# CompVis/stable-diffusion

Hardware: AMD Instinct MI355X
Metric: 512x512 images/sec, SD-v1-4 50-step PLMS CFG=7.5 (higher is better)
Workload: dtype f16

## Files before the change

include/sdmi.h:

```cpp
#ifndef SDMI_H_
#define SDMI_H_

#include <stdint.h>

#ifdef __cplusplus
extern "C" {
#endif

#define SDMI_ABI_VERSION 17

typedef struct sdmi_unet sdmi_unet;

typedef struct sdmi_unet_cfg {
  int32_t in_channels;
  int32_t out_channels;
  int32_t model_channels;
  int32_t num_res_blocks;
  int32_t n_levels;
  int32_t channel_mult[8];
  int32_t n_attention_resolutions;
  int32_t attention_resolutions[8];
  int32_t num_heads;
  int32_t transformer_depth;
  int32_t context_dim;
// ... 95 lines not shown
int sdmi_clip_set_weight(sdmi_clip* h, const char* key, const float* ptr, const int64_t* shape, int ndim, void* stream);
int sdmi_clip_finalize(sdmi_clip* h);
int64_t sdmi_clip_workspace_bytes(sdmi_clip* h, int B, int L);
int sdmi_clip_forward(sdmi_clip* h, const int64_t* ids, float* out, int B, int L, void* workspace, int64_t workspace_bytes,
                      void* stream);

typedef struct sdmi_bert sdmi_bert;
typedef struct sdmi_bert_cfg {
  int32_t vocab_size;
  int32_t dim;
  int32_t depth;
  int32_t heads;
  int32_t dim_head;
  int32_t ff_inner;
  int32_t max_seq_len;
} sdmi_bert_cfg;
int sdmi_bert_create(const sdmi_bert_cfg* cfg, sdmi_bert** out);
int sdmi_bert_destroy(sdmi_bert* h);
int sdmi_bert_num_weights(const sdmi_bert* h);
int sdmi_bert_weight_info(const sdmi_bert* h, int idx, char* key_buf, int key_buf_len, int64_t* shape4, int* ndim);
int sdmi_bert_set_weight(sdmi_bert* h, const char* key, const float* ptr, const int64_t* shape, int ndim, void* stream);
int sdmi_bert_finalize(sdmi_bert* h);
int64_t sdmi_bert_workspace_bytes(sdmi_bert* h, int B, int L);
int sdmi_bert_forward(sdmi_bert* h, const int64_t* ids, float* out, int B, int L, void* workspace, int64_t workspace_bytes,
                      void* stream);

typedef struct sdmi_igemm_desc {
  const void* a0; const void* a1; const void* a2;
  int32_t c0, c1, c2, lda0, lda1, lda2;
  int32_t B, Hin, Win, Hout, Wout, ksize, stride, up;
  const void* w;
  int32_t N;
  int32_t mode;
  const float* bias; const float* rowvec; int32_t ld_rowvec;
  const float* residual; int32_t ldr;
  float* out_f32; void* out_f16; int32_t ldo;
  void* seg_dst[3]; int32_t seg_kind[3];
  int32_t heads, dh, ntok, ntok_pad, segC;
  int32_t splitk;
  float* splitk_ws; int64_t splitk_ws_floats;
  int32_t tile;
  int32_t dma;
  int32_t asym_pad;
  int32_t gn_n; void* gn_acc[2]; int32_t gn_cpg[2]; int32_t gn_cbase[2];
  int32_t* splitk_cnt; int32_t splitk_cnt_ints;
  int32_t split16;
  const float* f16_scale; float* lnp_out;
  const float* lnf_part; int32_t lnf_npart; float lnf_eps; const float* lnf_cs; const float* lnf_d;
  const float* pgn_gamma; const float* pgn_beta; float pgn_eps; int32_t pgn_silu;
  void* pgn_out; int32_t pgn_keep_f32; int32_t* pgn_applied;
  void* out_lo;
} sdmi_igemm_desc;
int sdmi_k_igemm(const sdmi_igemm_desc* d, void* stream);
int sdmi_k_ff_tail(const sdmi_igemm_desc* proj_out, const void* ln_f16, const float* lnp, float ln_eps, const float* csd,
                   const void* wgg_f16, const void* wff2_f16, const float* bff2, const float* t, void* stream);
int sdmi_k_st_tail(const sdmi_igemm_desc* proj_out, const void* a_f16, const void* wo_f16, const float* bo, float* t, const float* ln_gamma,
                   float ln_eps, const float* csd, const void* wgg_f16, const void* wff2_f16, const float* bff2, void* stream);
int sdmi_k_gn_conv3(const sdmi_igemm_desc* conv, const float* x0, const float* x1, int c0, int c1, float* gn_ws, int64_t gn_ws_floats,
                    const float* gn_gamma, const float* gn_beta, float gn_eps, void* stream);
int sdmi_k_st_head(const float* x, float* gn_ws, int64_t gn_ws_floats, const float* gn_gamma, const float* gn_beta, float gn_eps,
                   const void* w_in3, const float* b_in, float* t, const float* ln_gamma, float ln_eps, const void* wqkv_f16,
                   const float* lnf_cs, const float* lnf_d, void* q, void* k, void* vt, int B, int ntok, int ntok_pad, int heads, int dh,
                   int C, void* stream);
int sdmi_k_st_mid(const void* a_f16, const void* wo_f16, const float* bo, float* t, const float* ln_gamma, float ln_eps, const void* wq_f16,
                  const float* lnf_cs, const float* lnf_d, void* q, int B, int ntok, int heads, int dh, int C, void* stream);
int sdmi_k_st_mid_ctx(const void* a_f16, const void* wo_f16, const float* bo, float* t, const float* ln_gamma, float ln_eps, const void* wq_f16,
                      const float* lnf_cs, const float* lnf_d, const void* ctx_k, const void* ctx_vt, int nkv, int nkv_pad, float scale, void* ao_out,
                      int B, int ntok, int heads, int dh, int C, void* stream);
int sdmi_k_ln_fold_prep(const void* w_f16, int N, int K, int ldw, const float* gamma, const float* beta, const float* bias,
                        float* cs, float* d, void* stream);
int sdmi_k_attention(const void* q, const void* k, const void* vt, void* out, int BH, int heads, int nq, int nkv,
                     int nkv_pad, int d, float scale, void* stream);
int sdmi_k_attention_split16(const void* q, const void* q_lo, const void* k, const void* k_lo, const void* vt, const void* vt_lo, void* out,
                             void* out_lo, int BH, int heads, int nq, int nkv, int nkv_pad, int d, float scale, void* stream);
int sdmi_k_attention_causal(const void* q, const void* k, const void* vt, void* out, int BH, int heads, int n, int n_pad,
                            int d, float scale, void* stream);
int sdmi_k_groupnorm(const float* x0, const float* x1, int c0, int c1, int B, int HW, const float* gamma,
                     const float* beta, float eps, int silu, void* out_f16, float* out_f32, void* raw_f16, void* out_lo,
                     void* raw_lo, float* partial_ws, int64_t partial_floats, void* stream);
int64_t sdmi_k_groupnorm_ws_floats(int B, int HW);
int sdmi_k_layernorm(const float* x, const float* gamma, const float* beta, void* out_f16, int M, int C, float eps,
                     void* stream);
int sdmi_k_cast_f16(const float* x, void* out_f16, void* out_lo, int64_t n, void* stream);
int sdmi_k_split_heads(const float* src, int ld, int col0, void* dst, void* dst_lo, int kind, int B, int ntok, int ntok_pad, int heads, int dh,
                       void* stream);
int sdmi_k_geglu_split(const float* src, int M, int F, void* out, void* out_lo, void* stream);
int sdmi_k_layernorm_split(const float* x, const float* gamma, const float* beta, void* out, void* out_lo, int M, int C, float eps, void* stream);
int sdmi_k_timestep_embedding(const int64_t* t_i64, const float* t_f32, float* out, int B, int dim, void* stream);
int sdmi_k_small_linear(const float* in, int ld_in, const float* w, const float* bias, float* out, int ld_out, int B,
                        int N, int K, int silu_in, void* stream);
int sdmi_k_conv_in(const float* x_nchw, const float* w_oihw, const float* bias, float* out_nhwc, int B, int Cin, int H,
                   int W, int Cout, void* stream);
int sdmi_k_conv_out(const float* h_nhwc, const float* w_ohwi, const float* bias, float* out_nchw, int B, int H, int W,
                    int Cin, int Cout, void* stream);
int sdmi_k_pack_conv_weight(const float* w_oihw, void* dst_f16, int O, int I, int KH, int KW, void* stream);
int sdmi_k_pack_conv_out(const float* w_oihw, float* dst_ohwi, int O, int I, void* stream);
int sdmi_k_pack_split3(const float* w, void* dst_f16, int N, int K, void* stream);
int sdmi_k_pack_conv_split3(const float* w_oihw, void* dst_f16, int O, int I, int KH, int KW, void* stream);
int sdmi_k_pointwise_nchw(const float* x, const float* w, const float* bias, float* out, int B, int Cin, int Cout, int HW,
                          float in_scale, void* stream);
int sdmi_k_softmax_rows(const float* S, void* P_f16, int rows, int cols, float scale, void* stream);
int sdmi_k_vq_quantize(const float* z, float z_scale, const float* codebook, float* norms_ws, int n_embed, int D, float* zq, int32_t* idx,
                       int B, int HW, void* stream);
int sdmi_k_resample2(const float* x, float* out_f32, void* out_f16, void* out_lo, int B, int H, int W, int C, int dir, void* stream);
int sdmi_k_gelu_erf(const float* x, void* out_f16, int64_t n, void* stream);
int sdmi_k_pack_geglu(const float* w, const float* bias, void* wdst_f16, float* bdst, int N, int K, void* stream);
// ... 17 lines not shown
```

stable-diffusion_amd/_lib.py:

```python
import ctypes as C
import os

_HERE = os.path.dirname(os.path.abspath(__file__))
LIB_PATH = os.environ.get('SDMI_LIB_PATH') or os.path.join(_HERE, 'libsdmi.so')

c_f32p = C.c_void_p
c_ptr = C.c_void_p


class UNetCfg(C.Structure):
    _fields_ = [('in_channels', C.c_int32), ('out_channels', C.c_int32), ('model_channels', C.c_int32),
                ('num_res_blocks', C.c_int32), ('n_levels', C.c_int32), ('channel_mult', C.c_int32 * 8),
                ('n_attention_resolutions', C.c_int32), ('attention_resolutions', C.c_int32 * 8),
                ('num_heads', C.c_int32), ('transformer_depth', C.c_int32), ('context_dim', C.c_int32)]


class VaeCfg(C.Structure):
    _fields_ = [('ch', C.c_int32), ('out_ch', C.c_int32), ('n_levels', C.c_int32), ('ch_mult', C.c_int32 * 8),
                ('num_res_blocks', C.c_int32), ('in_channels', C.c_int32), ('z_channels', C.c_int32),
                ('embed_dim', C.c_int32)]


class UNetExt(C.Structure):
    _fields_ = [('attention_block', C.c_int32), ('resblock_updown', C.c_int32)]
# ... 45 lines not shown
    'sdmi_unet_create_ext': (C.c_int, [C.POINTER(UNetCfg), C.POINTER(UNetExt), C.c_int, C.POINTER(c_ptr)]),
    'sdmi_unet_destroy': (C.c_int, [c_ptr]),
    'sdmi_unet_num_weights': (C.c_int, [c_ptr]),
    'sdmi_unet_weight_info': (C.c_int, [c_ptr, C.c_int, C.c_char_p, C.c_int, C.POINTER(C.c_int64), C.POINTER(C.c_int)]),
    'sdmi_unet_set_weight': (C.c_int, [c_ptr, C.c_char_p, c_ptr, C.POINTER(C.c_int64), C.c_int, c_ptr]),
    'sdmi_unet_finalize': (C.c_int, [c_ptr]),
    'sdmi_unet_packed_bytes': (C.c_int64, [c_ptr]),
    'sdmi_unet_export_packed': (C.c_int, [c_ptr, c_ptr, C.c_int64, c_ptr]),
    'sdmi_unet_import_packed': (C.c_int, [c_ptr, c_ptr, C.c_int64, c_ptr]),
    'sdmi_unet_workspace_bytes': (C.c_int64, [c_ptr, C.c_int, C.c_int, C.c_int, C.c_int]),
    'sdmi_unet_cache_context': (C.c_int, [c_ptr, c_ptr, C.c_int, C.c_int, c_ptr, C.c_int64, c_ptr]),
    'sdmi_unet_reserve_context': (C.c_int, [c_ptr, C.c_int, C.c_int]),
    'sdmi_unet_cache_timesteps': (C.c_int, [c_ptr, C.POINTER(C.c_int64), C.c_int, c_ptr]),
    'sdmi_unet_hint_timestep': (C.c_int, [c_ptr, C.c_int64]),
    'sdmi_unet_tape_stats': (C.c_int, [c_ptr, C.POINTER(C.c_int64), C.POINTER(C.c_int64)]),
    'sdmi_unet_forward': (C.c_int, [c_ptr, c_ptr, c_ptr, c_ptr, c_ptr, c_ptr, C.c_int, C.c_int, C.c_int, C.c_int,
                                    c_ptr, C.c_int64, c_ptr]),
    'sdmi_sampler_step': (C.c_int, [c_ptr, C.c_int, C.c_float, c_ptr, C.c_int, c_ptr, c_ptr, c_ptr, C.c_float,
                                    C.c_float, C.c_float, C.c_float, c_ptr, c_ptr, c_ptr, c_ptr, C.c_int64, c_ptr]),
    'sdmi_dpm_solver_step': (C.c_int, [c_ptr, C.c_int, C.c_float, c_ptr, c_ptr, C.c_float, C.c_float, C.c_float, C.c_float,
                                       C.c_float, C.c_int, c_ptr, c_ptr, C.c_int64, c_ptr]),
    'sdmi_vae_create': (C.c_int, [C.POINTER(VaeCfg), C.c_int, C.POINTER(c_ptr)]),
    'sdmi_vae_destroy': (C.c_int, [c_ptr]),
    'sdmi_vae_create_ext': (C.c_int, [C.POINTER(VaeCfg), C.POINTER(VaeExt), C.c_int, C.POINTER(c_ptr)]),
    'sdmi_vae_decode_vq': (C.c_int, [c_ptr, c_ptr, C.c_float, C.c_int, c_ptr, C.c_int, C.c_int, C.c_int, c_ptr, C.c_int64, c_ptr]),
    'sdmi_k_vq_quantize': (C.c_int, [c_ptr, C.c_float, c_ptr, c_ptr, C.c_int, C.c_int, c_ptr, c_ptr, C.c_int, C.c_int, c_ptr]),
    'sdmi_k_resample2': (C.c_int, [c_ptr, c_ptr, c_ptr, c_ptr, C.c_int, C.c_int, C.c_int, C.c_int, C.c_int, c_ptr]),
    'sdmi_vae_num_weights': (C.c_int, [c_ptr]),
    'sdmi_vae_weight_info': (C.c_int, [c_ptr, C.c_int, C.c_char_p, C.c_int, C.POINTER(C.c_int64), C.POINTER(C.c_int)]),
    'sdmi_vae_set_weight': (C.c_int, [c_ptr, C.c_char_p, c_ptr, C.POINTER(C.c_int64), C.c_int, c_ptr]),
    'sdmi_vae_finalize': (C.c_int, [c_ptr]),
    'sdmi_vae_decode_workspace_bytes': (C.c_int64, [c_ptr, C.c_int, C.c_int, C.c_int]),
    'sdmi_vae_decode': (C.c_int, [c_ptr, c_ptr, C.c_float, c_ptr, C.c_int, C.c_int, C.c_int, c_ptr, C.c_int64, c_ptr]),
    'sdmi_vae_encode_workspace_bytes': (C.c_int64, [c_ptr, C.c_int, C.c_int, C.c_int]),
    'sdmi_vae_encode': (C.c_int, [c_ptr, c_ptr, c_ptr, C.c_int, C.c_int, C.c_int, c_ptr, C.c_int64, c_ptr]),
    'sdmi_clip_create': (C.c_int, [C.POINTER(ClipCfg), C.POINTER(c_ptr)]),
    'sdmi_clip_destroy': (C.c_int, [c_ptr]),
    'sdmi_clip_num_weights': (C.c_int, [c_ptr]),
    'sdmi_clip_weight_info': (C.c_int, [c_ptr, C.c_int, C.c_char_p, C.c_int, C.POINTER(C.c_int64), C.POINTER(C.c_int)]),
    'sdmi_clip_set_weight': (C.c_int, [c_ptr, C.c_char_p, c_ptr, C.POINTER(C.c_int64), C.c_int, c_ptr]),
    'sdmi_clip_finalize': (C.c_int, [c_ptr]),
    'sdmi_clip_workspace_bytes': (C.c_int64, [c_ptr, C.c_int, C.c_int]),
    'sdmi_clip_forward': (C.c_int, [c_ptr, c_ptr, c_ptr, C.c_int, C.c_int, c_ptr, C.c_int64, c_ptr]),
    'sdmi_bert_create': (C.c_int, [C.POINTER(BertCfg), C.POINTER(c_ptr)]),
    'sdmi_bert_destroy': (C.c_int, [c_ptr]),
    'sdmi_bert_num_weights': (C.c_int, [c_ptr]),
    'sdmi_bert_weight_info': (C.c_int, [c_ptr, C.c_int, C.c_char_p, C.c_int, C.POINTER(C.c_int64), C.POINTER(C.c_int)]),
    'sdmi_bert_set_weight': (C.c_int, [c_ptr, C.c_char_p, c_ptr, C.POINTER(C.c_int64), C.c_int, c_ptr]),
    'sdmi_bert_finalize': (C.c_int, [c_ptr]),
    'sdmi_bert_workspace_bytes': (C.c_int64, [c_ptr, C.c_int, C.c_int]),
    'sdmi_bert_forward': (C.c_int, [c_ptr, c_ptr, c_ptr, C.c_int, C.c_int, c_ptr, C.c_int64, c_ptr]),
    'sdmi_has_experiments': (C.c_int, []),
    'sdmi_k_igemm': (C.c_int, [C.POINTER(IGemmDesc), c_ptr]),
    'sdmi_k_ff_tail': (C.c_int, [C.POINTER(IGemmDesc), c_ptr, c_ptr, C.c_float, c_ptr, c_ptr, c_ptr, c_ptr, c_ptr, c_ptr]),
    'sdmi_k_gn_conv3': (C.c_int, [C.POINTER(IGemmDesc), c_ptr, c_ptr, C.c_int, C.c_int, c_ptr, C.c_int64, c_ptr, c_ptr, C.c_float, c_ptr]),
    'sdmi_k_st_mid_ctx': (C.c_int, [c_ptr, c_ptr, c_ptr, c_ptr, c_ptr, C.c_float, c_ptr, c_ptr, c_ptr, c_ptr, c_ptr, C.c_int, C.c_int, C.c_float, c_ptr,
                                    C.c_int, C.c_int, C.c_int, C.c_int, C.c_int, c_ptr]),
    'sdmi_k_st_tail': (C.c_int, [C.POINTER(IGemmDesc), c_ptr, c_ptr, c_ptr, c_ptr, c_ptr, C.c_float, c_ptr, c_ptr, c_ptr, c_ptr, c_ptr]),
    'sdmi_k_st_mid': (C.c_int, [c_ptr, c_ptr, c_ptr, c_ptr, c_ptr, C.c_float, c_ptr, c_ptr, c_ptr, c_ptr, C.c_int, C.c_int, C.c_int, C.c_int,
                                C.c_int, c_ptr]),
    'sdmi_k_st_head': (C.c_int, [c_ptr, c_ptr, C.c_int64, c_ptr, c_ptr, C.c_float, c_ptr, c_ptr, c_ptr, c_ptr, C.c_float, c_ptr, c_ptr, c_ptr,
                                 c_ptr, c_ptr, c_ptr, C.c_int, C.c_int, C.c_int, C.c_int, C.c_int, C.c_int, c_ptr]),
    'sdmi_k_attention_split16': (C.c_int, [c_ptr, c_ptr, c_ptr, c_ptr, c_ptr, c_ptr, c_ptr, c_ptr, C.c_int, C.c_int, C.c_int, C.c_int,
                                           C.c_int, C.c_int, C.c_float, c_ptr]),
    'sdmi_k_attention_causal': (C.c_int, [c_ptr, c_ptr, c_ptr, c_ptr, C.c_int, C.c_int, C.c_int, C.c_int, C.c_int, C.c_float,
                                          c_ptr]),
    'sdmi_k_pointwise_nchw': (C.c_int, [c_ptr, c_ptr, c_ptr, c_ptr, C.c_int, C.c_int, C.c_int, C.c_int, C.c_float, c_ptr]),
    'sdmi_k_softmax_rows': (C.c_int, [c_ptr, c_ptr, C.c_int, C.c_int, C.c_float, c_ptr]),
    'sdmi_k_gelu_erf': (C.c_int, [c_ptr, c_ptr, C.c_int64, c_ptr]),
    'sdmi_k_attention': (C.c_int, [c_ptr, c_ptr, c_ptr, c_ptr, C.c_int, C.c_int, C.c_int, C.c_int, C.c_int, C.c_int,
                                   C.c_float, c_ptr]),
    'sdmi_k_groupnorm': (C.c_int, [c_ptr, c_ptr, C.c_int, C.c_int, C.c_int, C.c_int, c_ptr, c_ptr, C.c_float, C.c_int,
                                   c_ptr, c_ptr, c_ptr, c_ptr, c_ptr, c_ptr, C.c_int64, c_ptr]),
    'sdmi_k_groupnorm_ws_floats': (C.c_int64, [C.c_int, C.c_int]),
    'sdmi_k_layernorm': (C.c_int, [c_ptr, c_ptr, c_ptr, c_ptr, C.c_int, C.c_int, C.c_float, c_ptr]),
    'sdmi_k_cast_f16': (C.c_int, [c_ptr, c_ptr, c_ptr, C.c_int64, c_ptr]),
    'sdmi_k_split_heads': (C.c_int, [c_ptr, C.c_int, C.c_int, c_ptr, c_ptr, C.c_int, C.c_int, C.c_int, C.c_int, C.c_int, C.c_int,
                                     c_ptr]),
    'sdmi_k_geglu_split': (C.c_int, [c_ptr, C.c_int, C.c_int, c_ptr, c_ptr, c_ptr]),
    'sdmi_k_layernorm_split': (C.c_int, [c_ptr, c_ptr, c_ptr, c_ptr, c_ptr, C.c_int, C.c_int, C.c_float, c_ptr]),
    'sdmi_k_timestep_embedding': (C.c_int, [c_ptr, c_ptr, c_ptr, C.c_int, C.c_int, c_ptr]),
    'sdmi_k_small_linear': (C.c_int, [c_ptr, C.c_int, c_ptr, c_ptr, c_ptr, C.c_int, C.c_int, C.c_int, C.c_int,
                                      C.c_int, c_ptr]),
    'sdmi_k_conv_in': (C.c_int, [c_ptr, c_ptr, c_ptr, c_ptr, C.c_int, C.c_int, C.c_int, C.c_int, C.c_int, c_ptr]),
    'sdmi_k_conv_out': (C.c_int, [c_ptr, c_ptr, c_ptr, c_ptr, C.c_int, C.c_int, C.c_int, C.c_int, C.c_int, c_ptr]),
    'sdmi_k_pack_conv_weight': (C.c_int, [c_ptr, c_ptr, C.c_int, C.c_int, C.c_int, C.c_int, c_ptr]),
    'sdmi_k_pack_conv_out': (C.c_int, [c_ptr, c_ptr, C.c_int, C.c_int, c_ptr]),
    'sdmi_k_pack_split3': (C.c_int, [c_ptr, c_ptr, C.c_int, C.c_int, c_ptr]),
    'sdmi_k_pack_conv_split3': (C.c_int, [c_ptr, c_ptr, C.c_int, C.c_int, C.c_int, C.c_int, c_ptr]),
    'sdmi_k_pack_geglu': (C.c_int, [c_ptr, c_ptr, c_ptr, c_ptr, C.c_int, C.c_int, c_ptr]),
    'sdmi_k_ln_fold_prep': (C.c_int, [c_ptr, C.c_int, C.c_int, C.c_int, c_ptr, c_ptr, c_ptr, c_ptr, c_ptr, c_ptr]),
    'sdmi_image_to_uint8': (C.c_int, [c_ptr, c_ptr, C.c_int, C.c_int, C.c_int, C.c_int, c_ptr]),
    'sdmi_range_check': (C.c_int, [C.c_int]),
    'sdmi_range_report': (C.c_int, [C.c_char_p, C.c_int]),
    'sdmi_tune_begin': (C.c_int, []),
    'sdmi_tune_round': (C.c_int, [C.c_int]),
    'sdmi_tune_end': (C.c_int, [C.c_char_p, C.POINTER(C.c_int)]),
    'sdmi_tune_dump': (C.c_int, [C.c_char_p, C.c_int]),
    'sdmi_profile_begin': (C.c_int, []),
    'sdmi_profile_end': (C.c_int, [C.c_char_p, C.c_int]),
    'sdmi_k_prefetch_lines': (C.c_int, [c_ptr, C.c_int64, c_ptr]),
    'sdmi_zero_page': (c_ptr, []),
}

_lib = None

# ... 39 lines not shown
```

stable-diffusion_amd/csrc/api.cpp:

```cpp
#include <string.h>

#include <new>

#include "prof.h"
#include "split16.h"
#include "unet.h"
#include "vae.h"
#include "clip.h"

namespace sdmi {
static thread_local std::string g_err;
void set_error(const std::string& msg) { g_err = msg; }
int fail(const std::string& msg) { g_err = msg; return -1; }
}

struct sdmi_unet { sdmi::UNet impl; };
struct sdmi_vae { sdmi::Vae impl; };
struct sdmi_clip { sdmi::ClipText impl; };
struct sdmi_bert { sdmi::BertText impl; };

using namespace sdmi;

static void* g_zero_page[16] = {nullptr};
static int zero_page(const f16** out) {
// ... 273 lines not shown
  SDMI_CHECK(h && ids && out, "null argument");
  return h->impl.forward(ids, out, B, L, workspace, workspace_bytes, (hipStream_t)stream, false, nullptr);
}
int sdmi_k_vq_quantize(const float* z, float z_scale, const float* codebook, float* norms_ws, int n_embed, int D, float* zq, int32_t* idx,
                       int B, int HW, void* stream) {
  if (launch_vq_norms(codebook, norms_ws, n_embed, D, (hipStream_t)stream)) return -1;
  return launch_vq_quantize(z, z_scale, codebook, norms_ws, n_embed, D, zq, (int*)idx, B, HW, (hipStream_t)stream);
}
int sdmi_k_resample2(const float* x, float* out_f32, void* out_f16, void* out_lo, int B, int H, int W, int C, int dir, void* stream) {
  return launch_resample2(x, out_f32, (f16*)out_f16, (f16*)out_lo, B, H, W, C, dir, (hipStream_t)stream);
}
int sdmi_k_gelu_erf(const float* x, void* out_f16, int64_t n, void* stream) {
  return launch_gelu_erf(x, (f16*)out_f16, n, (hipStream_t)stream);
}
int sdmi_k_attention_causal(const void* q, const void* k, const void* vt, void* out, int BH, int heads, int n, int n_pad,
                            int d, float scale, void* stream) {
  AttnParams a = AttnParams();
  a.q = (const f16*)q; a.k = (const f16*)k; a.vt = (const f16*)vt; a.out = (f16*)out;
  a.BH = BH; a.heads = heads; a.nq = n; a.nkv = n; a.nkv_pad = n_pad; a.d = d; a.scale = scale; a.causal = 1;
  return launch_attention(a, (hipStream_t)stream);
}

static int igemm_params_of(const sdmi_igemm_desc* d, IGemmParams& p) {
  p.a0 = (const f16*)d->a0; p.a1 = (const f16*)d->a1; p.a2 = (const f16*)d->a2;
  p.c0 = d->c0; p.c1 = d->c1; p.c2 = d->c2; p.lda0 = d->lda0; p.lda1 = d->lda1; p.lda2 = d->lda2;
  p.B = d->B; p.Hin = d->Hin; p.Win = d->Win; p.Hout = d->Hout; p.Wout = d->Wout;
  p.ksize = d->ksize; p.stride = d->stride; p.up = d->up; p.pad = d->asym_pad ? 0 : 1;
  p.w = (const f16*)d->w; p.M = d->B * d->Hout * d->Wout; p.N = d->N; p.K = d->ksize * d->ksize * (d->c0 + d->c1 + d->c2);
  p.mode = d->mode; p.bias = d->bias; p.rowvec = d->rowvec; p.ld_rowvec = d->ld_rowvec;
  p.residual = d->residual; p.ldr = d->ldr; p.out_f32 = d->out_f32; p.out_f16 = (f16*)d->out_f16; p.ldo = d->ldo;
  for (int i = 0; i < 3; ++i) { p.seg_dst[i] = (f16*)d->seg_dst[i]; p.seg_kind[i] = d->seg_kind[i]; }
  p.heads = d->heads; p.dh = d->dh; p.ntok = d->ntok; p.ntok_pad = d->ntok_pad; p.segC = d->segC;
  p.splitk = d->splitk; p.splitk_ws = d->splitk_ws; p.splitk_ws_floats = d->splitk_ws_floats;
  p.splitk_cnt = d->splitk_cnt; p.splitk_cnt_ints = d->splitk_cnt_ints;
  p.gn_n = d->gn_n;
  for (int i = 0; i < 2; ++i) { p.gn_acc[i] = (long long*)d->gn_acc[i]; p.gn_cpg[i] = d->gn_cpg[i]; p.gn_cbase[i] = d->gn_cbase[i]; }
  if (d->split16) {
    p.split16 = 1; p.c1 = 0; p.K = d->c0; p.ldw = 3 * d->c0;
  }
  p.f16_scale = d->f16_scale; p.lnp_out = d->lnp_out;
  p.lnf_part = d->lnf_part; p.lnf_npart = d->lnf_npart; p.lnf_eps = d->lnf_eps; p.lnf_cs = d->lnf_cs; p.lnf_d = d->lnf_d;
  p.pgn_gamma = d->pgn_gamma; p.pgn_beta = d->pgn_beta; p.pgn_eps = d->pgn_eps; p.pgn_silu = d->pgn_silu;
  p.pgn_out = (f16*)d->pgn_out; p.pgn_keep_f32 = d->pgn_keep_f32; p.pgn_applied = d->pgn_applied;
  p.out_lo = (f16*)d->out_lo;
  return zero_page(&p.zero_page);
}
int sdmi_k_igemm(const sdmi_igemm_desc* d, void* stream) {
  SDMI_CHECK(d, "null descriptor");
  IGemmParams p = IGemmParams();
  if (igemm_params_of(d, p)) return -1;
  IGemmTune t; t.tile = d->tile; t.dma = d->dma;
  return launch_igemm(p, t, (hipStream_t)stream);
}
int sdmi_k_ff_tail(const sdmi_igemm_desc* proj_out, const void* ln_f16, const float* lnp, float ln_eps, const float* csd,
                   const void* wgg_f16, const void* wff2_f16, const float* bff2, const float* t, void* stream) {
  SDMI_CHECK(proj_out, "null descriptor");
  FfTailParams q = FfTailParams();
  if (igemm_params_of(proj_out, q.epi)) return -1;
  SDMI_CHECK(proj_out->split16 && proj_out->ksize == 1, "ff_tail: the proj_out descriptor is a split-fp16 1x1 (w = sdmi_k_pack_split3)");
  q.ln = (const f16*)ln_f16; q.lnp = lnp; q.ln_eps = ln_eps; q.csd = csd; q.wgg = (const f16*)wgg_f16; q.wff2 = (const f16*)wff2_f16;
  q.bff2 = bff2; q.t = t; q.wpo = (const f16*)proj_out->w;
  return launch_ff_tail(q, (hipStream_t)stream);
}
int sdmi_k_st_tail(const sdmi_igemm_desc* proj_out, const void* a_f16, const void* wo_f16, const float* bo, float* t, const float* ln_gamma,
                   float ln_eps, const float* csd, const void* wgg_f16, const void* wff2_f16, const float* bff2, void* stream) {
  SDMI_CHECK(proj_out && a_f16, "null argument");
  FfTailParams q = FfTailParams();
  if (igemm_params_of(proj_out, q.epi)) return -1;
  SDMI_CHECK(proj_out->split16 && proj_out->ksize == 1, "st_tail: the proj_out descriptor is a split-fp16 1x1 (w = sdmi_k_pack_split3)");
  q.a16 = (const f16*)a_f16; q.wo = (const f16*)wo_f16; q.bo = bo; q.ln_gamma = ln_gamma; q.ln_eps = ln_eps; q.csd = csd;
  q.wgg = (const f16*)wgg_f16; q.wff2 = (const f16*)wff2_f16; q.bff2 = bff2; q.t = t; q.wpo = (const f16*)proj_out->w;
  return launch_ff_tail(q, (hipStream_t)stream);
}
int sdmi_k_gn_conv3(const sdmi_igemm_desc* conv, const float* x0, const float* x1, int c0, int c1, float* gn_ws, int64_t gn_ws_floats,
                    const float* gn_gamma, const float* gn_beta, float gn_eps, void* stream) {
  SDMI_CHECK(conv && x0 && gn_ws && gn_gamma && gn_beta, "gn_conv3: null argument");
  GnConvParams q = GnConvParams();
  if (igemm_params_of(conv, q.epi)) return -1;
  const int B = q.epi.B;
  SDMI_CHECK(gn_ws_floats >= gn_acc_words(B) * 2, "groupnorm workspace too small");
  SDMI_HIP_OK(hipMemsetAsync(gn_ws, 0, gn_acc_words(B) * sizeof(long long), (hipStream_t)stream));
  GroupNormParams g = GroupNormParams();
  g.x0 = x0; g.c0 = c0; g.x1 = x1; g.c1 = c1; g.B = B; g.HW = q.epi.Hout * q.epi.Wout; g.gamma = gn_gamma; g.beta = gn_beta; g.eps = gn_eps;
  g.stats_only = 1; g.acc = (long long*)gn_ws;
  if (launch_groupnorm(g, (hipStream_t)stream)) return -1;
  q.x0 = x0; q.x1 = x1; q.c0 = c0; q.c1 = c1; q.gn_acc = (const long long*)gn_ws; q.gn_gamma = gn_gamma; q.gn_beta = gn_beta; q.gn_eps = gn_eps;
  q.w = (const f16*)conv->w;
  return launch_gn_conv3(q, (hipStream_t)stream);
}
int sdmi_k_st_head(const float* x, float* gn_ws, int64_t gn_ws_floats, const float* gn_gamma, const float* gn_beta, float gn_eps,
                   const void* w_in3, const float* b_in, float* t, const float* ln_gamma, float ln_eps, const void* wqkv_f16,
                   const float* lnf_cs, const float* lnf_d, void* q, void* k, void* vt, int B, int ntok, int ntok_pad, int heads, int dh,
                   int C, void* stream) {
  SDMI_CHECK(x && gn_ws && gn_gamma && gn_beta, "st_head: null argument");
  SDMI_CHECK(gn_ws_floats >= gn_acc_words(B) * 2, "groupnorm workspace too small");
  SDMI_HIP_OK(hipMemsetAsync(gn_ws, 0, gn_acc_words(B) * sizeof(long long), (hipStream_t)stream));
  GroupNormParams g = GroupNormParams();
  g.x0 = x; g.c0 = C; g.B = B; g.HW = ntok; g.gamma = gn_gamma; g.beta = gn_beta; g.eps = gn_eps; g.stats_only = 1; g.acc = (long long*)gn_ws;
  if (launch_groupnorm(g, (hipStream_t)stream)) return -1;
  StHeadParams p = StHeadParams();
  p.x = x; p.gn_acc = (const long long*)gn_ws; p.gn_gamma = gn_gamma; p.gn_beta = gn_beta; p.gn_eps = gn_eps;
  p.w_in = (const f16*)w_in3; p.b_in = b_in; p.t = t; p.ln_gamma = ln_gamma; p.ln_eps = ln_eps; p.wqkv = (const f16*)wqkv_f16;
  p.lnf_cs = lnf_cs; p.lnf_d = lnf_d; p.q = (f16*)q; p.k = (f16*)k; p.vt = (f16*)vt;
  p.M = B * ntok; p.B = B; p.ntok = ntok; p.ntok_pad = ntok_pad; p.heads = heads; p.dh = dh; p.C = C;
  return launch_st_head(p, (hipStream_t)stream);
}
// ... 142 lines not shown
```

stable-diffusion_amd/csrc/common.h:

```cpp
#pragma once
#include <hip/hip_runtime.h>
#include <stdint.h>
#include <algorithm>
#include <string>

#include "tape.h"

typedef _Float16 f16;
typedef _Float16 f16x2 __attribute__((ext_vector_type(2)));
typedef _Float16 f16x4 __attribute__((ext_vector_type(4)));
typedef _Float16 f16x8 __attribute__((ext_vector_type(8)));
typedef float f32x4 __attribute__((ext_vector_type(4)));
typedef float f32x16 __attribute__((ext_vector_type(16)));

#ifdef __HIPCC__
__device__ __forceinline__ float gn_apply_elem(float v, float mean, float rstd, float gamma, float beta, int silu) {
  float t = __builtin_fmaf((v - mean) * rstd, gamma, beta);
  if (silu) t = t * __builtin_amdgcn_rcpf(1.0f + __expf(-t));
  return t;
}
__device__ __forceinline__ void gn_acc_add(unsigned long long* dst, float v) {
  const double d = (double)v;
  const double hi = rint(d);
  atomicAdd(dst, (unsigned long long)(long long)hi);
// ... 30 lines not shown
      return ::sdmi::fail(std::string(#expr) + ": " + hipGetErrorString(_e));                \
  } while (0)

#define SDMI_CHECK(cond, msg)                                                                \
  do {                                                                                       \
    if (!(cond)) return ::sdmi::fail(std::string("check failed: ") + #cond + " -- " + (msg)); \
  } while (0)

static inline int cdiv(int a, int b) { return (a + b - 1) / b; }
static inline int64_t round_up(int64_t a, int64_t b) { return (a + b - 1) / b * b; }

enum EpiMode { EPI_PLAIN = 0, EPI_GEGLU = 1, EPI_HEADS = 2 };

#ifdef SDMI_NT_STORES
#define SDMI_ST(T, ptr, val) __builtin_nontemporal_store((T)(val), (T*)(ptr))
#else
#define SDMI_ST(T, ptr, val) (*(T*)(ptr) = (T)(val))
#endif
#ifndef SDMI_W_AUX
#define SDMI_W_AUX 0
#endif
#ifndef SDMI_WT_STORES
#define SDMI_WT_STORES 1
#endif
#if defined(__HIPCC__) && SDMI_WT_STORES >= 1
typedef unsigned sdmi_u32x4 __attribute__((ext_vector_type(4)));
typedef unsigned sdmi_u32x2 __attribute__((ext_vector_type(2)));
__device__ __forceinline__ void sdmi_st_wt16(const void* base, size_t byte_off, f32x4 v) {
  if (__builtin_expect(byte_off < (size_t)0x80000000u - 16, 1)) {
    const __amdgpu_buffer_rsrc_t r = __builtin_amdgcn_make_buffer_rsrc((void*)base, 0, (int)0x80000000, 0x00020000);
    __builtin_amdgcn_raw_buffer_store_b128(__builtin_bit_cast(sdmi_u32x4, v), r, (int)byte_off, 0, 16);
  } else {
    *(f32x4*)((char*)base + byte_off) = v;
  }
}
__device__ __forceinline__ void sdmi_st_wt8(const void* base, size_t byte_off, f16x4 v) {
  if (__builtin_expect(byte_off < (size_t)0x80000000u - 16, 1)) {
    const __amdgpu_buffer_rsrc_t r = __builtin_amdgcn_make_buffer_rsrc((void*)base, 0, (int)0x80000000, 0x00020000);
    __builtin_amdgcn_raw_buffer_store_b64(__builtin_bit_cast(sdmi_u32x2, v), r, (int)byte_off, 0, 16);
  } else {
    *(f16x4*)((char*)base + byte_off) = v;
  }
}
#define SDMI_ST_F32X4(base, off, val) sdmi_st_wt16((base), (size_t)(off) * 4, (val))
#if SDMI_WT_STORES >= 2
#define SDMI_ST_F16X4(base, off, val) sdmi_st_wt8((base), (size_t)(off) * 2, (val))
#else
#define SDMI_ST_F16X4(base, off, val) SDMI_ST(f16x4, (base) + (off), (val))
#endif
#else
#define SDMI_ST_F32X4(base, off, val) SDMI_ST(f32x4, (base) + (off), (val))
#define SDMI_ST_F16X4(base, off, val) SDMI_ST(f16x4, (base) + (off), (val))
#endif

struct IGemmParams {
  const f16* a0 = nullptr; const f16* a1 = nullptr; const f16* a2 = nullptr;
  int c0 = 0, c1 = 0, c2 = 0;
  int lda0 = 0, lda1 = 0, lda2 = 0;
  int B = 1, Hin = 1, Win = 1;
  int Hout = 1, Wout = 1;
  int ksize = 1, stride = 1, up = 0;
  int pad = 1;
  const f16* w = nullptr;
  int M = 0, N = 0, K = 0;
  int k_alg = 0;
  int split16 = 0;
  int ldw = 0;
  int mode = EPI_PLAIN;
  const float* bias = nullptr;
  const float* rowvec = nullptr; int ld_rowvec = 0;
  const float* residual = nullptr; int ldr = 0;
  float* out_f32 = nullptr; f16* out_f16 = nullptr; int ldo = 0;
  f16* out_lo = nullptr;
  const float* ln_gamma = nullptr; const float* ln_beta = nullptr; f16* ln_out = nullptr; float ln_eps = 1e-5f;
  const float* f16_scale = nullptr;
  float* lnp_out = nullptr;
  const float* lnf_part = nullptr; int lnf_npart = 0; float lnf_eps = 1e-5f;
  const float* lnf_cs = nullptr; const float* lnf_d = nullptr;
  f16* seg_dst[3] = {nullptr, nullptr, nullptr};
  int seg_kind[3] = {0, 0, 0};
  int heads = 0, dh = 0, ntok = 0, ntok_pad = 0, segC = 0;
  int splitk = 1;
  float* splitk_ws = nullptr; int64_t splitk_ws_floats = 0;
  int* splitk_cnt = nullptr; int splitk_cnt_ints = 0;
  int gn_safe = 0;
#ifdef SDMI_IGEMM_TIMING
  long long* dbg_times = nullptr;
  int dbg_abl = 0;
#endif
  int splitk_fused = 0;
  int slab_tiled = 0, slab_bm = 0, slab_bn = 0, slab_wm = 0, slab_wn = 0;
  int slab_sh_qpt = 0, slab_sh_nt = 0, slab_sh_tn = 0, slab_sh_wn = 0;
  int epi_vec = 0;
  int tile_n_fastest = 0;
  const f16* zero_page = nullptr;
  int gn_n = 0;
  long long* gn_acc[2] = {nullptr, nullptr};
  int gn_cpg[2] = {0, 0}, gn_cbase[2] = {0, 0};
  unsigned long long gn_magic[2] = {0, 0};
  const float* pgn_gamma = nullptr; const float* pgn_beta = nullptr; float pgn_eps = 1e-5f; int pgn_silu = 1;
  f16* pgn_out = nullptr;
  int pgn_keep_f32 = 0;
  int* pgn_applied = nullptr;
  unsigned long long magic_hw = 0, magic_w = 0, magic_w2 = 0;
  int log2w = 0;
  const float* xf0 = nullptr; const float* xf1 = nullptr;
  const long long* gn_in_acc = nullptr;
  const float* gn_in_gamma = nullptr; const float* gn_in_beta = nullptr; float gn_in_eps = 1e-5f; int gn_in_silu = 1;
  f16* raw_hi = nullptr; f16* raw_lo = nullptr;
  f16* gn_scratch = nullptr;
  unsigned long long magic_cpg_in = 0;
  int halo_thi = 0, halo_ipt = 1, log2_tpi = 30;
  unsigned long long magic_hpi = 0;
};

constexpr int SDMI_NUM_TILES = 22;
struct IGemmTune {
  int tile = -1;
  int dma = -1;
};

int launch_igemm(const IGemmParams& p, const IGemmTune& tune, hipStream_t stream);
bool range_check_enabled();
uint64_t tune_generation();
bool tune_collecting();
int range_check_set(int enable);
int range_scan(const char* what, const f16* p, int64_t n, hipStream_t stream);
int range_report(std::string* json);

int tune_begin();
int tune_round(int r);
int tune_end(const char* path, int* n_keys);
int tune_dump(std::string* out);
int launch_splitk_reduce(const IGemmParams& p, int nsplit, hipStream_t stream);

struct FfTailParams {
  const f16* ln = nullptr;
  const float* lnp = nullptr;
  float ln_eps = 1e-5f;
  const float* csd = nullptr;
  const f16* wgg = nullptr;
  const f16* wff2 = nullptr;
  const float* bff2 = nullptr;
  const float* t = nullptr;
  const f16* wpo = nullptr;
  const f16* a16 = nullptr;
  const f16* wo = nullptr;
  const float* bo = nullptr;
  const float* ln_gamma = nullptr;
#ifdef SDMI_RC_TIMING
  long long* dbg = nullptr;
#endif
  IGemmParams epi;
};
bool ff_tail_supported(int C, int M, int rows_per_sample);
int launch_ff_tail(const FfTailParams& p, hipStream_t stream);

struct StHeadParams {
  const f16* a16 = nullptr;
  const float* x = nullptr;
  const long long* gn_acc = nullptr;
  const float* gn_gamma = nullptr; const float* gn_beta = nullptr; float gn_eps = 1e-6f;
  const f16* w_in = nullptr;
  const float* b_in = nullptr;
  float* t = nullptr;
  const float* ln_gamma = nullptr;
// ... 134 lines not shown
```

stable-diffusion_amd/csrc/conv3halo.hip:

```cpp
#include "igemm_dev.h"

namespace sdmi {
namespace {

template <int BM, int BN, int WARPS_M, int WARPS_N, int NS>
__global__ void __launch_bounds__(WARPS_M* WARPS_N * 64) conv3halo_kernel(const IGemmParams p, const int tiles_m,
                                                                           const int tiles_n, const int chunks_per_split) {
#if defined(__HIP_DEVICE_COMPILE__)
  constexpr int NT = WARPS_M * WARPS_N * 64;
  constexpr int RPP = NT / 8;
  constexpr int PB = BN / RPP;
  constexpr int WTM = BM / WARPS_M, WTN = BN / WARPS_N;
  constexpr int TM = WTM / 32, TN = WTN / 32;
  constexpr int HPMAX = (BM / 64 + 2) * 66;
  constexpr int AHP = (HPMAX + RPP - 1) / RPP;
  constexpr int HALO_BYTES = AHP * RPP * 128;
  constexpr int BSTAGE = BN * 128;
  constexpr int LDS_BYTES = 2 * HALO_BYTES + NS * BSTAGE;
  constexpr int LASTA = 10 - NS;
  constexpr int PA = (AHP + LASTA) / (LASTA + 1);
  constexpr int KS = BK / 16;
  constexpr int G = (TM * TN >= 4) ? 1 : 2;
  constexpr int U = KS / G;
  constexpr int MPU = G * TM * TN;
  static_assert(PB >= 1 && TM >= 1 && TN >= 1 && RPP % 16 == 0 && NS >= 2 && NS <= 9, "tile/wave shape");
  static_assert(LDS_BYTES <= 160 * 1024, "LDS budget");

  __shared__ __attribute__((aligned(16))) unsigned char smem[LDS_BYTES];

  const int nblk = gridDim.x;
  const int bid = blockIdx.x;
  const int q8 = nblk >> 3, r8 = nblk & 7, xcd = bid & 7;
  const int wgid = (xcd < r8 ? xcd * (q8 + 1) : r8 * (q8 + 1) + (xcd - r8) * q8) + (bid >> 3);
  const int tiles_mn = tiles_m * tiles_n;
  const int split = wgid / tiles_mn;
  const int tmn = wgid - split * tiles_mn;
  int tile_m, tile_n;
  if (p.tile_n_fastest) { tile_m = tmn / tiles_n; tile_n = tmn - tile_m * tiles_n; }
  else { tile_n = tmn / tiles_m; tile_m = tmn - tile_n * tiles_m; }
  const int m0 = tile_m * BM, n0 = tile_n * BN;
  const int nch = (p.c0 + p.c1 + p.c2) / BK;
  const int c_begin = split * chunks_per_split;
  const int c_end = min(nch, c_begin + chunks_per_split);
  if (c_begin >= c_end) return;

  const int tid = threadIdx.x;
  SDMI_STAMP(dbg_t0);
  const int lane = tid & 63;
  const int wave = tid >> 6;
  const int cpos = tid & 7, lrow = tid >> 3;
  const int gch = cpos ^ ((lrow >> 1) & 7);
  const int wave_u = __builtin_amdgcn_readfirstlane(wave);
  const int wm = wave / WARPS_N, wn = wave - wm * WARPS_N;
  const int l31 = lane & 31, lg = lane >> 5;
  const int rsw = (l31 >> 1) & 7;

  const int W = p.Wout, H = p.Hout, HW = H * W, W2 = W + 2, ld = p.lda0;
  const int bimg = m0 / HW;
  const int THI = p.halo_thi;
  const int HPI = (THI + 2) * W2;
  const int y0 = p.halo_ipt > 1 ? 0 : (m0 - bimg * HW) >> p.log2w;
  const int HP = p.halo_ipt * HPI;
  constexpr int OOB = (int)0x80000000;

  int hvoff[AHP];
#pragma unroll
  for (int q = 0; q < AHP; ++q) {
    const int hp = q * RPP + lrow;
    const int ip = fast_div(hp, p.magic_hpi), hr = hp - ip * HPI;
    const int hy = fast_div(hr, p.magic_w2), hx = hr - hy * W2;
    const int y = y0 + hy - 1, x = hx - 1;
    const bool valid = hp < HP && y >= 0 && y < H && x >= 0 && x < W;
    hvoff[q] = valid ? ((((bimg + ip) * H + y) * W + x) * ld + gch * 8) * 2 : OOB;
  }
  int b_off[PB];
#pragma unroll
  for (int i = 0; i < PB; ++i) {
    const int n = min(n0 + i * RPP + lrow, p.N - 1);
    b_off[i] = (n * p.K + gch * 8) * 2;
  }
  int hr0[TM];
#pragma unroll
  for (int i = 0; i < TM; ++i) {
    const int ml = wm * WTM + i * 32 + l31;
// ... 91 lines not shown
      const int kt = c * 9 + tap;
      const int tap1 = tap == 8 ? 0 : tap + 1;
      const int hb1 = tap == 8 ? (hb ^ 1) : hb;
      const int cur1 = (cur + 1 == NS) ? 0 : cur + 1;
      int ab1[TM];
#pragma unroll
      for (int i = 0; i < TM; ++i) ab1[i] = a_base(i, tap1 / 3, tap1 % 3, hb1);
      const int alo = a_lo(tap);
      const int na = a_hi(tap) - alo;
      const int npieces = na + PB;
      const int ppu = (npieces + U - 2) / (U - 1);
      const int bt = min(kt + NS - 1, kt_last);
#pragma unroll
      for (int u = 0; u < U; ++u) {
        if (u + 1 < U) {
#pragma unroll
          for (int g = 0; g < G; ++g) read_frags(ab, cur, (u + 1) * G + g, fa[(u + 1) & 1][g], fb[(u + 1) & 1][g]);
#pragma unroll
          for (int e = u * ppu; e < (u + 1) * ppu && e < npieces; ++e) {
            if (e < na) issue_halo(csn, hb ^ 1, alo + e);
            else issue_b(bt, nxt, e - na);
          }
        } else {
          wait_vmcnt_n(in_flight_ok(tap));
          asm volatile("s_waitcnt lgkmcnt(0)\n\ts_barrier" ::: "memory");
#pragma unroll
          for (int g = 0; g < G; ++g) read_frags(ab1, cur1, g, fa[0][g], fb[0][g]);
        }
#pragma unroll
        for (int g = 0; g < G; ++g) mfma_step(fa[u & 1][g], fb[u & 1][g]);
        __builtin_amdgcn_sched_group_barrier(0x100, G * (TM + TN), 0);
#pragma unroll
        for (int e = 0; e < MPU; ++e) {
          __builtin_amdgcn_sched_group_barrier(0x008, 1, 0);
          if (u + 1 < U && e < ppu && u * ppu + e < npieces) __builtin_amdgcn_sched_group_barrier(0x010, 1, 0);
        }
      }
#pragma unroll
      for (int i = 0; i < TM; ++i) ab[i] = ab1[i];
      cur = cur1;
      nxt = (nxt + 1 == NS) ? 0 : nxt + 1;
      hb = hb1;
    }
  }
  wait_vmcnt<0>();
  SDMI_STAMP(dbg_t2);
  igemm_epilogue<BM, BN, WARPS_M, WARPS_N, LDS_BYTES>(p, acc, m0, n0, split, tile_m, tile_n, smem);
#ifdef SDMI_IGEMM_TIMING
  if (p.dbg_times && tid == 0) {
    long long* d = p.dbg_times + 6 * (size_t)blockIdx.x;
    d[0] = dbg_t0; d[1] = dbg_t1; d[2] = dbg_t2; d[4] = (long long)__builtin_readcyclecounter();
  }
#endif
#endif
}

}

bool halo_supported(const IGemmParams& p, int bm) {
  const int W = p.Wout, HW = p.Hout * p.Wout;
  if (!(p.ksize == 3 && p.stride == 1 && p.pad == 1 && !p.up && p.Hin == p.Hout && p.Win == p.Wout && W >= 8 && W <= 64 &&
        (W & (W - 1)) == 0 && bm % W == 0))
    return false;
  const int cap = (((bm / 64 + 2) * 66 + bm / 4 - 1) / (bm / 4)) * (bm / 4);
  if (bm <= HW) return HW % bm == 0 && (bm / W + 2) * (W + 2) <= cap;
  return bm % HW == 0 && p.M % bm == 0 && (bm / HW) * (p.Hout + 2) * (W + 2) <= cap;
}

template <int BM, int BN, int WARPS_M, int WARPS_N, int NS>
int launch_halo_cfg(const IGemmParams& p, int splitk, hipStream_t stream) {
  SDMI_CHECK(halo_supported(p, BM), "halo-staged conv tile requested for an unsupported shape");
  const int tiles_m = cdiv(p.M, BM), tiles_n = cdiv(p.N, BN);
  const int nch = (p.c0 + p.c1 + p.c2) / BK;
  const int chunks_per_split = cdiv(nch, splitk);
  const int nsplit = cdiv(nch, chunks_per_split);
  IGemmParams q = p;
  q.splitk = nsplit;
  q.tile_n_fastest = tile_order_n_fastest(p);
  q.splitk_fused = 0;
  slab_layout(q, BM, BN, WARPS_M, WARPS_N, nsplit);
  q.epi_vec = epi_vec_ok(p);
  SDMI_CHECK(splitk_ws_need(p, BM, BN, nsplit) <= p.splitk_ws_floats, "split-K workspace too small");
  SDMI_CHECK((int64_t)p.M < (int64_t)65536 * p.Hout * p.Wout, "fast_div_hw: at most 65535 samples per launch");
  q.magic_hw = div_magic_hw(p.Hout * p.Wout);
  q.magic_w = div_magic(p.Wout);
  q.magic_w2 = div_magic(p.Wout + 2);
  q.log2w = 0;
  while ((1 << q.log2w) < p.Wout) ++q.log2w;
  {
    const int HW = p.Hout * p.Wout;
    q.halo_ipt = BM <= HW ? 1 : BM / HW;
    q.halo_thi = BM <= HW ? BM / p.Wout : p.Hout;
    q.magic_hpi = div_magic((q.halo_thi + 2) * (p.Wout + 2));
    const int tpi = q.halo_thi * p.Wout;
    q.log2_tpi = 0;
    while ((1 << q.log2_tpi) < tpi) ++q.log2_tpi;
    if (q.halo_ipt == 1) q.log2_tpi = 30;
  }
  for (int t = 0; t < p.gn_n; ++t) q.gn_magic[t] = div_magic(p.gn_cpg[t]);
  dim3 grid(tiles_m * tiles_n * nsplit), block(WARPS_M * WARPS_N * 64);
  static const int by_shape = env_int("SDMI_PROF_SHAPES", 0);
  std::string pname = std::string("conv3halo_") + std::to_string(BM) + "x" + std::to_string(BN) + "w" +
                      std::to_string(WARPS_M * WARPS_N) + "s" + std::to_string(NS);
  if (by_shape && prof_enabled())
    pname += "_M" + std::to_string(p.M) + "_N" + std::to_string(p.N) + "_K" + std::to_string(p.K) + "_s" + std::to_string(nsplit);
  const double src_pix = (double)p.B * p.Hin * p.Win;
  ProfScope ps(pname.c_str(), 2.0 * p.M * (double)p.N * p.K,
               src_pix * (p.c0 + p.c1) * 2.0 + (double)p.N * p.K * 2.0 + (double)p.M * p.N * ((p.out_f32 ? 4.0 : 0.0) + (p.out_f16 ? 2.0 : 0.0)) +
                   (p.residual ? (double)p.M * p.N * 4.0 : 0.0),
               stream);
  SDMI_LAUNCH((conv3halo_kernel<BM, BN, WARPS_M, WARPS_N, NS>), grid, block, 0, stream, q, tiles_m, tiles_n, chunks_per_split);
  SDMI_HIP_OK(hipGetLastError());
  ps.end();
  if (nsplit > 1) return launch_splitk_reduce(q, nsplit, stream);
  if (q.ln_out) return launch_layernorm(q.out_f32, q.ln_gamma, q.ln_beta, q.ln_out, q.M, q.N, q.ln_eps, stream);
  return 0;
}

int launch_halo_tile(int tile, const IGemmParams& p, int splitk, hipStream_t stream) {
  switch (tile) {
    case 14: return launch_halo_cfg<256, 64, 4, 2, 5>(p, splitk, stream);
    case 15: return launch_halo_cfg<256, 128, 4, 2, 3>(p, splitk, stream);
    case 16: return launch_halo_cfg<128, 64, 2, 2, 8>(p, splitk, stream);
    case 17: return launch_halo_cfg<128, 128, 2, 2, 5>(p, splitk, stream);
    default: return fail("not a halo-staged conv tile id");
  }
}

}
```

stable-diffusion_amd/csrc/gemm_split16.hip:

```cpp
#include "igemm_dev.h"

namespace sdmi {
namespace {

template <int BM, int BN, int WARPS_M, int WARPS_N, int NS>
__global__ void __launch_bounds__(WARPS_M* WARPS_N * 64) gemm_split16_kernel(const IGemmParams p, const int tiles_m, const int tiles_n,
                                                                               const int kt_per_split) {
#if defined(__HIP_DEVICE_COMPILE__)
  constexpr int NT = WARPS_M * WARPS_N * 64;
  constexpr int RPP = NT / 8;
  constexpr int A_PASSES = BM / RPP, B_PASSES = BN / RPP;
  constexpr int WTM = BM / WARPS_M, WTN = BN / WARPS_N;
  constexpr int TM = WTM / 32, TN = WTN / 32;
  constexpr int A_BYTES = BM * 128, B_BYTES = BN * 128;
  constexpr int STAGE_BYTES = 2 * (A_BYTES + B_BYTES);
  constexpr int LPT = 2 * (A_PASSES + B_PASSES);
  constexpr int KS = BK / 16;
  constexpr int PPU = (LPT + KS - 2) / (KS - 1);
  static_assert(A_PASSES >= 1 && B_PASSES >= 1 && TM >= 1 && TN >= 1 && RPP % 16 == 0 && NS >= 2, "tile/wave shape");
  static_assert(NS * STAGE_BYTES <= 160 * 1024, "LDS budget");

  __shared__ __attribute__((aligned(16))) unsigned char smem[NS * STAGE_BYTES];

  const int nblk = gridDim.x, bid = blockIdx.x;
  const int q8 = nblk >> 3, r8 = nblk & 7, xcd = bid & 7;
  const int wgid = (xcd < r8 ? xcd * (q8 + 1) : r8 * (q8 + 1) + (xcd - r8) * q8) + (bid >> 3);
  const int tiles_mn = tiles_m * tiles_n;
  const int split = wgid / tiles_mn;
  const int tmn = wgid - split * tiles_mn;
  int tile_m, tile_n;
  if (p.tile_n_fastest) { tile_m = tmn / tiles_n; tile_n = tmn - tile_m * tiles_n; }
  else { tile_n = tmn / tiles_m; tile_m = tmn - tile_n * tiles_m; }
  const int m0 = tile_m * BM, n0 = tile_n * BN;
  const int nkt = p.K / BK;
  const int kt_begin = split * kt_per_split;
  const int kt_end = min(nkt, kt_begin + kt_per_split);
  if (kt_begin >= kt_end) return;

  const int tid = threadIdx.x;
  SDMI_STAMP(dbg_t0);
  const int lane = tid & 63, wave = tid >> 6;
  const int cpos = tid & 7, lrow = tid >> 3;
  const int gch = cpos ^ ((lrow >> 1) & 7);
  const int wave_u = __builtin_amdgcn_readfirstlane(wave);

  int a_off[A_PASSES], b_off[B_PASSES];
#pragma unroll
  for (int i = 0; i < A_PASSES; ++i) a_off[i] = (min(m0 + i * RPP + lrow, p.M - 1) * p.lda0 + gch * 8) * 2;
#pragma unroll
  for (int i = 0; i < B_PASSES; ++i) b_off[i] = (min(n0 + i * RPP + lrow, p.N - 1) * p.ldw + gch * 8) * 2;
  constexpr int OOB = (int)0x80000000;
  const __amdgpu_buffer_rsrc_t rsrc_hi = __builtin_amdgcn_make_buffer_rsrc((void*)p.a0, 0, OOB, 0x00020000);
  const __amdgpu_buffer_rsrc_t rsrc_lo = __builtin_amdgcn_make_buffer_rsrc((void*)p.a1, 0, OOB, 0x00020000);
  const __amdgpu_buffer_rsrc_t rsrc_w = __builtin_amdgcn_make_buffer_rsrc((void*)p.w, 0, OOB, 0x00020000);
  const int w_lo_off = 2 * p.K * 2;

  auto issue_piece = [&](int kt, int stage, int q) {
    const int soff = kt * (BK * 2);
    const bool isA = q < 2 * A_PASSES;
    const int qa = isA ? q : q - 2 * A_PASSES;
    const int npass = isA ? A_PASSES : B_PASSES;
    const int half = qa >= npass ? 1 : 0, pass = qa - half * npass;
    const unsigned row0 = (isA ? half * BM : 2 * BM + half * BN) + pass * RPP + wave_u * 8;
    auto dst = (__attribute__((address_space(3))) void*)(smem + stage * STAGE_BYTES + row0 * 128);
    if (isA) __builtin_amdgcn_raw_ptr_buffer_load_lds(half ? rsrc_lo : rsrc_hi, dst, 16, a_off[pass], soff, 0, 0);
    else __builtin_amdgcn_raw_ptr_buffer_load_lds(rsrc_w, dst, 16, b_off[pass], soff + (half ? w_lo_off : 0), 0, SDMI_W_AUX);
  };

  const int wm = wave / WARPS_N, wn = wave - wm * WARPS_N;
  const int l31 = lane & 31, lg = lane >> 5;
  const int rsw = (l31 >> 1) & 7;
  f32x16 acc[TM][TN];
#pragma unroll
  for (int i = 0; i < TM; ++i)
#pragma unroll
    for (int j = 0; j < TN; ++j)
#pragma unroll
      for (int r = 0; r < 16; ++r) acc[i][j][r] = 0.f;

  struct Frags { f16x8 ah[TM], al[TM], bh[TN], bl[TN]; };
  const int a_lds = (wm * WTM + l31) * 128, b_lds = 2 * A_BYTES + (wn * WTN + l31) * 128;
  auto read_frags = [&](int stage, int ks, Frags& f) {
    const unsigned char* st = smem + stage * STAGE_BYTES + (((ks * 2 + lg) ^ rsw) << 4);
#pragma unroll
    for (int i = 0; i < TM; ++i) {
      f.ah[i] = *(const f16x8*)(st + a_lds + i * 32 * 128);
      f.al[i] = *(const f16x8*)(st + a_lds + A_BYTES + i * 32 * 128);
    }
#pragma unroll
    for (int j = 0; j < TN; ++j) {
      f.bh[j] = *(const f16x8*)(st + b_lds + j * 32 * 128);
      f.bl[j] = *(const f16x8*)(st + b_lds + B_BYTES + j * 32 * 128);
    }
  };
  auto mfma_step = [&](const Frags& f) {
#pragma unroll
    for (int i = 0; i < TM; ++i)
#pragma unroll
      for (int j = 0; j < TN; ++j) {
        acc[i][j] = __builtin_amdgcn_mfma_f32_32x32x16_f16(f.ah[i], f.bh[j], acc[i][j], 0, 0, 0);
        acc[i][j] = __builtin_amdgcn_mfma_f32_32x32x16_f16(f.al[i], f.bh[j], acc[i][j], 0, 0, 0);
        acc[i][j] = __builtin_amdgcn_mfma_f32_32x32x16_f16(f.ah[i], f.bl[j], acc[i][j], 0, 0, 0);
      }
  };

  SDMI_STAMP(dbg_t1);
  int ld_kt = kt_begin;
  auto next_kt = [&]() { const int k = ld_kt; if (ld_kt + 1 < kt_end) ++ld_kt; return k; };
#pragma unroll
  for (int s = 0; s < NS - 1; ++s) {
    const int k = next_kt();
#pragma unroll
    for (int q = 0; q < LPT; ++q) issue_piece(k, s, q);
  }
  wait_vmcnt<LPT*(NS - 2)>();
  asm volatile("s_waitcnt lgkmcnt(0)\n\ts_barrier" ::: "memory");
  Frags fr[2];
  read_frags(0, 0, fr[0]);
  int cur = 0, nxt = NS - 1;
  for (int kt = kt_begin; kt < kt_end; ++kt) {
    const int kload = next_kt();
    const int cur1 = (cur + 1 == NS) ? 0 : cur + 1;
#pragma unroll
    for (int u = 0; u < KS; ++u) {
      if (u + 1 < KS) {
        read_frags(cur, u + 1, fr[(u + 1) & 1]);
#pragma unroll
        for (int q = u * PPU; q < (u + 1) * PPU && q < LPT; ++q) issue_piece(kload, nxt, q);
      } else {
        wait_vmcnt<LPT*(NS - 2)>();
        asm volatile("s_waitcnt lgkmcnt(0)\n\ts_barrier" ::: "memory");
        read_frags(cur1, 0, fr[0]);
      }
      mfma_step(fr[u & 1]);
      __builtin_amdgcn_sched_group_barrier(0x100, 2 * (TM + TN), 0);
#pragma unroll
      for (int e = 0; e < 3 * TM * TN; ++e) {
        __builtin_amdgcn_sched_group_barrier(0x008, 1, 0);
        if (u + 1 < KS && e < PPU && u * PPU + e < LPT) __builtin_amdgcn_sched_group_barrier(0x010, 1, 0);
      }
    }
    cur = cur1;
    nxt = (nxt + 1 == NS) ? 0 : nxt + 1;
  }
  wait_vmcnt<0>();
  SDMI_STAMP(dbg_t2);
  igemm_epilogue<BM, BN, WARPS_M, WARPS_N, NS * STAGE_BYTES>(p, acc, m0, n0, split, tile_m, tile_n, smem);
#ifdef SDMI_IGEMM_TIMING
  if (p.dbg_times && tid == 0) {
    long long* d = p.dbg_times + 6 * (size_t)blockIdx.x;
    d[0] = dbg_t0; d[1] = dbg_t1; d[2] = dbg_t2; d[4] = (long long)__builtin_readcyclecounter();
  }
#endif
#endif
}

template <int BM, int BN, int WARPS_M, int WARPS_N, int NS>
int launch_split16_cfg(const IGemmParams& p, int splitk, hipStream_t stream) {
  const int tiles_m = cdiv(p.M, BM), tiles_n = cdiv(p.N, BN);
  const int nkt = p.K / BK;
  const int kt_per_split = cdiv(nkt, splitk);
  const int nsplit = cdiv(nkt, kt_per_split);
  IGemmParams q = p;
  q.splitk = nsplit;
  q.tile_n_fastest = tile_order_n_fastest(p);
  q.splitk_fused = 0;
  slab_layout(q, BM, BN, WARPS_M, WARPS_N, nsplit);
  q.epi_vec = epi_vec_ok(p);
  SDMI_CHECK(splitk_ws_need(p, BM, BN, nsplit) <= p.splitk_ws_floats, "split-K workspace too small");
  SDMI_CHECK((int64_t)p.M < (int64_t)65536 * p.Hout * p.Wout, "fast_div_hw: at most 65535 samples per launch");
  q.magic_hw = div_magic_hw(p.Hout * p.Wout);
  q.magic_w = div_magic(p.Wout);
  for (int t = 0; t < p.gn_n; ++t) q.gn_magic[t] = div_magic(p.gn_cpg[t]);
  dim3 grid(tiles_m * tiles_n * nsplit), block(WARPS_M * WARPS_N * 64);
  static const int by_shape = env_int("SDMI_PROF_SHAPES", 0);
  std::string pname = std::string("gemm_split16_") + std::to_string(BM) + "x" + std::to_string(BN) + "w" +
                      std::to_string(WARPS_M * WARPS_N) + "s" + std::to_string(NS);
  if (by_shape && prof_enabled())
    pname += "_M" + std::to_string(p.M) + "_N" + std::to_string(p.N) + "_K" + std::to_string(p.K) + "_s" + std::to_string(nsplit);
  ProfScope ps(pname.c_str(), 2.0 * p.M * (double)p.N * p.K,
               (double)p.M * p.K * 2.0 + (double)p.N * p.K * 2.0 + (double)p.M * p.N * ((p.out_f32 ? 4.0 : 0.0) + (p.out_f16 ? 2.0 : 0.0)) +
                   (p.residual ? (double)p.M * p.N * 4.0 : 0.0),
               stream, 6.0 * p.M * (double)p.N * p.K);
  SDMI_LAUNCH((gemm_split16_kernel<BM, BN, WARPS_M, WARPS_N, NS>), grid, block, 0, stream, q, tiles_m, tiles_n, kt_per_split);
  SDMI_HIP_OK(hipGetLastError());
  ps.end();
  if (nsplit > 1) return launch_splitk_reduce(q, nsplit, stream);
  if (q.ln_out) return launch_layernorm(q.out_f32, q.ln_gamma, q.ln_beta, q.ln_out, q.M, q.N, q.ln_eps, stream);
  return 0;
}

}

bool split16_tile_supported(int tile) { return tile == 0 || tile == 1 || tile == 2 || tile == 4 || tile == 5 || tile == 8 || tile == 10; }

int launch_split16_tile(int tile, const IGemmParams& p, int splitk, hipStream_t stream) {
  SDMI_CHECK(p.a0 && p.a1 && p.ksize == 1 && p.mode == EPI_PLAIN && p.c1 == 0 && p.c2 == 0 && p.K == p.c0 && p.K % BK == 0 &&
                 p.lda0 % 8 == 0 && p.ldw % 8 == 0 && p.ldw >= 3 * p.K,
             "split-fp16 GEMM: hi + lo operands, plain epilogue, K % 64 == 0, packed [N][3K] weights");
  switch (tile) {
    case 0: return launch_split16_cfg<128, 128, 2, 2, 2>(p, splitk, stream);
    case 1: return launch_split16_cfg<128, 64, 2, 2, 2>(p, splitk, stream);
    case 2: return launch_split16_cfg<64, 64, 2, 2, 2>(p, splitk, stream);
    case 4: return launch_split16_cfg<128, 64, 2, 2, 3>(p, splitk, stream);
    case 5: return launch_split16_cfg<64, 64, 2, 2, 3>(p, splitk, stream);
    case 8: return launch_split16_cfg<64, 128, 2, 2, 3>(p, splitk, stream);
    case 10: return launch_split16_cfg<64, 64, 2, 2, 4>(p, splitk, stream);
    default: return fail("split-fp16 GEMM: tile id without an instantiation");
  }
}

}
```

stable-diffusion_amd/csrc/igemm.hip:

```cpp
#include <dlfcn.h>

#include <map>
#include <mutex>
#include <tuple>
#include <vector>

#include "igemm_dev.h"

namespace sdmi {
namespace {

__global__ void __launch_bounds__(256) splitk_reduce_kernel(IGemmParams p, int nsplit, int rows_per_block) {
  __shared__ unsigned long long s_gn[2][32][GN_WORDS];
  const int tx = threadIdx.x & 7, ty = threadIdx.x >> 3;
  const int n = (blockIdx.x * 8 + tx) * 4;
  const int row0 = blockIdx.y * rows_per_block;
  const int HW = p.Hout * p.Wout;
  const bool gn = p.gn_n > 0;
  const bool ncol = n < p.N;
  if (gn) {
    for (int i = threadIdx.x; i < 2 * 32 * GN_WORDS; i += 256) (&s_gn[0][0][0])[i] = 0ull;
    __syncthreads();
  }
  const size_t slab_sz = (size_t)p.M * p.N;
// ... 85 lines not shown
  f16* dst = p.seg_dst[seg];
  if (p.seg_kind[seg] == 0) {
    *(f16x4*)(dst + (bh * p.ntok + tok) * p.dh + dd) = f16x4{(f16)v[0], (f16)v[1], (f16)v[2], (f16)v[3]};
  } else {
#pragma unroll
    for (int j = 0; j < 4; ++j) dst[(bh * p.dh + dd + j) * p.ntok_pad + tok] = (f16)v[j];
  }
}

__device__ __forceinline__ float pick4(const f32x4 v, int idx) {
  return idx == 0 ? v[0] : (idx == 1 ? v[1] : (idx == 2 ? v[2] : v[3]));
}
template <int CTRL>
__device__ __forceinline__ float quad_dpp(float x) {
  return __builtin_bit_cast(float, __builtin_amdgcn_update_dpp(0, __builtin_bit_cast(int, x), CTRL, 0xF, 0xF, true));
}
__device__ __forceinline__ f32x4 quad_transpose(const f32x4 v, int sub) {
  const float r0 = pick4(v, sub);
  const float r1 = quad_dpp<0x93>(pick4(v, (sub + 1) & 3));
  const float r2 = quad_dpp<0x4E>(pick4(v, (sub + 2) & 3));
  const float r3 = quad_dpp<0x39>(pick4(v, (sub + 3) & 3));
  const f32x4 r = {r0, r1, r2, r3};
  return f32x4{pick4(r, sub & 3), pick4(r, (sub - 1) & 3), pick4(r, (sub - 2) & 3), pick4(r, (sub - 3) & 3)};
}
__device__ __forceinline__ void quad_partials_split(const f32x4 v, int gsplit, float* a1, float* a2, float* c1, float* c2) {
#pragma clang fp contract(off)
  float s1 = 0.f, s2 = 0.f, t1 = 0.f, t2 = 0.f;
#pragma unroll
  for (int j = 0; j < 4; ++j) {
    const float sq = v[j] * v[j];
    if (j < gsplit) { s1 += v[j]; s2 += sq; } else { t1 += v[j]; t2 += sq; }
  }
  *a1 = s1; *a2 = s2; *c1 = t1; *c2 = t2;
}
struct TiledQuad { size_t off; int m, n; bool valid; };
__device__ __forceinline__ TiledQuad tiled_quad(const IGemmParams& p, int q, int lane) {
  const int BM = p.slab_bm, BN = p.slab_bn;
  const int WTM = BM / p.slab_wm, WTN = BN >> p.slab_sh_wn;
  const int tiles_n = (p.N + BN - 1) / BN;
  const int tile = q >> p.slab_sh_qpt, rem = q - (tile << p.slab_sh_qpt);
  const int blk = rem >> p.slab_sh_nt, t_in = rem - (blk << p.slab_sh_nt);
  const int wave = t_in >> 6;
  const int ij = blk >> 2, r4 = blk & 3, i = ij >> p.slab_sh_tn, j = ij - (i << p.slab_sh_tn);
  const int wm = wave >> p.slab_sh_wn, wn = wave - (wm << p.slab_sh_wn);
  const int tile_m = tile / tiles_n, tile_n = tile - tile_m * tiles_n;
  const int l31 = lane & 31, lg = lane >> 5;
  TiledQuad t;
  t.off = (size_t)tile * (size_t)(BM * BN) + (size_t)rem * 4;
  t.m = tile_m * BM + wm * WTM + i * 32 + 8 * r4 + 4 * lg + (l31 & 3);
  t.n = tile_n * BN + wn * WTN + j * 32 + (l31 & ~3);
  t.valid = t.m < p.M && t.n < p.N;
  return t;
}
#ifndef SDMI_REDUCE_GN_XCD_DEFAULT
#define SDMI_REDUCE_GN_XCD_DEFAULT 0
#endif
constexpr int COOP_BAR_INTS = 18 * 32;
template <bool COOP>
__global__ void __launch_bounds__(COOP ? 1024 : 256) splitk_reduce_tiled_kernel(IGemmParams p, int nsplit) {
  constexpr int NWV = COOP ? 16 : 4;
  __shared__ unsigned long long s_gn[2][NWV][32][GN_WORDS];
  const int tid = threadIdx.x, lane = tid & 63, wv = tid >> 6, NTB = blockDim.x;
  const bool gn = p.gn_n > 0;
  if (gn) {
    for (int i = tid; i < 2 * NWV * 32 * GN_WORDS; i += NTB) (&s_gn[0][0][0][0])[i] = 0ull;
    __syncthreads();
  }
  const TiledQuad t = tiled_quad(p, blockIdx.x * NTB + tid, lane);
  const int ntiles = ((p.M + p.slab_bm - 1) / p.slab_bm) * ((p.N + p.slab_bn - 1) / p.slab_bn);
  const size_t split_stride = (size_t)ntiles * (size_t)(p.slab_bm * p.slab_bn);
  const float* src = p.splitk_ws + t.off;
  const int HW = p.Hout * p.Wout;
  const int m = min(t.m, p.M - 1), n = min(t.n, p.N - 4);
  f32x4 biasv = {0.f, 0.f, 0.f, 0.f}, rvv = {0.f, 0.f, 0.f, 0.f}, resv = {0.f, 0.f, 0.f, 0.f};
  if (p.bias) biasv = *(const f32x4*)(p.bias + n);
  if (p.rowvec) rvv = *(const f32x4*)(p.rowvec + (size_t)(m / HW) * p.ld_rowvec + n);
  if (p.residual) resv = *(const f32x4*)(p.residual + (size_t)m * p.ldr + n);
  f32x4 part[16];
#pragma unroll
  for (int s = 0; s < 16; ++s) part[s] = (s < nsplit) ? *(const f32x4*)(src + s * split_stride) : f32x4{0.f, 0.f, 0.f, 0.f};
  f32x4 a = part[0];
#pragma unroll
  for (int s = 1; s < 16; ++s) a += part[s];
  f32x4 v = quad_transpose(a, lane & 3);
  v += biasv;
  if (p.rowvec) v += rvv;
  if (p.residual) v += resv;
  if (t.valid) {
    if (p.out_f32 && (!COOP || p.pgn_keep_f32)) SDMI_ST_F32X4(p.out_f32, (size_t)m * p.ldo + n, v);
    if (p.out_f16) SDMI_ST_F16X4(p.out_f16, (size_t)m * p.ldo + n, (f16x4{(f16)v[0], (f16)v[1], (f16)v[2], (f16)v[3]}));
    if (p.out_lo) {
      f16x4 lo;
#pragma unroll
      for (int j = 0; j < 4; ++j) lo[j] = (f16)(v[j] - (float)(f16)v[j]);
      *(f16x4*)(p.out_lo + (size_t)m * p.ldo + n) = lo;
    }
  }
  if (gn) {
    if (t.valid) {
      for (int tg = 0; tg < p.gn_n; ++tg) {
        const int c = p.gn_cbase[tg] + n;
        const int g0 = fast_div(c, p.gn_magic[tg]), g1 = fast_div(c + 3, p.gn_magic[tg]);
        const int gsplit = (g0 + 1) * p.gn_cpg[tg] - c;
        float a1, a2, c1, c2;
        quad_partials_split(v, gsplit, &a1, &a2, &c1, &c2);
        gn_acc_add(&s_gn[tg][wv][g0][0], a1);
        gn_acc_add(&s_gn[tg][wv][g0][2], a2);
        if (g1 != g0) { gn_acc_add(&s_gn[tg][wv][g1][0], c1); gn_acc_add(&s_gn[tg][wv][g1][2], c2); }
      }
    }
    __syncthreads();
    const int slot = blockIdx.x & (GN_SLOTS - 1);
    for (int e = tid; e < p.gn_n * NWV * 32 * GN_WORDS; e += NTB) {
      const unsigned long long w = (&s_gn[0][0][0][0])[e];
      if (w == 0ull) continue;
      const int word = e % GN_WORDS, g = (e / GN_WORDS) % 32, w4 = (e / (GN_WORDS * 32)) % NWV, tg = e / (GN_WORDS * 32 * NWV);
      if (w4 * 64 >= NTB) continue;
      const TiledQuad t0 = tiled_quad(p, blockIdx.x * NTB + w4 * 64, 0);
      if (t0.m >= p.M) continue;
      const int b = t0.m / HW;
      atomicAdd((unsigned long long*)p.gn_acc[tg] + ((size_t)(b * 32 + g) * GN_SLOTS + slot) * GN_STRIDE + word, w);
    }
  }
  if constexpr (COOP) {
    __shared__ int s_ok;
    __shared__ float2 s_tab[NWV][4];
    asm volatile("s_waitcnt vmcnt(0)" ::: "memory");
    __syncthreads();
    int* const blk = p.splitk_cnt + p.splitk_cnt_ints - COOP_BAR_INTS;
    const int nblk = (int)gridDim.x, ngrp = min(nblk, 8);
    if (tid == 0) {
      const int g = (int)blockIdx.x & 7, pop = (nblk - g + 7) >> 3;
      const int ep = __hip_atomic_load(blk + 9 * 32, __ATOMIC_RELAXED, __HIP_MEMORY_SCOPE_AGENT) + 1;
      if (__hip_atomic_fetch_add(blk + g * 32, 1, __ATOMIC_RELAXED, __HIP_MEMORY_SCOPE_AGENT) == pop - 1) {
        if (__hip_atomic_fetch_add(blk + 8 * 32, 1, __ATOMIC_RELAXED, __HIP_MEMORY_SCOPE_AGENT) == ngrp - 1) {
          for (int j = 0; j <= 8; ++j) __hip_atomic_store(blk + j * 32, 0, __ATOMIC_RELAXED, __HIP_MEMORY_SCOPE_AGENT);
          __hip_atomic_store(blk + 9 * 32, ep, __ATOMIC_RELAXED, __HIP_MEMORY_SCOPE_AGENT);
          for (int j = 0; j < ngrp; ++j) __hip_atomic_store(blk + (10 + j) * 32, ep, __ATOMIC_RELAXED, __HIP_MEMORY_SCOPE_AGENT);
        }
      }
// ... 18 lines not shown
      if (sub == 0) {
        float mu, rs;
        gn_mean_rstd(a0, a1, q0, q1, (double)cpg * (double)HW, p.pgn_eps, &mu, &rs);
        s_tab[wv][lane >> 3] = float2{mu, rs};
      }
    }
    __syncthreads();
    if (t.valid) {
      const float2 mr = s_tab[wv][min(fast_div(n, p.gn_magic[0]) - gfirst, 3)];
      const f32x4 ga = *(const f32x4*)(p.pgn_gamma + n), be = *(const f32x4*)(p.pgn_beta + n);
      f16x4 o;
#pragma unroll
      for (int j = 0; j < 4; ++j) o[j] = s_ok ? (f16)gn_apply_elem(v[j], mr.x, mr.y, ga[j], be[j], p.pgn_silu) : (f16)__builtin_nanf("");
      SDMI_ST_F16X4(p.pgn_out, (size_t)m * p.N + n, o);
    }
  }
}

__global__ void __launch_bounds__(256) splitk_reduce_tiled_heads_kernel(IGemmParams p, int nsplit) {
  const int tid = threadIdx.x, lane = tid & 63;
  const TiledQuad t = tiled_quad(p, blockIdx.x * 256 + tid, lane);
  const int ntiles = ((p.M + p.slab_bm - 1) / p.slab_bm) * ((p.N + p.slab_bn - 1) / p.slab_bn);
  const size_t split_stride = (size_t)ntiles * (size_t)(p.slab_bm * p.slab_bn);
  const float* src = p.splitk_ws + t.off;
  f32x4 part[16];
#pragma unroll
  for (int s = 0; s < 16; ++s) part[s] = (s < nsplit) ? *(const f32x4*)(src + s * split_stride) : f32x4{0.f, 0.f, 0.f, 0.f};
  f32x4 a = part[0];
#pragma unroll
  for (int s = 1; s < 16; ++s) a += part[s];
  f32x4 v = quad_transpose(a, lane & 3);
  if (!t.valid) return;
  const int m = t.m, n = t.n;
  if (p.bias) v += *(const f32x4*)(p.bias + n);
  const int seg = n / p.segC;
  const int c = n - seg * p.segC;
  const int head = c / p.dh;
  const int dd = c - head * p.dh;
  const int b = m / p.ntok;
  const int tok = m - b * p.ntok;
  const size_t bh = (size_t)b * p.heads + head;
  f16* dst = p.seg_dst[seg];
  if (p.seg_kind[seg] == 0) {
    *(f16x4*)(dst + (bh * p.ntok + tok) * p.dh + dd) = f16x4{(f16)v[0], (f16)v[1], (f16)v[2], (f16)v[3]};
  } else {
#pragma unroll
    for (int j = 0; j < 4; ++j) dst[(bh * p.dh + dd + j) * p.ntok_pad + tok] = (f16)v[j];
  }
}


}

int launch_splitk_reduce(const IGemmParams& p, int nsplit, hipStream_t stream) {
  SDMI_CHECK(nsplit >= 1 && nsplit <= 16 && p.N % 4 == 0 && p.splitk_ws, "splitk_reduce: bad arguments");
  if (p.slab_tiled) {
    const int64_t quads = (int64_t)cdiv(p.M, p.slab_bm) * cdiv(p.N, p.slab_bn) * (p.slab_bm * p.slab_bn / 4);
    SDMI_CHECK(quads % 256 == 0 && quads / 256 < (1ll << 31) && p.slab_wm > 0 && p.slab_wn > 0, "tiled split-K slabs: bad geometry");
    const double mn = (double)p.M * p.N;
    if (p.mode == EPI_HEADS) {
      ProfScope psh("splitk_reduce", 0.0, mn * (4.0 * nsplit + 2.0), stream);
      SDMI_LAUNCH(splitk_reduce_tiled_heads_kernel, dim3((unsigned)(quads / 256)), dim3(256), 0, stream, p, nsplit);
      SDMI_HIP_OK(hipGetLastError());
      return 0;
    }
    if (p.gn_n > 0) SDMI_CHECK((p.Hout * p.Wout) % 32 == 0, "GroupNorm statistics need Hout*Wout % 32 == 0");
    const bool coop = env_int("SDMI_REDUCE_GN_XCD", SDMI_REDUCE_GN_XCD_DEFAULT) && p.pgn_out && p.pgn_gamma && p.pgn_beta && p.mode == EPI_PLAIN && p.gn_n == 1 &&
                      p.gn_cbase[0] == 0 && p.gn_cpg[0] == p.N / 32 && p.N % 128 == 0 && p.N / 32 >= 16 && p.M == p.B * p.Hout * p.Wout &&
                      (p.Hout * p.Wout) % 32 == 0 && !p.out_f16 && !p.out_lo && !p.ln_out && p.splitk_cnt && p.splitk_cnt_ints >= COOP_BAR_INTS &&
                      quads % 1024 == 0 && quads / 1024 <= 256 && (!p.pgn_keep_f32 || (p.out_f32 && p.ldo % 4 == 0));
    ProfScope pst(coop ? "splitk_reduce_gn" : "splitk_reduce", 0.0, coop ? mn * (4.0 * nsplit + 2.0 + (p.pgn_keep_f32 ? 4.0 : 0.0)) : mn * 4.0 * (nsplit + 1), stream);
    const int rb_env = env_int("SDMI_REDUCE_BLOCK", 256);
    const int rb = (rb_env == 128 || (rb_env == 0 && quads / 256 < 512)) ? 128 : 256;
    if (coop) {
      SDMI_LAUNCH(splitk_reduce_tiled_kernel<true>, dim3((unsigned)(quads / 1024)), dim3(1024), 0, stream, p, nsplit);
      SDMI_HIP_OK(hipGetLastError());
      pst.end();
      if (p.pgn_applied) *p.pgn_applied = 1;
      if (range_check_enabled() && range_scan("GroupNorm fp16 output (split-K reduction)", p.pgn_out, (int64_t)p.M * p.N, stream)) return -1;
      return 0;
    }
    SDMI_LAUNCH(splitk_reduce_tiled_kernel<false>, dim3((unsigned)(quads / rb)), dim3(rb), 0, stream, p, nsplit);
    SDMI_HIP_OK(hipGetLastError());
    pst.end();
    if (p.ln_out) return launch_layernorm(p.out_f32, p.ln_gamma, p.ln_beta, p.ln_out, p.M, p.N, p.ln_eps, stream);
    return 0;
  }
  if (p.mode == EPI_HEADS) {
    const int64_t total_h = (int64_t)p.M * (p.N / 4);
    ProfScope psh("splitk_reduce", 0.0, (double)p.M * p.N * (4.0 * nsplit + 2.0), stream);
    SDMI_LAUNCH(splitk_reduce_heads_kernel, dim3((unsigned)((total_h + 255) / 256)), dim3(256), 0, stream, p, nsplit);
    SDMI_HIP_OK(hipGetLastError());
    return 0;
  }
  const int hw = p.Hout * p.Wout;
  if (p.gn_n > 0) SDMI_CHECK(hw % 32 == 0, "GroupNorm statistics need Hout*Wout % 32 == 0");
  const int rpb = reduce_rows_per_block(p);
  ProfScope ps2("splitk_reduce", 0.0, (double)p.M * p.N * 4.0 * (nsplit + 1), stream);
  SDMI_LAUNCH(splitk_reduce_kernel, dim3((unsigned)cdiv(p.N / 4, 8), (unsigned)cdiv(p.M, rpb)), dim3(256), 0, stream, p, nsplit,
                     rpb);
  SDMI_HIP_OK(hipGetLastError());
  ps2.end();
  if (p.ln_out) return launch_layernorm(p.out_f32, p.ln_gamma, p.ln_beta, p.ln_out, p.M, p.N, p.ln_eps, stream);
  return 0;
}

struct TileCfg { int bm, bn, wm, wn, ns; };
static const TileCfg kTiles[SDMI_NUM_TILES] = {
    {128, 128, 2, 2, 2},
    {128, 64, 2, 2, 2},
    {64, 64, 2, 2, 2},
    {256, 128, 4, 2, 2},
    {128, 64, 2, 2, 3},
    {64, 64, 2, 2, 3},
    {256, 128, 4, 2, 3},
    {128, 128, 2, 2, 3},
    {64, 128, 2, 2, 3},
    {128, 128, 4, 2, 3},
    {64, 64, 2, 2, 4},
    {128, 256, 2, 4, 2},
    {64, 256, 1, 4, 3},
    {256, 64, 4, 1, 3},
    {256, 64, 4, 2, 5},
    {256, 128, 4, 2, 3},
    {128, 64, 2, 2, 8},
    {128, 128, 2, 2, 5},
    {64, 64, 2, 2, 8},
    {64, 128, 2, 2, 6},
    {128, 64, 2, 2, 6},
    {128, 128, 4, 2, 4},
};
static inline bool tile_is_halo(int t) { return t >= 14 && t <= 17; }
static inline bool tile_tn_even(int t) { return (kTiles[t].bn / kTiles[t].wn / 32) % 2 == 0; }

static int launch_tile(int tile, const IGemmParams& p, bool dma, int splitk, hipStream_t stream) {
// ... 124 lines not shown
}
bool tune_collecting() { return g_tuner.collecting; }
static uint64_t g_tune_generation = 0;
uint64_t tune_generation() { return g_tune_generation; }
int tune_end(const char* path, int* n_keys) {
  std::lock_guard<std::mutex> lk(g_tuner.mu);
  if (!g_tuner.collecting) return fail("sdmi_tune_end without sdmi_tune_begin");
  if (tune_drain()) return -1;
  g_tuner.collecting = false;
  auto score = [](std::vector<float> v) -> double {
    if (v.empty()) return 1e30;
    std::sort(v.begin(), v.end());
    return v.size() % 2 ? v[v.size() / 2] : 0.5 * (v[v.size() / 2 - 1] + v[v.size() / 2]);
  };
  for (auto& kv : g_tuner.stats) {
    double best = 1e30; const TuneChoice* bc = nullptr;
    for (auto& c : kv.second) {
      const double sc = score(c.second);
      if (sc < best) { best = sc; bc = &c.first; }
    }
    if (bc) g_tuner.table[kv.first] = {bc->tile, bc->splitk, best};
  }
  if (n_keys) *n_keys = (int)g_tuner.stats.size();
  ++g_tune_generation;
  const std::string out = (path && *path) ? std::string(path) : Tuner::default_path();
  FILE* f = fopen(out.c_str(), "w");
  if (!f) return fail("cannot write the tuning table to " + out);
  fprintf(f, "# libsdmi igemm tuning table (gfx950), measured in situ by tools/tune.py -- M N K ksize stride up mode splitk_req tile splitk us\n");
  for (auto& kv : g_tuner.table) {
    const TuneKey& k = kv.first;
    fprintf(f, "%d %d %d %d %d %d %d %d %d %d %.2f\n", k.M, k.N, k.K, k.ksize, k.stride, k.up, k.mode, k.splitk_req, kv.second.tile,
            kv.second.splitk, kv.second.us);
  }
  fclose(f);
  return 0;
}
int tune_dump(std::string* out) {
  std::lock_guard<std::mutex> lk(g_tuner.mu);
  char buf[256];
  for (auto& kv : g_tuner.stats) {
    const TuneKey& k = kv.first;
    for (auto& c : kv.second) {
      if (c.second.empty()) continue;
      std::vector<float> v = c.second;
      std::sort(v.begin(), v.end());
      snprintf(buf, sizeof buf, "%d %d %d %d %d %d %d %d | %d %d %.2f %.2f %d\n", k.M, k.N, k.K, k.ksize, k.stride, k.up, k.mode,
               k.splitk_req, c.first.tile, c.first.splitk, (double)v[v.size() / 2], (double)v[0], (int)v.size());
      *out += buf;
    }
  }
  return 0;
}

int launch_igemm(const IGemmParams& p, const IGemmTune& tune, hipStream_t stream) {
  SDMI_CHECK(p.M > 0 && p.N > 0 && p.K > 0, "empty GEMM");
  SDMI_CHECK(p.ksize == 1 || p.ksize == 3, "ksize must be 1 or 3");
  const int Cin = p.c0 + p.c1 + p.c2;
  SDMI_CHECK(p.K == p.ksize * p.ksize * Cin, "K != ksize^2 * (c0 + c1 + c2)");
  SDMI_CHECK(Cin % BK == 0 && p.c0 % BK == 0 && p.c1 % BK == 0, "channel counts must be multiples of 64");
  SDMI_CHECK(p.lda0 % 8 == 0 && (p.a1 == nullptr || p.lda1 % 8 == 0), "A row pitch must be a multiple of 8 halves");
  SDMI_CHECK(p.zero_page != nullptr, "zero page missing");
  SDMI_CHECK(p.M == p.B * p.Hout * p.Wout, "M != B * Hout * Wout");
  SDMI_CHECK(p.c1 == 0 || p.a1 != nullptr, "second A source missing");
  SDMI_CHECK(p.c2 == 0 || (p.a2 != nullptr && p.lda2 % 8 == 0), "third A source missing");
  SDMI_CHECK((p.c1 == 0 || p.lda1 == p.lda0) && (p.c2 == 0 || p.lda2 == p.lda0), "all A sources must share one row pitch");
  SDMI_CHECK(!p.up || (p.ksize == 3 && p.stride == 1), "upsample folding needs a 3x3 stride-1 conv");
  if (p.mode == EPI_GEGLU) SDMI_CHECK(p.N % 64 == 0 && p.out_f16 != nullptr, "GEGLU needs N % 64 == 0 and an fp16 output");
  if (p.ln_out)
    SDMI_CHECK(p.mode == EPI_PLAIN && p.out_f32 && p.ldo == p.N && p.N % 4 == 0 && p.N <= 2560 && p.ln_gamma && p.ln_beta,
               "LayerNorm post-op needs plain mode, an fp32 output with ldo == N <= 2560, gamma and beta");
  if (p.out_lo) SDMI_CHECK(p.mode == EPI_PLAIN && p.ldo % 4 == 0, "out_lo needs plain mode");
  if (p.lnp_out || p.f16_scale)
    SDMI_CHECK(p.mode == EPI_PLAIN && p.out_f32 && p.out_f16 && !p.out_lo && !p.ln_out && p.N % 64 == 0 && p.M % 64 == 0 &&
                   (p.Hout * p.Wout) % 64 == 0 && p.splitk == 1 && epi_vec_ok(p),
               "LayerNorm row statistics: plain mode, fp32 + fp16 outputs, no split-K, M / N / rows per sample multiples of 64, 16-byte aligned rows");
  if (p.lnf_part)
    SDMI_CHECK(p.ksize == 1 && p.c1 == 0 && p.c2 == 0 && !p.split16 && p.lnf_npart * 32 == p.K && p.lnf_cs && p.lnf_d && !p.bias &&
                   p.splitk == 1 && p.lnf_npart <= 40,
               "LayerNorm-folding GEMM: dense, one source, K = 32 * lnf_npart <= 1280, column sums + offsets, no bias, no split-K");
  if (p.gn_n) {
    SDMI_CHECK(p.mode == EPI_PLAIN && p.gn_n <= 2 && (p.Hout * p.Wout) % 32 == 0, "GroupNorm statistics need plain mode and Hout*Wout % 32 == 0");
    SDMI_CHECK(p.N % 4 == 0, "GroupNorm statistics: N % 4 == 0");
    for (int t = 0; t < p.gn_n; ++t)
      SDMI_CHECK(p.gn_acc[t] && p.gn_cpg[t] >= 2 && (p.gn_cbase[t] + p.N + p.gn_cpg[t] - 1) / p.gn_cpg[t] <= 32, "bad GroupNorm statistics target");
  }
  if (p.mode == EPI_HEADS) SDMI_CHECK(p.segC > 0 && p.dh > 0 && p.N % p.segC == 0 && p.N / p.segC <= 3, "bad head scatter");

  SDMI_CHECK((int64_t)p.B * p.Hin * p.Win * p.lda0 * 2 + (int64_t)(p.Win + 1) * p.lda0 * 2 < ((int64_t)1 << 31) - 65536 &&
                 (int64_t)p.N * p.K * 2 < ((int64_t)1 << 31) - 65536,
             "tensor too large for 31-bit byte offsets (buffer addressing)");
  static const int env_dma = env_int("SDMI_IGEMM_DMA", 1);
  static const int env_tile = env_int("SDMI_IGEMM_TILE", -1);
  const bool dma = (tune.dma >= 0 ? tune.dma : env_dma) != 0;
  int tile = tune.tile >= 0 ? tune.tile : env_tile;
  SDMI_CHECK(tile < SDMI_NUM_TILES, "unknown igemm tile id");
  int splitk = p.splitk;
  const int nkt = p.K / BK;
  static const int env_split = env_int("SDMI_SPLITK", -1);
  const bool can_split_plain = p.mode == EPI_PLAIN && p.splitk_ws && p.N % 4 == 0 && p.ldo % 4 == 0 &&
                               (p.residual == nullptr || p.ldr % 4 == 0);
  const bool can_split_heads = p.mode == EPI_HEADS && p.splitk_ws && p.dh % 4 == 0 && p.segC % 4 == 0;
  const bool can_split = can_split_plain || can_split_heads;
  if (env_split >= 0 && splitk == 0) splitk = env_split;

  hipEvent_t ev0 = nullptr, ev1 = nullptr;
  TuneKey tkey{p.M, p.N, p.K, p.split16 ? 11 : p.ksize, p.stride, p.up, p.mode, splitk};
  int tcand = -1;
  if (tile < 0) {
    std::lock_guard<std::mutex> lk(g_tuner.mu);
    g_tuner.ensure_loaded();
    static const int only_ksize = env_int("SDMI_TUNE_ONLY_KSIZE", -1);
    if (g_tuner.collecting && (only_ksize < 0 || tkey.ksize == only_ksize)) {
      IGemmParams q = p; q.splitk = splitk;
      const std::vector<TuneChoice> cands = tune_candidates(q, can_split);
      auto& st = g_tuner.stats[tkey];
      if (st.empty()) for (auto& c : cands) st.push_back({c, {}});
      tcand = g_tuner.round % (int)cands.size();
      tile = cands[tcand].tile; splitk = cands[tcand].splitk;
      ev0 = g_tuner.ev(); ev1 = g_tuner.ev();
    } else {
      auto it = g_tuner.table.find(tkey);
      if (it != g_tuner.table.end()) {
        const int tt = it->second.tile, sk = it->second.splitk;
        const bool halo = tile_is_halo(tt);
        const bool ws_ok = sk == 1 || (can_split && splitk_ws_need(p, kTiles[tt].bm, kTiles[tt].bn, sk) <= p.splitk_ws_floats);
        const bool split_ok = splitk != 0 ? (sk == splitk && ws_ok)
                                          : (sk == 1 || (ws_ok && nkt / sk >= 4 && (halo || (sk != 5 && sk != 10)) &&
                                                         (!halo || (nkt / 9) % sk == 0)));
        if (split_ok && (p.mode != EPI_GEGLU || tile_tn_even(tt)) && (!halo || halo_supported(p, kTiles[tt].bm)) &&
            (!p.split16 || split16_tile_supported(tt))) {
          tile = tt; splitk = sk;
        }
      }
    }
  }
  if (p.mode == EPI_GEGLU && tile >= 0 && !tile_tn_even(tile)) tile = 0;
  if (p.split16) {
    if (tile >= 0) SDMI_CHECK(split16_tile_supported(tile), "split-fp16 GEMM: tile id without an instantiation");
    else tile = 5;
  }
  if (tile < 0) {
    const double gflop = 2.0 * p.M * (double)p.N * p.K * 1e-9;
    if (p.mode == EPI_GEGLU) tile = 0;
    else if (p.mode == EPI_HEADS) tile = 2;
    else tile = gflop >= 25.0 ? 3 : 5;
  }
  if (p.lnp_out) {
    const int hw = p.Hout * p.Wout;
    if (p.M % kTiles[tile].bm || p.N % kTiles[tile].bn || hw % kTiles[tile].bm || (p.split16 && !split16_tile_supported(tile))) tile = 5;
  }
  if (splitk <= 0) {
    splitk = 1;
    if (can_split) {
      const long blocks = (long)cdiv(p.M, kTiles[tile].bm) * cdiv(p.N, kTiles[tile].bn);
      const long want = (kTiles[tile].wm * kTiles[tile].wn == 8) ? 160 : 512;
      while (blocks * splitk < want && nkt / (splitk * 2) >= 8 && splitk < 16 &&
             splitk_ws_need(p, kTiles[tile].bm, kTiles[tile].bn, splitk * 2) <= p.splitk_ws_floats)
        splitk *= 2;
    }
  }
  if (splitk > 1) {
    SDMI_CHECK(can_split, "split-K needs plain or head-scatter mode, a slab workspace and N / ldo / ldr multiples of 4");
    SDMI_CHECK(splitk_ws_need(p, kTiles[tile].bm, kTiles[tile].bn, splitk) <= p.splitk_ws_floats, "split-K workspace too small");
  }
  if (ev0) SDMI_HIP_OK(hipEventRecord(ev0, stream));
#ifdef SDMI_IGEMM_TIMING
  static const char* dbg_path = getenv("SDMI_IGEMM_TIMING");
  static const int dbg_abl = env_int("SDMI_EPI_ABL", 0);
  static long long* dbg_buf = nullptr;
  constexpr int DBG_WG = 16384;
  IGemmParams pd = p;
  pd.dbg_abl = dbg_abl;
  if (dbg_path) {
    if (!dbg_buf) SDMI_HIP_OK(hipMalloc((void**)&dbg_buf, 6 * DBG_WG * sizeof(long long)));
    SDMI_HIP_OK(hipMemsetAsync(dbg_buf, 0, 6 * DBG_WG * sizeof(long long), stream));
    pd.dbg_times = dbg_buf;
  }
  const int rc = launch_tile(tile, pd, dma, splitk, stream);
  if (dbg_path && pd.dbg_times && rc == 0) {
    SDMI_HIP_OK(hipStreamSynchronize(stream));
    std::vector<long long> h(6 * DBG_WG);
    SDMI_HIP_OK(hipMemcpy(h.data(), dbg_buf, h.size() * sizeof(long long), hipMemcpyDeviceToHost));
    std::vector<long long> pro, loop, epi, sto, start;
    long long tmin = 0, tmax = 0;
    for (int b = 0; b < DBG_WG; ++b) {
      const long long* d = &h[6 * b];
      if (d[4] == 0) continue;
      pro.push_back(d[1] - d[0]); loop.push_back(d[2] - d[1]); epi.push_back(d[4] - d[2]);
      sto.push_back(d[3] ? d[3] - d[2] : d[4] - d[2]);
      if (start.empty() || d[0] < tmin) tmin = d[0];
      if (d[4] > tmax) tmax = d[4];
      start.push_back(d[0]);
    }
    if (!pro.empty()) {
      auto med = [](std::vector<long long>& v) { std::sort(v.begin(), v.end()); return v[v.size() / 2]; };
      auto mx = [](std::vector<long long>& v) { return *std::max_element(v.begin(), v.end()); };
      long long late = 0;
      for (long long t : start) late = std::max(late, t - tmin);
      if (FILE* f = fopen(dbg_path, "a")) {
        const int nkt_split = (p.K / BK + std::max(splitk, 1) - 1) / std::max(splitk, 1);
        fprintf(f, "M%d N%d K%d k%d mode%d tile%d split%d res%d gn%d blocks%zu k-tiles/block %d | shader cycles: span %lld last-start %lld | median prologue %lld loop %lld epilogue %lld (stores %lld) | max loop %lld max epi %lld | loop cycles per k-tile %.1f\n",
                p.M, p.N, p.K, p.ksize, p.mode, tile, splitk, p.residual ? 1 : 0, p.gn_n, pro.size(), nkt_split, tmax - tmin, late, med(pro), med(loop),
                med(epi), med(sto), mx(loop), mx(epi), (double)med(loop) / nkt_split);
        fclose(f);
      }
    }
  }
#else
  const int rc = launch_tile(tile, p, dma, splitk, stream);
#endif
  if (rc == 0 && range_check_enabled()) {
    const char* what = p.mode == EPI_GEGLU ? "igemm GEGLU output" : (p.mode == EPI_HEADS ? "igemm q/k/v^T" : "igemm fp16 output");
    if (p.mode == EPI_HEADS) {
      for (int sg = 0; sg < p.N / p.segC; ++sg)
        if (range_scan(what, p.seg_dst[sg], p.seg_kind[sg] == 0 ? (int64_t)p.M * p.segC : (int64_t)p.B * p.segC * p.ntok_pad, stream)) return -1;
    } else if (p.out_f16) {
// ... 15 lines not shown
```

stable-diffusion_amd/csrc/igemm_dev.h:

```cpp
#pragma once
#include "common.h"
#include "prof.h"

namespace sdmi {
typedef unsigned u32x4 __attribute__((ext_vector_type(4)));

int launch_splitk_reduce(const IGemmParams& p, int nsplit, hipStream_t stream);
int launch_generic_tile_g0(int tile, const IGemmParams& p, bool dma, int splitk, hipStream_t stream);
int launch_generic_tile_g1(int tile, const IGemmParams& p, bool dma, int splitk, hipStream_t stream);
int launch_generic_tile_g2(int tile, const IGemmParams& p, bool dma, int splitk, hipStream_t stream);

static int env_int(const char* name, int dflt) {
  const char* v = getenv(name);
  return v ? atoi(v) : dflt;
}

namespace {

constexpr int BK = 64;

#ifdef SDMI_IGEMM_TIMING
#define SDMI_STAMP(name) const long long name = p.dbg_times ? (long long)__builtin_readcyclecounter() : 0
#else
#define SDMI_STAMP(name)
// ... 541 lines not shown
              if (m >= p.M) continue;
              const int b2 = m / p.ntok;
              const int t2 = m - b2 * p.ntok;
              const size_t bh2 = (size_t)b2 * p.heads + head;
              const size_t off = kind == 0 ? ((bh2 * p.ntok + t2) * p.dh + dd) : ((bh2 * p.dh + dd) * p.ntok_pad + t2);
              dst[off] = (f16)acc[i][j][r4 * 4 + e];
            }
          }
        }
    }
  }
}

#endif

static unsigned long long div_magic(int d) {
  const unsigned long long one = 1ull << 40;
  return (one + (unsigned long long)d - 1) / (unsigned long long)d;
}
static unsigned long long div_magic_hw(int d) {
  const unsigned long long one = 1ull << 48;
  return (one + (unsigned long long)d - 1) / (unsigned long long)d;
}

static int tile_order_n_fastest(const IGemmParams& p) {
  static const int env_order = env_int("SDMI_TILE_ORDER", 0);
  if (env_order == 1) return 0;
  if (env_order == 2) return 1;
  return p.M > p.N ? 1 : 0;
}

static int reduce_rows_per_block(const IGemmParams& p) {
  int rpb = 32;
  const int hw = p.Hout * p.Wout;
  while (rpb < 256 && (int64_t)cdiv(p.N / 4, 8) * cdiv(p.M, rpb * 2) >= 1024 && (p.gn_n == 0 || hw % (rpb * 2) == 0)) rpb *= 2;
  return rpb;
}
static bool slab_tiled_ok(const IGemmParams& p, int bm, int bn, int nsplit) {
  const int on = env_int("SDMI_SLAB_TILED", 1);
  if (!on || nsplit <= 1 || p.mode == EPI_GEGLU || p.N % 4) return false;
  if ((bm & (bm - 1)) || (bn & (bn - 1))) return false;
  if (p.mode == EPI_PLAIN && p.gn_n > 0 && reduce_rows_per_block(p) != 32) return false;
  if (p.lnf_part || p.lnp_out || p.f16_scale) return false;
  if ((int64_t)nsplit * cdiv(p.M, bm) * bm * cdiv(p.N, bn) * bn > p.splitk_ws_floats) return false;
  return true;
}
static void slab_layout(IGemmParams& q, int bm, int bn, int wm, int wn, int nsplit) {
  q.slab_tiled = slab_tiled_ok(q, bm, bn, nsplit) ? 1 : 0;
  q.slab_bm = bm; q.slab_bn = bn; q.slab_wm = wm; q.slab_wn = wn;
  auto lg2 = [](int v) { int s = 0; while ((1 << s) < v) ++s; return s; };
  q.slab_sh_qpt = lg2(bm * bn / 4); q.slab_sh_nt = lg2(wm * wn * 64); q.slab_sh_tn = lg2(bn / wn / 32); q.slab_sh_wn = lg2(wn);
  if (q.slab_tiled && (((wm * wn) & (wm * wn - 1)) || (wn & (wn - 1)))) q.slab_tiled = 0;
}
static int64_t splitk_ws_need(const IGemmParams& p, int bm, int bn, int nsplit) {
  if (nsplit <= 1) return 0;
  if (slab_tiled_ok(p, bm, bn, nsplit)) return (int64_t)nsplit * cdiv(p.M, bm) * bm * cdiv(p.N, bn) * bn;
  return (int64_t)nsplit * p.M * p.N;
}

static int epi_vec_ok(const IGemmParams& p) {
  if (!env_int("SDMI_EPI_VEC", 1) || p.N % 4) return 0;
  auto al = [](const void* q, uintptr_t a) { return ((uintptr_t)q & (a - 1)) == 0; };
  if (p.mode == EPI_PLAIN)
    return p.ldo % 4 == 0 && al(p.out_f32, 16) && al(p.out_f16, 8) && al(p.out_lo, 8) && al(p.bias, 16) &&
           al(p.rowvec, 16) && p.ld_rowvec % 4 == 0 && al(p.residual, 16) && p.ldr % 4 == 0;
  if (p.mode == EPI_GEGLU) return 0;
  return p.segC % 32 == 0 && p.dh % 4 == 0 && al(p.bias, 16) && al(p.seg_dst[0], 8) && al(p.seg_dst[1], 8) && al(p.seg_dst[2], 8);
}

}

bool halo_supported(const IGemmParams& p, int bm);
int launch_halo_tile(int tile, const IGemmParams& p, int splitk, hipStream_t stream);
bool split16_tile_supported(int tile);

int launch_split16_tile(int tile, const IGemmParams& p, int splitk, hipStream_t stream);

}
```

stable-diffusion_amd/csrc/igemm_kernel.h:

```cpp
#pragma once
#include <string>

#include "igemm_dev.h"

namespace sdmi {
namespace {


template <int BM, int BN, int WARPS_M, int WARPS_N, bool DMA, int NS, int KIND>
__global__ void __launch_bounds__(WARPS_M* WARPS_N * 64) igemm_kernel(const IGemmParams p, const int tiles_m,
                                                                       const int tiles_n, const int kt_per_split) {
  static_assert(DMA || NS == 2, "the register-staged path is double buffered");
#if defined(__HIP_DEVICE_COMPILE__)
  constexpr bool UP = KIND == KIND_3X3_UP;
  constexpr bool K3 = KIND != KIND_1X1;
  constexpr int NT = WARPS_M * WARPS_N * 64;
  constexpr int RPP = NT / 8;
  constexpr int A_PASSES = BM / RPP;
  constexpr int B_PASSES = BN / RPP;
  constexpr int WTM = BM / WARPS_M, WTN = BN / WARPS_N;
  constexpr int TM = WTM / 32, TN = WTN / 32;
  constexpr int STAGE_BYTES = (BM + BN) * 128;
  static_assert(A_PASSES >= 1 && B_PASSES >= 1 && TM >= 1 && TN >= 1, "tile/wave shape");
  static_assert(RPP % 16 == 0, "swizzle assumes pass offset keeps row bits 1..3");
// ... 223 lines not shown
        __builtin_amdgcn_sched_group_barrier(0x100, G * (TM + TN), 0);
#pragma unroll
        for (int e = 0; e < MPU; ++e) {
          __builtin_amdgcn_sched_group_barrier(0x008, 1, 0);
          if (u + 1 < U && e < PPU && u * PPU + e < LPT) __builtin_amdgcn_sched_group_barrier(0x010, 1, 0);
        }
      }
      cur = cur1;
      nxt = (nxt + 1 == NS) ? 0 : nxt + 1;
    }
    wait_vmcnt<0>();
  } else {
    issue_loads(0);
    commit_regs(0);
    for (int kt = kt_begin; kt < kt_end; ++kt) {
      const int cur = (kt - kt_begin) & 1;
      __syncthreads();
      const bool more = (kt + 1 < kt_end);
      if (more) issue_loads(cur ^ 1);
#pragma unroll
      for (int ks = 0; ks < BK / 16; ++ks) {
        f16x8 a[TM], b[TN];
        read_frags(cur, ks, a, b);
        mfma_step(a, b);
      }
      if (more) commit_regs(cur ^ 1);
    }
  }

  SDMI_STAMP(dbg_t2);
  igemm_epilogue<BM, BN, WARPS_M, WARPS_N, NS * STAGE_BYTES>(p, acc, m0, n0, split, tile_m, tile_n, smem, lnf_mean, lnf_rstd);
#ifdef SDMI_IGEMM_TIMING
  if (p.dbg_times && tid == 0) {
    long long* d = p.dbg_times + 6 * (size_t)blockIdx.x;
    d[0] = dbg_t0; d[1] = dbg_t1; d[2] = dbg_t2; d[4] = (long long)__builtin_readcyclecounter();
  }
#endif
#endif
}

template <int BM, int BN, int WARPS_M, int WARPS_N, int NS>
int launch_cfg(const IGemmParams& p, bool dma, int splitk, hipStream_t stream) {
  const int tiles_m = cdiv(p.M, BM), tiles_n = cdiv(p.N, BN);
  const int nkt = p.K / BK;
  const int kt_per_split = cdiv(nkt, splitk);
  const int nsplit = cdiv(nkt, kt_per_split);
  IGemmParams q = p;
  q.splitk = nsplit;
  q.tile_n_fastest = tile_order_n_fastest(p);
  q.splitk_fused = 0;
  slab_layout(q, BM, BN, WARPS_M, WARPS_N, nsplit);
  q.epi_vec = epi_vec_ok(p);
  SDMI_CHECK(splitk_ws_need(p, BM, BN, nsplit) <= p.splitk_ws_floats, "split-K workspace too small");
  SDMI_CHECK((int64_t)p.M < (int64_t)65536 * p.Hout * p.Wout, "fast_div_hw: at most 65535 samples per launch");
  q.magic_hw = div_magic_hw(p.Hout * p.Wout);
  q.magic_w = div_magic(p.Wout);
  for (int t = 0; t < p.gn_n; ++t) q.gn_magic[t] = div_magic(p.gn_cpg[t]);
  dim3 grid(tiles_m * tiles_n * nsplit), block(WARPS_M * WARPS_N * 64);
  static const int by_shape = env_int("SDMI_PROF_SHAPES", 0);
  std::string pname = std::string("igemm_") + std::to_string(BM) + "x" + std::to_string(BN) + "w" +
                      std::to_string(WARPS_M * WARPS_N) + "s" + std::to_string(NS);
  if (by_shape && prof_enabled())
    pname += "_M" + std::to_string(p.M) + "_N" + std::to_string(p.N) + "_K" + std::to_string(p.K) + "_k" +
             std::to_string(p.ksize) + "_m" + std::to_string(p.mode) + "_s" + std::to_string(nsplit);
  const double src_pix = (double)p.B * p.Hin * p.Win;
  const double out_b = (p.out_f32 ? 4.0 : 0.0) + ((p.out_f16 || p.mode != EPI_PLAIN) ? 2.0 : 0.0);
  const double n_out = p.mode == EPI_GEGLU ? p.N / 2.0 : (double)p.N;
  const int k_alg = p.k_alg > 0 ? p.k_alg : p.K;
  const double cin_alg = p.k_alg > 0 ? (double)p.k_alg : (double)(p.c0 + p.c1 + p.c2);
  ProfScope ps(pname.c_str(), 2.0 * p.M * (double)p.N * k_alg,
               src_pix * cin_alg * 2.0 + (double)p.N * k_alg * 2.0 + (double)p.M * n_out * out_b +
                   (p.residual ? (double)p.M * p.N * 4.0 : 0.0),
               stream, 2.0 * p.M * (double)p.N * p.K);
  const int kind = p.ksize == 1 ? KIND_1X1 : (p.up ? KIND_3X3_UP : KIND_3X3);
#define SDMI_LAUNCH_KIND(K_)                                                                                        \
  do {                                                                                                              \
    if (dma) SDMI_LAUNCH((igemm_kernel<BM, BN, WARPS_M, WARPS_N, true, NS, K_>), grid, block, 0, stream, q,   \
                                tiles_m, tiles_n, kt_per_split);                                                    \
    else SDMI_LAUNCH((igemm_kernel<BM, BN, WARPS_M, WARPS_N, false, 2, K_>), grid, block, 0, stream, q,       \
                            tiles_m, tiles_n, kt_per_split);                                                        \
  } while (0)
  if (kind == KIND_1X1) SDMI_LAUNCH_KIND(KIND_1X1);
  else if (kind == KIND_3X3) SDMI_LAUNCH_KIND(KIND_3X3);
  else SDMI_LAUNCH_KIND(KIND_3X3_UP);
#undef SDMI_LAUNCH_KIND
  SDMI_HIP_OK(hipGetLastError());
  ps.end();
  if (nsplit > 1) return launch_splitk_reduce(q, nsplit, stream);
  if (q.ln_out) return launch_layernorm(q.out_f32, q.ln_gamma, q.ln_beta, q.ln_out, q.M, q.N, q.ln_eps, stream);
  return 0;
}

}
}
```

stable-diffusion_amd/csrc/unet.cpp:

```cpp
#include "unet.h"

extern "C" char** environ;
#include "prof.h"
#include "split16.h"

#include <math.h>
#include <stdio.h>
#include <string.h>

#include <algorithm>

namespace sdmi {

static bool in_list(const int* v, int n, int x) {
  for (int i = 0; i < n; ++i)
    if (v[i] == x) return true;
  return false;
}

void UNet::expect(const std::string& key, std::vector<int64_t> shape, WKind kind, void** dst, int row0, int ld,
                  void** dst2) {
  WeightSlot s;
  s.key = key; s.shape = std::move(shape); s.kind = kind; s.dst = dst; s.row0 = row0; s.ld = ld; s.dst2 = dst2;
  slot_index_[key] = (int)slots_.size();
// ... 473 lines not shown
  if (full()) h.reserved |= PK_FULL;
  h.total_bytes = total;
  memcpy(host_buf, &h, sizeof(h));
  int64_t off = (int64_t)round_up((int64_t)sizeof(PackedHeader), PK_ALIGN);
  for (auto& b : bufs) {
    SDMI_HIP_OK(hipMemcpyAsync((char*)host_buf + off, *b.first, b.second, hipMemcpyDeviceToHost, stream));
    off += (int64_t)round_up((int64_t)b.second, PK_ALIGN);
  }
  SDMI_HIP_OK(hipStreamSynchronize(stream));
  return 0;
}

int UNet::import_packed(const void* host_buf, int64_t bytes, hipStream_t stream) {
  SDMI_CHECK(host_buf && bytes >= (int64_t)sizeof(PackedHeader), "packed blob truncated");
  PackedHeader h;
  memcpy(&h, host_buf, sizeof(h));
  SDMI_CHECK(memcmp(h.magic, "SDMIPK01", 8) == 0, "not a libsdmi packed-weight blob");
  SDMI_CHECK(h.abi == SDMI_ABI_VERSION, "packed blob was written by a different ABI version: repack it");
  SDMI_CHECK(memcmp(&h.cfg, &cfg_, sizeof(cfg_)) == 0, "packed blob was written for a different UNet configuration");
  SDMI_CHECK(((h.reserved & PK_FULL) != 0) == full(), std::string("packed blob was written by a ") +
             ((h.reserved & PK_FULL) ? "full" : "mixed") + "-precision UNet handle and cannot be imported into a " + (full() ? "full" : "mixed") +
             "-precision one: repack it with a handle of this precision");
  SDMI_CHECK((h.precise_1x1 != 0) == precise_1x1_, "packed blob was written with a different precision allocation (split-fp16 1x1 convs)");
  SDMI_CHECK((h.reserved & (3 << 4)) == ((ext_.attention_block << 4) | (ext_.resblock_updown << 5)),
             "packed blob was written for a different UNet family (attention_block / resblock_updown)");
  SDMI_CHECK((h.reserved & ~PK_FULL & ~(3 << 4)) == ((precise_kv_ ? 1 : 0) | (precise_last_res_ ? 2 : 0) | (precise_1x1_max_ds_ << 8)),
             "packed blob was written with a different precision allocation (context K / V, last ResBlock, 1x1 conv levels)");
  std::vector<std::pair<void**, size_t>> bufs;
  int64_t total = 0;
  packed_layout(&bufs, &total);
  SDMI_CHECK(h.n_buffers == (int32_t)bufs.size() && h.total_bytes == total && bytes >= total, "packed blob truncated or inconsistent");
  int64_t off = (int64_t)round_up((int64_t)sizeof(PackedHeader), PK_ALIGN);
  for (auto& b : bufs) {
    if (dev_alloc(b.first, b.second)) return -1;
    SDMI_HIP_OK(hipMemcpyAsync(*b.first, (const char*)host_buf + off, b.second, hipMemcpyHostToDevice, stream));
    off += (int64_t)round_up((int64_t)b.second, PK_ALIGN);
  }
  SDMI_HIP_OK(hipStreamSynchronize(stream));
  for (auto& s : slots_) s.set = true;
  ctx_valid_ = false;
  drop_timestep_table();
  return finalize();
}

struct Fwd : FwdBase {
  UNet* u; int Lctx;
  bool ln_fold_on = false;
  bool ff_tail_on = false;
  bool st_head_on = false;
  bool st_mid_on = false;
  bool st_tail_on = false;
  bool st_mid_ctx_on = false;
  bool ctx1_on = false;
  bool gn_conv_on = false;
  float* emb_all = nullptr;
  int emb_ld = 0;
  bool emb_caller = false;
  const f16* ctx16 = nullptr;
  const f16* ctx16_lo = nullptr;

  Act res_block(Layer& L, const Act& x0, const Act* x1) {
    const int H = x0.H, W = x0.W, M = B * H * W;
    const int Cin = x0.C + (x1 ? x1->C : 0), Cout = L.cout;
    if (Cin != L.cin) { ok(fail("res block channel mismatch at " + L.prefix)); }
    if (Cin == Cout && x1) ok(fail("identity skip with a concatenated input at " + L.prefix));
    const size_t mark = scratch.off;
    f16* raw = (Cin != Cout) ? S<f16>((size_t)M * Cin) : nullptr;
    const bool p1 = L.p1x1;
    const bool p3 = L.precise3;
    f16* raw_lo = (Cin != Cout && p1) ? S<f16>((size_t)M * Cin) : nullptr;
    auto split3 = [&](IGemmParams& q, const f16* hi, const f16* lo, int C) {
      q.a0 = hi; q.c0 = C; q.lda0 = C; q.a1 = lo; q.c1 = C; q.lda1 = C; q.a2 = hi; q.c2 = C; q.lda2 = C; q.K = 27 * C; q.k_alg = 9 * C;
    };
    float* h = S<float>((size_t)M * Cout);
    Act out = make_act(P<float>((size_t)M * Cout), Cout, H, W, true);
    Act hact = make_act(h, Cout, H, W, true);
    f16* a2 = nullptr;
    int& gn2_applied = u->gn2_applied_;
    gn2_applied = 0;
    const bool gc1 = gn_conv_on && !p3 && Cin == Cout && gn_conv3_supported(B, H, W, x0.C, x1 ? x1->C : 0, Cout);
    const bool gc2 = gn_conv_on && !p3 && gn_conv3_supported(B, H, W, Cout, 0, Cout);
    auto gn_conv = [&](const Act& a0, const Act* a1, const float* gamma, const float* beta, const f16* w, IGemmParams& e) {
      GnConvParams g = GnConvParams();
      g.gn_acc = groupnorm(a0, a1, gamma, beta, 1e-5f, 1, nullptr, nullptr, nullptr, nullptr, nullptr, true);
      g.x0 = a0.p; g.c0 = a0.C; g.x1 = a1 ? a1->p : nullptr; g.c1 = a1 ? a1->C : 0;
      g.gn_gamma = gamma; g.gn_beta = beta; g.gn_eps = 1e-5f; g.w = w; g.epi = e;
      if (!dry && !rc) ok(launch_gn_conv3(g, s));
    };
    if (gc1) {
      IGemmParams p = conv3(nullptr, Cin, H, W, H, W, 1, 0, L.w16[0], Cout);
      p.bias = L.f32[2]; p.rowvec = emb_all + L.emb_off; p.ld_rowvec = emb_ld;
      p.out_f32 = h; p.ldo = Cout;
      attach_gn_targets(p, hact);
      TapeCaller tc(Tape::R_EMB, emb_caller ? p.rowvec : nullptr);
      gn_conv(x0, x1, L.f32[0], L.f32[1], L.w16[0], p);
    } else {
      f16* a = S<f16>((size_t)M * Cin);
      f16* a_lo = p3 ? S<f16>((size_t)M * Cin) : nullptr;
      groupnorm(x0, x1, L.f32[0], L.f32[1], 1e-5f, 1, a, nullptr, raw, a_lo, raw_lo);
      IGemmParams p = conv3(a, Cin, H, W, H, W, 1, 0, L.w16[0], Cout);
      if (p3) split3(p, a, a_lo, Cin);
      p.bias = L.f32[2]; p.rowvec = emb_all + L.emb_off; p.ld_rowvec = emb_ld;
      p.out_f32 = h; p.ldo = Cout;
      attach_gn_targets(p, hact);
      if (!gc2 && !p3) {
        a2 = S<f16>((size_t)M * Cout);
        p.pgn_gamma = L.f32[3]; p.pgn_beta = L.f32[4]; p.pgn_eps = 1e-5f; p.pgn_silu = 1; p.pgn_out = a2; p.pgn_applied = &gn2_applied;
      }
      TapeCaller tc(Tape::R_EMB, emb_caller ? p.rowvec : nullptr);
      gemm(p);
    }
    const float* residual = x0.p;
    if (Cin != Cout) {
      IGemmParams p = dense1x1(raw, raw_lo, M, Cin, L.w16[2], Cout, H * W, p1);
      p.bias = L.f32[6]; p.out_f32 = out.p; p.ldo = Cout;
      gemm(p);
      residual = out.p;
    }
    if (gc2) {
      IGemmParams p = conv3(nullptr, Cout, H, W, H, W, 1, 0, L.w16[1], Cout);
      p.bias = L.f32[5]; p.residual = residual; p.ldr = Cout; p.out_f32 = out.p; p.ldo = Cout;
      attach_gn_targets(p, out);
      attach_f16_copy(p, out);
      gn_conv(hact, nullptr, L.f32[3], L.f32[4], L.w16[1], p);
    } else {
      f16* a2_lo = nullptr;
      if (p3) { a2 = S<f16>((size_t)M * Cout); a2_lo = S<f16>((size_t)M * Cout); }
      groupnorm(hact, nullptr, L.f32[3], L.f32[4], 1e-5f, 1, a2, nullptr, nullptr, a2_lo, nullptr, false, gn2_applied != 0);
      IGemmParams p = conv3(a2, Cout, H, W, H, W, 1, 0, L.w16[1], Cout);
      if (p3) split3(p, a2, a2_lo, Cout);
      p.bias = L.f32[5]; p.residual = residual; p.ldr = Cout; p.out_f32 = out.p; p.ldo = Cout;
      attach_gn_targets(p, out);
      attach_f16_copy(p, out);
      gemm(p);
    }
    scratch.off = mark;
    return out;
  }

  void context_kv(Layer& L, int d) {
    TBlock& T = L.tb[d];
    const int C = L.cin, Lp = (int)round_up(Lctx, 8);
    const int CD = u->cfg_.context_dim;
    IGemmParams p = dense(ctx16, B * Lctx, CD, T.wkv2, 2 * C, Lctx);
    if (ctx16_lo) {
      p.a1 = ctx16_lo; p.c1 = CD; p.lda1 = CD; p.a2 = ctx16; p.c2 = CD; p.lda2 = CD; p.K = 3 * CD; p.k_alg = CD;
    }
    if (u->full()) {
      const size_t mark = scratch.off;
      float* kv = S<float>((size_t)B * Lctx * 2 * C);
      p.out_f32 = kv; p.ldo = 2 * C;
      gemm(p);
      if (!dry && !rc) ok(launch_split_heads(kv, 2 * C, 0, T.ck, T.ck_lo, 0, B, Lctx, Lp, L.heads, L.dh, s));
      if (!dry && !rc) ok(launch_split_heads(kv, 2 * C, C, T.cvt, T.cvt_lo, 1, B, Lctx, Lp, L.heads, L.dh, s));
      scratch.off = mark;
      return;
    }
    p.mode = EPI_HEADS; p.seg_dst[0] = T.ck; p.seg_dst[1] = T.cvt; p.seg_kind[0] = 0; p.seg_kind[1] = 1;
    p.heads = L.heads; p.dh = L.dh; p.ntok = Lctx; p.ntok_pad = Lp; p.segC = C; p.splitk = 1;
    if (!dry && !rc && Lp != Lctx) {
      hipError_t e = memset_async(T.cvt, 0, (size_t)B * C * Lp * sizeof(f16), s);
      if (e != hipSuccess) ok(fail(std::string("hipMemsetAsync: ") + hipGetErrorString(e)));
    }
    gemm(p);
  }

  Act attn_block_full(Layer& L, const Act& x) {
    const int H = x.H, W = x.W, N = H * W, M = B * N, C = L.cin;
    const int Np = (int)round_up(N, 8), Lp = (int)round_up(Lctx, 8);
    const float scale = 1.0f / sqrtf((float)L.dh);
    const size_t mark = scratch.off;
    f16* a = S<f16>((size_t)M * C); f16* a_lo = S<f16>((size_t)M * C);
    float* t = S<float>((size_t)M * C);
    float* y = S<float>((size_t)M * 8 * C);
    f16* q = S<f16>((size_t)M * C); f16* q_lo = S<f16>((size_t)M * C);
    f16* k = S<f16>((size_t)M * C); f16* k_lo = S<f16>((size_t)M * C);
    f16* vt = S<f16>((size_t)B * C * Np); f16* vt_lo = S<f16>((size_t)B * C * Np);
    f16* gg = S<f16>((size_t)M * 4 * C); f16* gg_lo = S<f16>((size_t)M * 4 * C);
    auto linear = [&](const f16* hi, const f16* lo, int K, const f16* w, int n_out, const float* bias, float* out, bool residual) {
      IGemmParams p = dense1x1(hi, lo, M, K, w, n_out, N, true);
      p.bias = bias; p.out_f32 = out; p.ldo = n_out;
      if (residual) { p.residual = out; p.ldr = n_out; }
      gemm(p);
    };
// ... 449 lines not shown
    tkey.env = sdmi_env_hash() ^ (tune_generation() * 0x9e3779b97f4a7c15ull); tkey.weights_gen = weights_gen_; tkey.ctx_gen = ctx_gen_;
    auto low4 = [](const void* p, int shift) { return (unsigned)((uintptr_t)p & 15) << shift; };
    tkey.align = low4(x, 0) | low4(eps_out, 4) | low4(ctx, 8) | low4(t_i64 ? (const void*)t_i64 : t_f32, 12);
    caller[Tape::R_X] = (uintptr_t)x; caller[Tape::R_OUT] = (uintptr_t)eps_out;
    caller[Tape::R_T] = hinted ? 0 : (t_i64 ? (uintptr_t)t_i64 : (uintptr_t)t_f32);
    caller[Tape::R_CTX] = (uintptr_t)ctx;
    caller[Tape::R_EMB] = hinted ? (uintptr_t)(emb_tab_ + (size_t)hint_row * emb_total_) : 0;
    for (size_t i = 0; i < tapes_.size(); ++i) {
      if (!(tapes_[i].first == tkey)) continue;
      std::unique_ptr<Tape> hit = std::move(tapes_[i].second);
      tapes_.erase(tapes_.begin() + (long)i);
      SDMI_CHECK(finalized_, "sdmi_unet_finalize() has not succeeded yet");
      if (ensure_ctx_cache(B, Lctx, false)) return -1;
      if (!ctx && has_ctx()) SDMI_CHECK(ctx_valid_, "ctx == NULL but no cached context for this (B, Lctx); call sdmi_unet_cache_context first");
      hit->retarget(caller);
      if (replay_verify) { verify_against = std::move(hit); break; }
      const int e = hit->replay(stream);
      const bool sets = hit->sets_ctx_valid;
      const int64_t need = hit->bytes_needed;
      tapes_.emplace_back(tkey, std::move(hit));
      if (e) return fail(std::string("launch tape replay: ") + hipGetErrorString((hipError_t)e));
      if (sets) ctx_valid_ = true;
      if (bytes_needed) *bytes_needed = need;
      ++tape_hits_;
      return 0;
    }
  }
  std::unique_ptr<Tape> fresh;
  if (tape_ok) {
    fresh.reset(new Tape());
    memcpy(fresh->caller, caller, sizeof(caller));
    rec = fresh.get();
  }

  Fwd f;
  f.u = this; f.s = stream; f.dry = dry; f.B = B; f.Lctx = Lctx; f.zero = zero_; f.precise_1x1 = precise_1x1_;
  {
    const char* e_fold = getenv("SDMI_LN_FOLD"); const char* e_vec = getenv("SDMI_EPI_VEC");
    f.ln_fold_on = (e_fold ? atoi(e_fold) != 0 : ln_fold_) && !(e_vec && atoi(e_vec) == 0);
    const char* e_ff = getenv("SDMI_FF_TAIL");
    f.ff_tail_on = e_ff ? atoi(e_ff) != 0 : ff_tail_;
    const char* e_sh = getenv("SDMI_ST_HEAD");
    f.st_head_on = e_sh ? atoi(e_sh) != 0 : st_head_;
    const char* e_sm = getenv("SDMI_ST_MID");
    f.st_mid_on = e_sm ? atoi(e_sm) != 0 : st_head_;
    const char* e_st = getenv("SDMI_ST_TAIL");
    f.st_tail_on = e_st ? atoi(e_st) != 0 : ff_tail_;
    const char* e_mc = getenv("SDMI_ST_MID_CTX");
    f.st_mid_ctx_on = e_mc ? atoi(e_mc) != 0 : st_head_;
    const char* e_c1 = getenv("SDMI_CTX1");
    f.ctx1_on = !(e_c1 && atoi(e_c1) == 0);
    const char* e_gc = getenv("SDMI_GN_CONV");
    f.gn_conv_on = e_gc ? atoi(e_gc) != 0 : false;
    if (full()) {
      f.ln_fold_on = f.ff_tail_on = f.st_head_on = f.st_mid_on = f.st_tail_on = f.st_mid_ctx_on = f.gn_conv_on = false;
    }
  }
  int64_t persist_bytes = 0, scratch_bytes = 0;
  for (int pass = (dry ? 0 : 0); pass < 2; ++pass) {
    const bool d = (pass == 0) ? true : false;
    if (pass == 1 && dry) break;
    f.dry = d; f.rc = 0;
    f.n_acts = 0;
    TapeRecGuard tape_guard(d ? nullptr : rec);
    f.plan = fuse_gn_stats_ ? &gn_plan_ : nullptr;
    if (d) gn_plan_.clear();
    f.persist = Arena(); f.scratch = Arena();
    f.persist.dry = f.scratch.dry = d;
    if (!d) {
      SDMI_CHECK(persist_bytes + scratch_bytes <= ws_bytes, "workspace too small: need " +
                 std::to_string(persist_bytes + scratch_bytes) + " bytes, got " + std::to_string(ws_bytes));
      SDMI_CHECK(workspace != nullptr, "workspace is NULL");
      f.persist.base = (char*)workspace; f.persist.cap = (size_t)persist_bytes;
      f.scratch.base = (char*)workspace + persist_bytes; f.scratch.cap = (size_t)scratch_bytes;
      if (ensure_ctx_cache(B, Lctx, ctx_only)) return -1;
    }
    const int mc = cfg_.model_channels;
    if (f.begin_pass((int64_t)12 << 20)) return -1;
    f16* ctx16 = f.P<f16>((size_t)B * Lctx * cfg_.context_dim);
    f16* ctx16_lo = precise_kv_ ? f.P<f16>((size_t)B * Lctx * cfg_.context_dim) : nullptr;
    const bool have_ctx = has_ctx() && ((ctx != nullptr) || d);
    if (!has_ctx()) {
      f.ctx16 = nullptr; f.ctx16_lo = nullptr;
    } else if (have_ctx) {
      if (!d) {
        TapeCaller tc(Tape::R_CTX, ctx);
        int r = launch_cast_f16(ctx, ctx16, ctx16_lo, (int64_t)B * Lctx * cfg_.context_dim, stream);
        if (r) return r;
      }
      f.ctx16 = ctx16; f.ctx16_lo = ctx16_lo;
    } else {
      SDMI_CHECK(ctx_valid_, "ctx == NULL but no cached context for this (B, Lctx); call sdmi_unet_cache_context first");
      f.ctx16 = nullptr; f.ctx16_lo = nullptr;
    }
    if (ctx_only) {
      auto each = [&](Layer& L) { if (L.kind == L_ATTN) for (int dd = 0; dd < (int)L.tb.size(); ++dd) f.context_kv(L, dd); };
      for (auto& blk : input_blocks_) for (auto& L : blk) each(L);
      for (auto& L : middle_) each(L);
      for (auto& blk : output_blocks_) for (auto& L : blk) each(L);
    } else {
      float* temb = f.P<float>((size_t)B * mc);
      float* e1 = f.P<float>((size_t)B * te_);
      float* emb = f.P<float>((size_t)B * te_);
      f.emb_all = f.P<float>((size_t)B * emb_total_);
      f.emb_ld = emb_total_;
      if (!d && t_i64 != nullptr && hint_row >= 0 && hint_row < (int)emb_tab_t_.size()) {
// ... 90 lines not shown
```

stable-diffusion_amd/csrc/unet.h:

```cpp
#pragma once
#include <stdlib.h>

#include <map>
#include <memory>
#include <string>
#include <utility>
#include <vector>

#include "../../include/sdmi.h"
#include "common.h"

namespace sdmi {

struct Arena {
  char* base = nullptr; size_t cap = 0, off = 0, peak = 0; bool dry = false; bool overflow = false;
  void* alloc(size_t bytes) {
    const size_t a = (off + 255) & ~(size_t)255;
    off = a + bytes;
    peak = std::max(peak, off);
    if (dry) return (void*)(uintptr_t)(a + 4096);
    if (off > cap) { overflow = true; return base; }
    return base + a;
  }
};

struct Act { float* p = nullptr; int C = 0, H = 0, W = 0; int id = -1; bool stats = false; bool can_f16 = false; };

struct GnTarget { int gn_idx = 0, cbase = 0, cpg = 0; };
struct GnPlan {
  std::vector<std::vector<GnTarget>> targets;
  std::vector<char> fused;
  std::vector<char> want_f16;
  void clear() { targets.clear(); fused.clear(); want_f16.clear(); }
};

struct FwdBase {
  hipStream_t s = nullptr; bool dry = false; int B = 1;
  const f16* zero = nullptr;
  bool precise_1x1 = true;
  Arena persist, scratch;
  long long* gn_acc = nullptr;
  int gn_calls = 0;
  float* splitk_ws = nullptr; int64_t splitk_ws_floats = 0;
  int* splitk_cnt = nullptr;
  static constexpr int SPLITK_CNT_INTS = 8192;
  int rc = 0;
  GnPlan* plan = nullptr;
  int n_acts = 0;

  Act make_act(float* ptr, int C, int H, int W, bool by_igemm) {
    Act a; a.p = ptr; a.C = C; a.H = H; a.W = W; a.id = n_acts++;
    a.stats = by_igemm && plan != nullptr && (H * W) % 32 == 0 && H * W >= 1024 / C + 2 && C % 4 == 0 && C / 32 >= 2;
    if (plan && dry && (int)plan->targets.size() < n_acts) plan->targets.resize(n_acts);
    if (plan && dry && (int)plan->want_f16.size() < n_acts) plan->want_f16.resize(n_acts, 0);
    return a;
  }
  std::vector<f16*> f16_of;
  void attach_f16_copy(IGemmParams& p, Act& a) {
    a.can_f16 = plan != nullptr && p.out_f16 == nullptr && p.mode == EPI_PLAIN;
    if (dry || !a.can_f16 || a.id < 0 || a.id >= (int)plan->want_f16.size() || !plan->want_f16[a.id]) return;
    f16* c = P<f16>((size_t)B * a.H * a.W * a.C);
    if ((int)f16_of.size() <= a.id) f16_of.resize(a.id + 1, nullptr);
    f16_of[a.id] = c;
    p.out_f16 = c;
  }
  bool want_f16_copy(const Act& a) {
    if (!dry || !plan || !a.can_f16 || a.id < 0 || a.id >= (int)plan->want_f16.size()) return false;
    if (const char* e = getenv("SDMI_F16_COPY")) { if (atoi(e) == 0) return false; }
    plan->want_f16[a.id] = 1;
    (void)P<f16>((size_t)B * a.H * a.W * a.C);
    return true;
  }
  const f16* f16_copy(const Act& a) const {
    return (!dry && a.id >= 0 && a.id < (int)f16_of.size()) ? f16_of[a.id] : nullptr;
  }
  void attach_gn_targets(IGemmParams& p, const Act& a) {
    p.gn_n = 0;
    if (dry || !plan || !a.stats || a.id < 0 || a.id >= (int)plan->targets.size()) return;
    for (const GnTarget& t : plan->targets[a.id]) {
      if (p.gn_n >= 2) { ok(fail("internal: more than two GroupNorm consumers of one activation")); return; }
      p.gn_acc[p.gn_n] = gn_acc + (size_t)t.gn_idx * gn_acc_words(B);
      p.gn_cpg[p.gn_n] = t.cpg; p.gn_cbase[p.gn_n] = t.cbase;
      ++p.gn_n;
    }
  }

  template <class T> T* P(size_t n) { return (T*)persist.alloc(n * sizeof(T)); }
  template <class T> T* S(size_t n) { return (T*)scratch.alloc(n * sizeof(T)); }
  void ok(int r) { if (r && !rc) rc = r; }
  long long* next_gn_acc() {
    if (gn_calls >= GN_MAX_CALLS) { ok(fail("more GroupNorm calls than accumulator regions")); return gn_acc; }
    return gn_acc + (size_t)(gn_calls++) * gn_acc_words(B);
  }
  long long* last_gn_acc() const { return gn_acc + (size_t)(gn_calls - 1) * gn_acc_words(B); }
  int begin_pass(int64_t splitk_floats, bool with_gn = true) {
    gn_calls = 0;
    gn_acc = nullptr;
    const size_t acc_words = with_gn ? (size_t)GN_MAX_CALLS * gn_acc_words(B) : 0;
    long long* blk = P<long long>(acc_words + SPLITK_CNT_INTS / 2);
    gn_acc = with_gn ? blk : nullptr;
    splitk_cnt = (int*)(blk + acc_words);
    if (!dry) SDMI_HIP_OK(memset_async(blk, 0, (acc_words + SPLITK_CNT_INTS / 2) * sizeof(long long), s));
    splitk_ws_floats = splitk_floats;
    splitk_ws = P<float>((size_t)splitk_floats);
    (void)P<float>((size_t)(splitk_floats / 2));
    return 0;
  }

  void gemm(IGemmParams& p) {
    p.zero_page = zero;
    p.splitk_ws = splitk_ws; p.splitk_ws_floats = splitk_ws_floats;
    p.splitk_cnt = splitk_cnt; p.splitk_cnt_ints = SPLITK_CNT_INTS;
    if (!dry && !rc) ok(launch_igemm(p, IGemmTune(), s));
  }
  IGemmParams dense(const f16* a, int M, int K, const f16* w, int N, int rows_per_batch) {
    IGemmParams p = IGemmParams();
    p.a0 = a; p.c0 = K; p.lda0 = K;
    p.B = M / rows_per_batch; p.Hin = p.Hout = rows_per_batch; p.Win = p.Wout = 1;
    p.ksize = 1; p.w = w; p.M = M; p.N = N; p.K = K; p.splitk = 0;
    return p;
  }
  IGemmParams conv3(const f16* a, int C, int Hin, int Win, int Hout, int Wout, int stride, int up, const f16* w, int N) {
    IGemmParams p = IGemmParams();
    p.a0 = a; p.c0 = C; p.lda0 = C;
    p.B = B; p.Hin = Hin; p.Win = Win; p.Hout = Hout; p.Wout = Wout;
    p.ksize = 3; p.stride = stride; p.up = up; p.w = w; p.M = B * Hout * Wout; p.N = N; p.K = 9 * C; p.splitk = 0;
    return p;
  }
  IGemmParams dense1x1(const f16* hi, const f16* lo, int M, int K, const f16* w, int N, int rows_per_batch, bool precise) {
    IGemmParams p = dense(hi, M, K, w, N, rows_per_batch);
    if (precise) {
      static const bool family = !(getenv("SDMI_SPLIT16_KERNEL") && atoi(getenv("SDMI_SPLIT16_KERNEL")) == 0);
      if (family && K % 64 == 0) {
        p.a1 = lo; p.lda1 = K; p.split16 = 1; p.ldw = 3 * K;
      } else {
        p.a1 = lo; p.c1 = K; p.lda1 = K; p.a2 = hi; p.c2 = K; p.lda2 = K; p.K = 3 * K; p.k_alg = K;
      }
    }
    return p;
  }
  long long* groupnorm(const Act& x0, const Act* x1, const float* gamma, const float* beta, float eps, int silu, f16* o16,
                       float* o32, f16* raw, f16* o16_lo = nullptr, f16* raw_lo = nullptr, bool stats_only = false,
                       bool already_applied = false) {
    GroupNormParams g = GroupNormParams();
    g.x0 = x0.p; g.c0 = x0.C;
    if (x1) { g.x1 = x1->p; g.c1 = x1->C; }
    g.B = B; g.HW = x0.H * x0.W; g.gamma = gamma; g.beta = beta; g.eps = eps; g.silu = silu;
    g.out_f16 = o16; g.out_f32 = o32; g.raw_f16 = raw; g.out_lo = o16_lo; g.raw_lo = raw_lo;
    g.stats_only = stats_only ? 1 : 0;
    const int idx = gn_calls;
    g.acc = next_gn_acc();
    if (plan) {
      const int cpg = (g.c0 + g.c1) / 32;
      if (dry) {
        const bool f = x0.stats && (!x1 || x1->stats) && x0.id >= 0 && (!x1 || x1->id >= 0);
        if ((int)plan->fused.size() <= idx) plan->fused.resize(idx + 1, 0);
        plan->fused[idx] = f ? 1 : 0;
        if (f) {
// ... 65 lines not shown
  int set_weight(const char* key, const float* ptr, const int64_t* shape, int ndim, hipStream_t stream);
  int finalize();
  int packed_layout(std::vector<std::pair<void**, size_t>>* bufs, int64_t* total) const;
  int export_packed(void* host_buf, int64_t bytes, hipStream_t stream);
  int import_packed(const void* host_buf, int64_t bytes, hipStream_t stream);
  int run(const float* x, const int64_t* t_i64, const float* t_f32, const float* ctx, float* eps_out, int B, int H, int W,
          int Lctx, void* workspace, int64_t ws_bytes, hipStream_t stream, bool dry, bool ctx_only, int64_t* bytes_needed);

  int cache_timesteps(const int64_t* t_host, int n, hipStream_t stream);
  int reserve_ctx_cache(int B, int Lctx);
  int hint_timestep(int64_t t);

  const std::vector<WeightSlot>& slots() const { return slots_; }

  sdmi_unet_cfg cfg_{};
  sdmi_unet_ext ext_{};
  bool has_ctx() const { return ext_.attention_block == 0; }
  int precision_ = SDMI_PRECISION_MIXED;
  bool full() const { return precision_ == SDMI_PRECISION_FULL; }
  int te_ = 0, emb_total_ = 0, n_attn_ = 0;
  f16* zero_ = nullptr;
  bool precise_1x1_ = true;
  bool precise_last_res_ = true;
  int precise_1x1_max_ds_ = 4;
  bool precise_kv_ = true;

 private:
  friend struct Fwd;
  void expect(const std::string& key, std::vector<int64_t> shape, WKind kind, void** dst, int row0 = 0, int ld = 0,
              void** dst2 = nullptr);
  int dev_alloc(void** dst, size_t bytes);
  size_t slot_bytes(const WeightSlot& s) const;
  int ensure_ctx_cache(int B, int Lctx, bool may_grow);
  GnPlan gn_plan_;
  bool fuse_gn_stats_ = true;
  bool ln_fold_ = true; int ln_fold_min_rows_ = 512;
  bool ff_tail_ = true;
  bool st_head_ = true;

  struct TapeKey {
    int B = 0, H = 0, W = 0, Lctx = 0, mode = 0;
    const void* ws = nullptr; int64_t ws_bytes = 0; bool have_ctx = false;
    uint64_t env = 0, weights_gen = 0, ctx_gen = 0;
    unsigned align = 0;
    bool operator==(const TapeKey& o) const {
      return B == o.B && H == o.H && W == o.W && Lctx == o.Lctx && mode == o.mode && ws == o.ws && ws_bytes == o.ws_bytes &&
             have_ctx == o.have_ctx && env == o.env && weights_gen == o.weights_gen && ctx_gen == o.ctx_gen && align == o.align;
    }
  };
  std::vector<std::pair<TapeKey, std::unique_ptr<Tape>>> tapes_;
  static constexpr size_t kMaxTapes = 12;
  uint64_t weights_gen_ = 0, ctx_gen_ = 0;
  int gn2_applied_ = 0;
 public:
  uint64_t tape_hits_ = 0, tape_records_ = 0;
 private:

  std::vector<std::vector<Layer>> input_blocks_, output_blocks_;
  std::vector<Layer> middle_;
  std::vector<WeightSlot> slots_;
  std::map<std::string, int> slot_index_;
  std::vector<void*> owned_;
  float *te_w0_ = nullptr, *te_b0_ = nullptr, *te_w2_ = nullptr, *te_b2_ = nullptr;
  float *emb_w_ = nullptr, *emb_b_ = nullptr;
  float *out_gamma_ = nullptr, *out_beta_ = nullptr, *out_w_ = nullptr, *out_b_ = nullptr;
  bool finalized_ = false;
  int ctx_B_ = 0, ctx_L_ = 0; bool ctx_valid_ = false;
  int64_t ctx_cap_ = 0;
  float* emb_tab_ = nullptr; size_t emb_tab_floats_ = 0;
  int64_t* emb_tab_tdev_ = nullptr; size_t emb_tab_tcap_ = 0;
  std::vector<int64_t> emb_tab_t_;
  std::vector<int64_t> emb_tab_src_;
  int emb_hint_row_ = -1;
  void drop_timestep_table() { emb_tab_t_.clear(); emb_hint_row_ = -1; }
};

}
```

Baseline: 3.617.

## Fuse resblock 1x1 skip GEMM into conv3 launch and defer its split-K reduce

New measurement: 3.676, median of 6. 1.7% higher.

```diff
diff --git a/include/sdmi.h b/include/sdmi.h
--- a/include/sdmi.h
+++ b/include/sdmi.h
@@ -171,6 +171,11 @@
   void* out_lo;
 } sdmi_igemm_desc;
 int sdmi_k_igemm(const sdmi_igemm_desc* d, void* stream);
+int sdmi_k_conv3_skip(const sdmi_igemm_desc* conv, const sdmi_igemm_desc* skip, int* rode, void* stream);
+int64_t sdmi_k_slab_floats(int M, int N, int bm, int bn, int nsplit);
+int64_t sdmi_k_slab_quad_offset(int bm, int bn, int wm, int wn, int N, int m4, int col);
+int sdmi_k_igemm_res_slabs(const sdmi_igemm_desc* skip, const sdmi_igemm_desc* conv, float* slab_ws, int64_t slab_ws_floats, int* deferred,
+                           void* stream);
 int sdmi_k_ff_tail(const sdmi_igemm_desc* proj_out, const void* ln_f16, const float* lnp, float ln_eps, const float* csd,
                    const void* wgg_f16, const void* wff2_f16, const float* bff2, const float* t, void* stream);
 int sdmi_k_st_tail(const sdmi_igemm_desc* proj_out, const void* a_f16, const void* wo_f16, const float* bo, float* t, const float* ln_gamma,
diff --git a/stable-diffusion_amd/_lib.py b/stable-diffusion_amd/_lib.py
--- a/stable-diffusion_amd/_lib.py
+++ b/stable-diffusion_amd/_lib.py
@@ -121,6 +121,10 @@
     'sdmi_bert_forward': (C.c_int, [c_ptr, c_ptr, c_ptr, C.c_int, C.c_int, c_ptr, C.c_int64, c_ptr]),
     'sdmi_has_experiments': (C.c_int, []),
     'sdmi_k_igemm': (C.c_int, [C.POINTER(IGemmDesc), c_ptr]),
+    'sdmi_k_slab_floats': (C.c_int64, [C.c_int] * 5),
+    'sdmi_k_slab_quad_offset': (C.c_int64, [C.c_int] * 7),
+    'sdmi_k_conv3_skip': (C.c_int, [C.POINTER(IGemmDesc), C.POINTER(IGemmDesc), C.POINTER(C.c_int32), c_ptr]),
+    'sdmi_k_igemm_res_slabs': (C.c_int, [C.POINTER(IGemmDesc), C.POINTER(IGemmDesc), c_ptr, C.c_int64, C.POINTER(C.c_int32), c_ptr]),
     'sdmi_k_ff_tail': (C.c_int, [C.POINTER(IGemmDesc), c_ptr, c_ptr, C.c_float, c_ptr, c_ptr, c_ptr, c_ptr, c_ptr, c_ptr]),
     'sdmi_k_gn_conv3': (C.c_int, [C.POINTER(IGemmDesc), c_ptr, c_ptr, C.c_int, C.c_int, c_ptr, C.c_int64, c_ptr, c_ptr, C.c_float, c_ptr]),
     'sdmi_k_st_mid_ctx': (C.c_int, [c_ptr, c_ptr, c_ptr, c_ptr, c_ptr, C.c_float, c_ptr, c_ptr, c_ptr, c_ptr, c_ptr, C.c_int, C.c_int, C.c_float, c_ptr,
diff --git a/stable-diffusion_amd/csrc/api.cpp b/stable-diffusion_amd/csrc/api.cpp
--- a/stable-diffusion_amd/csrc/api.cpp
+++ b/stable-diffusion_amd/csrc/api.cpp
@@ -349,6 +349,43 @@
   IGemmTune t; t.tile = d->tile; t.dma = d->dma;
   return launch_igemm(p, t, (hipStream_t)stream);
 }
+int sdmi_k_igemm_res_slabs(const sdmi_igemm_desc* skip, const sdmi_igemm_desc* conv, float* slab_ws, int64_t slab_ws_floats, int* deferred,
+                           void* stream) {
+  SDMI_CHECK(skip && conv, "null descriptor");
+  IGemmParams ps = IGemmParams(), pc = IGemmParams();
+  if (igemm_params_of(skip, ps) || igemm_params_of(conv, pc)) return -1;
+  SDMI_CHECK(ps.M == pc.M && ps.N == pc.N && ps.out_f32 && ps.out_f32 == pc.out_f32 && ps.ldo == pc.ldo && !pc.residual,
+             "res_slabs: the two GEMMs share M, N and the fp32 output (conv's in-place residual); conv has no other residual");
+  SlabDefer df;
+  df.ws = slab_ws; df.ws_floats = slab_ws_floats;
+  ps.defer = &df;
+  IGemmTune ts; ts.tile = skip->tile; ts.dma = skip->dma;
+  if (launch_igemm(ps, ts, (hipStream_t)stream)) return -1;
+  if (deferred) *deferred = df.got.nsplit > 0 ? 1 : 0;
+  if (df.got.nsplit > 0) pc.rs = df.got;
+  else { pc.residual = ps.out_f32; pc.ldr = ps.ldo; }
+  IGemmTune tc; tc.tile = conv->tile; tc.dma = conv->dma;
+  return launch_igemm(pc, tc, (hipStream_t)stream);
+}
+int64_t sdmi_k_slab_floats(int M, int N, int bm, int bn, int nsplit) { return tiled_slab_floats(M, N, bm, bn, nsplit); }
+int64_t sdmi_k_slab_quad_offset(int bm, int bn, int wm, int wn, int N, int m4, int col) {
+  SlabResidual r;
+  r.bm = bm; r.bn = bn; r.wm = wm; r.wn = wn;
+  return slab_quad_offset(r, N, m4, col);
+}
+int sdmi_k_conv3_skip(const sdmi_igemm_desc* conv, const sdmi_igemm_desc* skip, int* rode, void* stream) {
+  SDMI_CHECK(conv && skip, "null descriptor");
+  IGemmParams pc = IGemmParams(), ps = IGemmParams();
+  if (igemm_params_of(conv, pc) || igemm_params_of(skip, ps)) return -1;
+  int taken = 0;
+  pc.ride = &ps; pc.ride_taken = &taken;
+  IGemmTune tc; tc.tile = conv->tile; tc.dma = conv->dma;
+  if (launch_igemm(pc, tc, (hipStream_t)stream)) return -1;
+  if (rode) *rode = taken;
+  if (taken) return 0;
+  IGemmTune ts; ts.tile = skip->tile; ts.dma = skip->dma;
+  return launch_igemm(ps, ts, (hipStream_t)stream);
+}
 int sdmi_k_ff_tail(const sdmi_igemm_desc* proj_out, const void* ln_f16, const float* lnp, float ln_eps, const float* csd,
                    const void* wgg_f16, const void* wff2_f16, const float* bff2, const float* t, void* stream) {
   SDMI_CHECK(proj_out, "null descriptor");
diff --git a/stable-diffusion_amd/csrc/common.h b/stable-diffusion_amd/csrc/common.h
--- a/stable-diffusion_amd/csrc/common.h
+++ b/stable-diffusion_amd/csrc/common.h
@@ -106,6 +106,17 @@
 #define SDMI_ST_F32X4(base, off, val) SDMI_ST(f32x4, (base) + (off), (val))
 #define SDMI_ST_F16X4(base, off, val) SDMI_ST(f16x4, (base) + (off), (val))
 #endif
+
+struct SlabResidual {
+  const float* ws = nullptr; const float* bias = nullptr;
+  int nsplit = 0, bm = 0, bn = 0, wm = 0, wn = 0;
+};
+int64_t tiled_slab_floats(int M, int N, int bm, int bn, int nsplit);
+int64_t slab_quad_offset(const SlabResidual& r, int N, int m4, int col);
+struct SlabDefer {
+  float* ws = nullptr; int64_t ws_floats = 0;
+  SlabResidual got;
+};
 
 struct IGemmParams {
   const f16* a0 = nullptr; const f16* a1 = nullptr; const f16* a2 = nullptr;
@@ -166,6 +177,10 @@
   unsigned long long magic_cpg_in = 0;
   int halo_thi = 0, halo_ipt = 1, log2_tpi = 30;
   unsigned long long magic_hpi = 0;
+  SlabResidual rs;
+  SlabDefer* defer = nullptr;
+  const IGemmParams* ride = nullptr;
+  int* ride_taken = nullptr;
 };
 
 constexpr int SDMI_NUM_TILES = 22;
diff --git a/stable-diffusion_amd/csrc/conv3halo.hip b/stable-diffusion_amd/csrc/conv3halo.hip
--- a/stable-diffusion_amd/csrc/conv3halo.hip
+++ b/stable-diffusion_amd/csrc/conv3halo.hip
@@ -1,12 +1,17 @@
-#include "igemm_dev.h"
+#include "gemm_split16_body.h"
 
 namespace sdmi {
 namespace {
 
+template <int BM, int WARPS_M, int WARPS_N>
+constexpr int HALO_BUF_BYTES = (((BM / 64 + 2) * 66 + WARPS_M * WARPS_N * 8 - 1) / (WARPS_M * WARPS_N * 8)) * (WARPS_M * WARPS_N * 8) * 128;
 template <int BM, int BN, int WARPS_M, int WARPS_N, int NS>
-__global__ void __launch_bounds__(WARPS_M* WARPS_N * 64) conv3halo_kernel(const IGemmParams p, const int tiles_m,
-                                                                           const int tiles_n, const int chunks_per_split) {
+constexpr int HALO_LDS_BYTES = 2 * HALO_BUF_BYTES<BM, WARPS_M, WARPS_N> + NS * BN * 128;
+
 #if defined(__HIP_DEVICE_COMPILE__)
+template <int BM, int BN, int WARPS_M, int WARPS_N, int NS>
+__device__ __forceinline__ void conv3halo_body(const IGemmParams& p, const int tiles_m, const int tiles_n, const int chunks_per_split,
+                                               const int nblk, const int bid, unsigned char* const smem) {
   constexpr int NT = WARPS_M * WARPS_N * 64;
   constexpr int RPP = NT / 8;
   constexpr int PB = BN / RPP;
@@ -24,12 +29,8 @@
   constexpr int U = KS / G;
   constexpr int MPU = G * TM * TN;
   static_assert(PB >= 1 && TM >= 1 && TN >= 1 && RPP % 16 == 0 && NS >= 2 && NS <= 9, "tile/wave shape");
-  static_assert(LDS_BYTES <= 160 * 1024, "LDS budget");
-
-  __shared__ __attribute__((aligned(16))) unsigned char smem[LDS_BYTES];
-
-  const int nblk = gridDim.x;
-  const int bid = blockIdx.x;
+  static_assert(LDS_BYTES <= 160 * 1024 && LDS_BYTES == HALO_LDS_BYTES<BM, BN, WARPS_M, WARPS_N, NS>, "LDS budget");
+
   const int q8 = nblk >> 3, r8 = nblk & 7, xcd = bid & 7;
   const int wgid = (xcd < r8 ? xcd * (q8 + 1) : r8 * (q8 + 1) + (xcd - r8) * q8) + (bid >> 3);
   const int tiles_mn = tiles_m * tiles_n;
@@ -227,6 +228,32 @@
     d[0] = dbg_t0; d[1] = dbg_t1; d[2] = dbg_t2; d[4] = (long long)__builtin_readcyclecounter();
   }
 #endif
+}
+#endif
+
+template <int BM, int BN, int WARPS_M, int WARPS_N, int NS>
+__global__ void __launch_bounds__(WARPS_M* WARPS_N * 64) conv3halo_kernel(const IGemmParams p, const int tiles_m,
+                                                                           const int tiles_n, const int chunks_per_split) {
+#if defined(__HIP_DEVICE_COMPILE__)
+  __shared__ __attribute__((aligned(16))) unsigned char smem[HALO_LDS_BYTES<BM, BN, WARPS_M, WARPS_N, NS>];
+  conv3halo_body<BM, BN, WARPS_M, WARPS_N, NS>(p, tiles_m, tiles_n, chunks_per_split, (int)gridDim.x, (int)blockIdx.x, smem);
+#endif
+}
+
+template <int BM, int BN, int WARPS_M, int WARPS_N, int NS, int SBM, int SBN, int SNS>
+__global__ void __launch_bounds__(WARPS_M* WARPS_N * 64) conv3halo_kernel_ride(const IGemmParams p, const int tiles_m, const int tiles_n,
+                                                                                const int chunks_per_split, const int n_main,
+                                                                                const IGemmParams ps, const int s_tiles_m,
+                                                                                const int s_tiles_n, const int s_kt_per_split) {
+#if defined(__HIP_DEVICE_COMPILE__)
+  constexpr int LDS_BYTES = HALO_LDS_BYTES<BM, BN, WARPS_M, WARPS_N, NS>;
+  __shared__ __attribute__((aligned(16))) unsigned char smem[LDS_BYTES];
+  const int bid = (int)blockIdx.x;
+  if (bid >= n_main) {
+    gemm_split16_body<SBM, SBN, WARPS_M, WARPS_N, SNS, LDS_BYTES>(ps, s_tiles_m, s_tiles_n, s_kt_per_split, (int)gridDim.x - n_main, bid - n_main, smem);
+    return;
+  }
+  conv3halo_body<BM, BN, WARPS_M, WARPS_N, NS>(p, tiles_m, tiles_n, chunks_per_split, n_main, bid, smem);
 #endif
 }
 
@@ -240,6 +267,22 @@
   const int cap = (((bm / 64 + 2) * 66 + bm / 4 - 1) / (bm / 4)) * (bm / 4);
   if (bm <= HW) return HW % bm == 0 && (bm / W + 2) * (W + 2) <= cap;
   return bm % HW == 0 && p.M % bm == 0 && (bm / HW) * (p.Hout + 2) * (W + 2) <= cap;
+}
+
+static bool ride_ok(const IGemmParams& r, int n_main, int bm) {
+  const int knob = env_int("SDMI_SKIP_RIDE", 1);
+  if (!knob || (knob != 2 && bm != 256)) return false;
+  static const int n_cu = [] { int d = 0, n = 0; return (hipGetDevice(&d) == hipSuccess && hipDeviceGetAttribute(&n, hipDeviceAttributeMultiprocessorCount, d) == hipSuccess) ? n : 0; }();
+  if ((int64_t)n_main * 100 > (int64_t)n_cu * env_int("SDMI_SKIP_RIDE_FILL", 75)) return false;
+  if (!(r.split16 && r.a0 && r.a1 && r.ksize == 1 && r.mode == EPI_PLAIN && r.c1 == 0 && r.c2 == 0 && r.K == r.c0 && r.K % BK == 0 &&
+        r.lda0 % 8 == 0 && r.lda1 == r.lda0 && r.ldw % 8 == 0 && r.ldw >= 3 * r.K && r.M > 0 && r.N > 0 && r.M == r.B * r.Hout * r.Wout &&
+        r.zero_page))
+    return false;
+  if (range_check_enabled() || r.out_f16 || r.out_lo) return false;
+  if (r.gn_n || r.ln_out || r.lnp_out || r.f16_scale || r.lnf_part || r.pgn_out || r.rs.nsplit || r.ride) return false;
+  if ((int64_t)r.M * r.lda0 * 2 >= ((int64_t)1 << 31) - 65536 || (int64_t)r.N * r.ldw * 2 >= ((int64_t)1 << 31) - 65536) return false;
+  if ((int64_t)r.M >= (int64_t)65536 * r.Hout * r.Wout) return false;
+  return r.splitk == 1 || (r.splitk == 0 && igemm_table_split(r) == 1);
 }
 
 template <int BM, int BN, int WARPS_M, int WARPS_N, int NS>
@@ -280,13 +323,42 @@
   if (by_shape && prof_enabled())
     pname += "_M" + std::to_string(p.M) + "_N" + std::to_string(p.N) + "_K" + std::to_string(p.K) + "_s" + std::to_string(nsplit);
   const double src_pix = (double)p.B * p.Hin * p.Win;
-  ProfScope ps(pname.c_str(), 2.0 * p.M * (double)p.N * p.K,
-               src_pix * (p.c0 + p.c1) * 2.0 + (double)p.N * p.K * 2.0 + (double)p.M * p.N * ((p.out_f32 ? 4.0 : 0.0) + (p.out_f16 ? 2.0 : 0.0)) +
-                   (p.residual ? (double)p.M * p.N * 4.0 : 0.0),
-               stream);
-  SDMI_LAUNCH((conv3halo_kernel<BM, BN, WARPS_M, WARPS_N, NS>), grid, block, 0, stream, q, tiles_m, tiles_n, chunks_per_split);
-  SDMI_HIP_OK(hipGetLastError());
-  ps.end();
+  double flops = 2.0 * p.M * (double)p.N * p.K;
+  double bytes = src_pix * (p.c0 + p.c1) * 2.0 + (double)p.N * p.K * 2.0 + (double)p.M * p.N * ((p.out_f32 ? 4.0 : 0.0) + (p.out_f16 ? 2.0 : 0.0)) +
+                 (p.residual ? (double)p.M * p.N * 4.0 : 0.0);
+  constexpr bool CAN_RIDE = BN == 64 && (BM == 256 || BM == 128);
+  constexpr int SBM = BM / 2, SBN = 64, SNS = BM == 256 ? 3 : 4;
+  if (CAN_RIDE && p.ride && ride_ok(*p.ride, (int)grid.x, BM)) {
+    if constexpr (CAN_RIDE) {
+      const IGemmParams& r = *p.ride;
+      IGemmParams qs = r;
+      qs.splitk = 1; qs.splitk_fused = 0; qs.defer = nullptr; qs.ride_taken = nullptr;
+      qs.tile_n_fastest = tile_order_n_fastest(r);
+      slab_layout(qs, SBM, SBN, WARPS_M, WARPS_N, 1);
+      qs.epi_vec = epi_vec_ok(r);
+      qs.magic_hw = div_magic_hw(r.Hout * r.Wout);
+      qs.magic_w = div_magic(r.Wout);
+      const int s_tiles_m = cdiv(r.M, SBM), s_tiles_n = cdiv(r.N, SBN);
+      const int n_main = (int)grid.x;
+      grid.x += (unsigned)(s_tiles_m * s_tiles_n);
+      pname.insert(pname.find("_M") == std::string::npos ? pname.size() : pname.find("_M"), "+skip");
+      if (by_shape && prof_enabled()) pname += "+M" + std::to_string(r.M) + "_N" + std::to_string(r.N) + "_K" + std::to_string(r.K) + "_s1";
+      flops += 2.0 * r.M * (double)r.N * r.K;
+      bytes += (double)r.M * r.K * 2.0 + (double)r.N * r.K * 2.0 + (double)r.M * r.N * ((r.out_f32 ? 4.0 : 0.0) + (r.out_f16 ? 2.0 : 0.0)) +
+               (r.residual ? (double)r.M * r.N * 4.0 : 0.0);
+      ProfScope ps(pname.c_str(), flops, bytes, stream);
+      SDMI_LAUNCH((conv3halo_kernel_ride<BM, BN, WARPS_M, WARPS_N, NS, SBM, SBN, SNS>), grid, block, 0, stream, q, tiles_m, tiles_n,
+                  chunks_per_split, n_main, qs, s_tiles_m, s_tiles_n, r.K / BK);
+      SDMI_HIP_OK(hipGetLastError());
+      ps.end();
+      if (p.ride_taken) *p.ride_taken = 1;
+    }
+  } else {
+    ProfScope ps(pname.c_str(), flops, bytes, stream);
+    SDMI_LAUNCH((conv3halo_kernel<BM, BN, WARPS_M, WARPS_N, NS>), grid, block, 0, stream, q, tiles_m, tiles_n, chunks_per_split);
+    SDMI_HIP_OK(hipGetLastError());
+    ps.end();
+  }
   if (nsplit > 1) return launch_splitk_reduce(q, nsplit, stream);
   if (q.ln_out) return launch_layernorm(q.out_f32, q.ln_gamma, q.ln_beta, q.ln_out, q.M, q.N, q.ln_eps, stream);
   return 0;
diff --git a/stable-diffusion_amd/csrc/gemm_split16.hip b/stable-diffusion_amd/csrc/gemm_split16.hip
--- a/stable-diffusion_amd/csrc/gemm_split16.hip
+++ b/stable-diffusion_amd/csrc/gemm_split16.hip
@@ -1,4 +1,4 @@
-#include "igemm_dev.h"
+#include "gemm_split16_body.h"
 
 namespace sdmi {
 namespace {
@@ -7,151 +7,9 @@
 __global__ void __launch_bounds__(WARPS_M* WARPS_N * 64) gemm_split16_kernel(const IGemmParams p, const int tiles_m, const int tiles_n,
                                                                                const int kt_per_split) {
 #if defined(__HIP_DEVICE_COMPILE__)
-  constexpr int NT = WARPS_M * WARPS_N * 64;
-  constexpr int RPP = NT / 8;
-  constexpr int A_PASSES = BM / RPP, B_PASSES = BN / RPP;
-  constexpr int WTM = BM / WARPS_M, WTN = BN / WARPS_N;
-  constexpr int TM = WTM / 32, TN = WTN / 32;
-  constexpr int A_BYTES = BM * 128, B_BYTES = BN * 128;
-  constexpr int STAGE_BYTES = 2 * (A_BYTES + B_BYTES);
-  constexpr int LPT = 2 * (A_PASSES + B_PASSES);
-  constexpr int KS = BK / 16;
-  constexpr int PPU = (LPT + KS - 2) / (KS - 1);
-  static_assert(A_PASSES >= 1 && B_PASSES >= 1 && TM >= 1 && TN >= 1 && RPP % 16 == 0 && NS >= 2, "tile/wave shape");
-  static_assert(NS * STAGE_BYTES <= 160 * 1024, "LDS budget");
-
-  __shared__ __attribute__((aligned(16))) unsigned char smem[NS * STAGE_BYTES];
-
-  const int nblk = gridDim.x, bid = blockIdx.x;
-  const int q8 = nblk >> 3, r8 = nblk & 7, xcd = bid & 7;
-  const int wgid = (xcd < r8 ? xcd * (q8 + 1) : r8 * (q8 + 1) + (xcd - r8) * q8) + (bid >> 3);
-  const int tiles_mn = tiles_m * tiles_n;
-  const int split = wgid / tiles_mn;
-  const int tmn = wgid - split * tiles_mn;
-  int tile_m, tile_n;
-  if (p.tile_n_fastest) { tile_m = tmn / tiles_n; tile_n = tmn - tile_m * tiles_n; }
-  else { tile_n = tmn / tiles_m; tile_m = tmn - tile_n * tiles_m; }
-  const int m0 = tile_m * BM, n0 = tile_n * BN;
-  const int nkt = p.K / BK;
-  const int kt_begin = split * kt_per_split;
-  const int kt_end = min(nkt, kt_begin + kt_per_split);
-  if (kt_begin >= kt_end) return;
-
-  const int tid = threadIdx.x;
-  SDMI_STAMP(dbg_t0);
-  const int lane = tid & 63, wave = tid >> 6;
-  const int cpos = tid & 7, lrow = tid >> 3;
-  const int gch = cpos ^ ((lrow >> 1) & 7);
-  const int wave_u = __builtin_amdgcn_readfirstlane(wave);
-
-  int a_off[A_PASSES], b_off[B_PASSES];
-#pragma unroll
-  for (int i = 0; i < A_PASSES; ++i) a_off[i] = (min(m0 + i * RPP + lrow, p.M - 1) * p.lda0 + gch * 8) * 2;
-#pragma unroll
-  for (int i = 0; i < B_PASSES; ++i) b_off[i] = (min(n0 + i * RPP + lrow, p.N - 1) * p.ldw + gch * 8) * 2;
-  constexpr int OOB = (int)0x80000000;
-  const __amdgpu_buffer_rsrc_t rsrc_hi = __builtin_amdgcn_make_buffer_rsrc((void*)p.a0, 0, OOB, 0x00020000);
-  const __amdgpu_buffer_rsrc_t rsrc_lo = __builtin_amdgcn_make_buffer_rsrc((void*)p.a1, 0, OOB, 0x00020000);
-  const __amdgpu_buffer_rsrc_t rsrc_w = __builtin_amdgcn_make_buffer_rsrc((void*)p.w, 0, OOB, 0x00020000);
-  const int w_lo_off = 2 * p.K * 2;
-
-  auto issue_piece = [&](int kt, int stage, int q) {
-    const int soff = kt * (BK * 2);
-    const bool isA = q < 2 * A_PASSES;
-    const int qa = isA ? q : q - 2 * A_PASSES;
-    const int npass = isA ? A_PASSES : B_PASSES;
-    const int half = qa >= npass ? 1 : 0, pass = qa - half * npass;
-    const unsigned row0 = (isA ? half * BM : 2 * BM + half * BN) + pass * RPP + wave_u * 8;
-    auto dst = (__attribute__((address_space(3))) void*)(smem + stage * STAGE_BYTES + row0 * 128);
-    if (isA) __builtin_amdgcn_raw_ptr_buffer_load_lds(half ? rsrc_lo : rsrc_hi, dst, 16, a_off[pass], soff, 0, 0);
-    else __builtin_amdgcn_raw_ptr_buffer_load_lds(rsrc_w, dst, 16, b_off[pass], soff + (half ? w_lo_off : 0), 0, SDMI_W_AUX);
-  };
-
-  const int wm = wave / WARPS_N, wn = wave - wm * WARPS_N;
-  const int l31 = lane & 31, lg = lane >> 5;
-  const int rsw = (l31 >> 1) & 7;
-  f32x16 acc[TM][TN];
-#pragma unroll
-  for (int i = 0; i < TM; ++i)
-#pragma unroll
-    for (int j = 0; j < TN; ++j)
-#pragma unroll
-      for (int r = 0; r < 16; ++r) acc[i][j][r] = 0.f;
-
-  struct Frags { f16x8 ah[TM], al[TM], bh[TN], bl[TN]; };
-  const int a_lds = (wm * WTM + l31) * 128, b_lds = 2 * A_BYTES + (wn * WTN + l31) * 128;
-  auto read_frags = [&](int stage, int ks, Frags& f) {
-    const unsigned char* st = smem + stage * STAGE_BYTES + (((ks * 2 + lg) ^ rsw) << 4);
-#pragma unroll
-    for (int i = 0; i < TM; ++i) {
-      f.ah[i] = *(const f16x8*)(st + a_lds + i * 32 * 128);
-      f.al[i] = *(const f16x8*)(st + a_lds + A_BYTES + i * 32 * 128);
-    }
-#pragma unroll
-    for (int j = 0; j < TN; ++j) {
-      f.bh[j] = *(const f16x8*)(st + b_lds + j * 32 * 128);
-      f.bl[j] = *(const f16x8*)(st + b_lds + B_BYTES + j * 32 * 128);
-    }
-  };
-  auto mfma_step = [&](const Frags& f) {
-#pragma unroll
-    for (int i = 0; i < TM; ++i)
-#pragma unroll
-      for (int j = 0; j < TN; ++j) {
-        acc[i][j] = __builtin_amdgcn_mfma_f32_32x32x16_f16(f.ah[i], f.bh[j], acc[i][j], 0, 0, 0);
-        acc[i][j] = __builtin_amdgcn_mfma_f32_32x32x16_f16(f.al[i], f.bh[j], acc[i][j], 0, 0, 0);
-        acc[i][j] = __builtin_amdgcn_mfma_f32_32x32x16_f16(f.ah[i], f.bl[j], acc[i][j], 0, 0, 0);
-      }
-  };
-
-  SDMI_STAMP(dbg_t1);
-  int ld_kt = kt_begin;
-  auto next_kt = [&]() { const int k = ld_kt; if (ld_kt + 1 < kt_end) ++ld_kt; return k; };
-#pragma unroll
-  for (int s = 0; s < NS - 1; ++s) {
-    const int k = next_kt();
-#pragma unroll
-    for (int q = 0; q < LPT; ++q) issue_piece(k, s, q);
-  }
-  wait_vmcnt<LPT*(NS - 2)>();
-  asm volatile("s_waitcnt lgkmcnt(0)\n\ts_barrier" ::: "memory");
-  Frags fr[2];
-  read_frags(0, 0, fr[0]);
-  int cur = 0, nxt = NS - 1;
-  for (int kt = kt_begin; kt < kt_end; ++kt) {
-    const int kload = next_kt();
-    const int cur1 = (cur + 1 == NS) ? 0 : cur + 1;
-#pragma unroll
-    for (int u = 0; u < KS; ++u) {
-      if (u + 1 < KS) {
-        read_frags(cur, u + 1, fr[(u + 1) & 1]);
-#pragma unroll
-        for (int q = u * PPU; q < (u + 1) * PPU && q < LPT; ++q) issue_piece(kload, nxt, q);
-      } else {
-        wait_vmcnt<LPT*(NS - 2)>();
-        asm volatile("s_waitcnt lgkmcnt(0)\n\ts_barrier" ::: "memory");
-        read_frags(cur1, 0, fr[0]);
-      }
-      mfma_step(fr[u & 1]);
-      __builtin_amdgcn_sched_group_barrier(0x100, 2 * (TM + TN), 0);
-#pragma unroll
-      for (int e = 0; e < 3 * TM * TN; ++e) {
-        __builtin_amdgcn_sched_group_barrier(0x008, 1, 0);
-        if (u + 1 < KS && e < PPU && u * PPU + e < LPT) __builtin_amdgcn_sched_group_barrier(0x010, 1, 0);
-      }
-    }
-    cur = cur1;
-    nxt = (nxt + 1 == NS) ? 0 : nxt + 1;
-  }
-  wait_vmcnt<0>();
-  SDMI_STAMP(dbg_t2);
-  igemm_epilogue<BM, BN, WARPS_M, WARPS_N, NS * STAGE_BYTES>(p, acc, m0, n0, split, tile_m, tile_n, smem);
-#ifdef SDMI_IGEMM_TIMING
-  if (p.dbg_times && tid == 0) {
-    long long* d = p.dbg_times + 6 * (size_t)blockIdx.x;
-    d[0] = dbg_t0; d[1] = dbg_t1; d[2] = dbg_t2; d[4] = (long long)__builtin_readcyclecounter();
-  }
-#endif
+  constexpr int LDS_BYTES = SPLIT16_LDS_BYTES<BM, BN, NS>;
+  __shared__ __attribute__((aligned(16))) unsigned char smem[LDS_BYTES];
+  gemm_split16_body<BM, BN, WARPS_M, WARPS_N, NS, LDS_BYTES>(p, tiles_m, tiles_n, kt_per_split, (int)gridDim.x, (int)blockIdx.x, smem);
 #endif
 }
 
@@ -168,6 +26,7 @@
   slab_layout(q, BM, BN, WARPS_M, WARPS_N, nsplit);
   q.epi_vec = epi_vec_ok(p);
   SDMI_CHECK(splitk_ws_need(p, BM, BN, nsplit) <= p.splitk_ws_floats, "split-K workspace too small");
+  const bool deferred = defer_slabs(p, q, BM, BN, WARPS_M, WARPS_N, nsplit);
   SDMI_CHECK((int64_t)p.M < (int64_t)65536 * p.Hout * p.Wout, "fast_div_hw: at most 65535 samples per launch");
   q.magic_hw = div_magic_hw(p.Hout * p.Wout);
   q.magic_w = div_magic(p.Wout);
@@ -185,6 +44,7 @@
   SDMI_LAUNCH((gemm_split16_kernel<BM, BN, WARPS_M, WARPS_N, NS>), grid, block, 0, stream, q, tiles_m, tiles_n, kt_per_split);
   SDMI_HIP_OK(hipGetLastError());
   ps.end();
+  if (deferred) return 0;
   if (nsplit > 1) return launch_splitk_reduce(q, nsplit, stream);
   if (q.ln_out) return launch_layernorm(q.out_f32, q.ln_gamma, q.ln_beta, q.ln_out, q.M, q.N, q.ln_eps, stream);
   return 0;
diff --git a/stable-diffusion_amd/csrc/gemm_split16_body.h b/stable-diffusion_amd/csrc/gemm_split16_body.h
--- /dev/null
+++ b/stable-diffusion_amd/csrc/gemm_split16_body.h
@@ -0,0 +1,160 @@
+#pragma once
+#include "igemm_dev.h"
+
+namespace sdmi {
+namespace {
+
+template <int BM, int BN, int NS> constexpr int SPLIT16_LDS_BYTES = NS * 2 * (BM + BN) * 128;
+
+#if defined(__HIP_DEVICE_COMPILE__)
+template <int BM, int BN, int WARPS_M, int WARPS_N, int NS, int LDS_BYTES>
+__device__ __forceinline__ void gemm_split16_body(const IGemmParams& p, const int tiles_m, const int tiles_n, const int kt_per_split,
+                                                  const int nblk, const int bid, unsigned char* const smem) {
+  static_assert(LDS_BYTES >= SPLIT16_LDS_BYTES<BM, BN, NS>, "the ring does not fit the workgroup's LDS");
+  constexpr int NT = WARPS_M * WARPS_N * 64;
+  constexpr int RPP = NT / 8;
+  constexpr int A_PASSES = BM / RPP, B_PASSES = BN / RPP;
+  constexpr int WTM = BM / WARPS_M, WTN = BN / WARPS_N;
+  constexpr int TM = WTM / 32, TN = WTN / 32;
+  constexpr int A_BYTES = BM * 128, B_BYTES = BN * 128;
+  constexpr int STAGE_BYTES = 2 * (A_BYTES + B_BYTES);
+  constexpr int LPT = 2 * (A_PASSES + B_PASSES);
+  constexpr int KS = BK / 16;
+  constexpr int PPU = (LPT + KS - 2) / (KS - 1);
+  static_assert(A_PASSES >= 1 && B_PASSES >= 1 && TM >= 1 && TN >= 1 && RPP % 16 == 0 && NS >= 2, "tile/wave shape");
+  static_assert(NS * STAGE_BYTES == SPLIT16_LDS_BYTES<BM, BN, NS> && NS * STAGE_BYTES <= 160 * 1024, "LDS budget");
+
+  const int q8 = nblk >> 3, r8 = nblk & 7, xcd = bid & 7;
+  const int wgid = (xcd < r8 ? xcd * (q8 + 1) : r8 * (q8 + 1) + (xcd - r8) * q8) + (bid >> 3);
+  const int tiles_mn = tiles_m * tiles_n;
+  const int split = wgid / tiles_mn;
+  const int tmn = wgid - split * tiles_mn;
+  int tile_m, tile_n;
+  if (p.tile_n_fastest) { tile_m = tmn / tiles_n; tile_n = tmn - tile_m * tiles_n; }
+  else { tile_n = tmn / tiles_m; tile_m = tmn - tile_n * tiles_m; }
+  const int m0 = tile_m * BM, n0 = tile_n * BN;
+  const int nkt = p.K / BK;
+  const int kt_begin = split * kt_per_split;
+  const int kt_end = min(nkt, kt_begin + kt_per_split);
+  if (kt_begin >= kt_end) return;
+
+  const int tid = threadIdx.x;
+  SDMI_STAMP(dbg_t0);
+  const int lane = tid & 63, wave = tid >> 6;
+  const int cpos = tid & 7, lrow = tid >> 3;
+  const int gch = cpos ^ ((lrow >> 1) & 7);
+  const int wave_u = __builtin_amdgcn_readfirstlane(wave);
+
+  int a_off[A_PASSES], b_off[B_PASSES];
+#pragma unroll
+  for (int i = 0; i < A_PASSES; ++i) a_off[i] = (min(m0 + i * RPP + lrow, p.M - 1) * p.lda0 + gch * 8) * 2;
+#pragma unroll
+  for (int i = 0; i < B_PASSES; ++i) b_off[i] = (min(n0 + i * RPP + lrow, p.N - 1) * p.ldw + gch * 8) * 2;
+  constexpr int OOB = (int)0x80000000;
+  const __amdgpu_buffer_rsrc_t rsrc_hi = __builtin_amdgcn_make_buffer_rsrc((void*)p.a0, 0, OOB, 0x00020000);
+  const __amdgpu_buffer_rsrc_t rsrc_lo = __builtin_amdgcn_make_buffer_rsrc((void*)p.a1, 0, OOB, 0x00020000);
+  const __amdgpu_buffer_rsrc_t rsrc_w = __builtin_amdgcn_make_buffer_rsrc((void*)p.w, 0, OOB, 0x00020000);
+  const int w_lo_off = 2 * p.K * 2;
+
+  auto issue_piece = [&](int kt, int stage, int q) {
+    const int soff = kt * (BK * 2);
+    const bool isA = q < 2 * A_PASSES;
+    const int qa = isA ? q : q - 2 * A_PASSES;
+    const int npass = isA ? A_PASSES : B_PASSES;
+    const int half = qa >= npass ? 1 : 0, pass = qa - half * npass;
+    const unsigned row0 = (isA ? half * BM : 2 * BM + half * BN) + pass * RPP + wave_u * 8;
+    auto dst = (__attribute__((address_space(3))) void*)(smem + stage * STAGE_BYTES + row0 * 128);
+    if (isA) __builtin_amdgcn_raw_ptr_buffer_load_lds(half ? rsrc_lo : rsrc_hi, dst, 16, a_off[pass], soff, 0, 0);
+    else __builtin_amdgcn_raw_ptr_buffer_load_lds(rsrc_w, dst, 16, b_off[pass], soff + (half ? w_lo_off : 0), 0, SDMI_W_AUX);
+  };
+
+  const int wm = wave / WARPS_N, wn = wave - wm * WARPS_N;
+  const int l31 = lane & 31, lg = lane >> 5;
+  const int rsw = (l31 >> 1) & 7;
+  f32x16 acc[TM][TN];
+#pragma unroll
+  for (int i = 0; i < TM; ++i)
+#pragma unroll
+    for (int j = 0; j < TN; ++j)
+#pragma unroll
+      for (int r = 0; r < 16; ++r) acc[i][j][r] = 0.f;
+
+  struct Frags { f16x8 ah[TM], al[TM], bh[TN], bl[TN]; };
+  const int a_lds = (wm * WTM + l31) * 128, b_lds = 2 * A_BYTES + (wn * WTN + l31) * 128;
+  auto read_frags = [&](int stage, int ks, Frags& f) {
+    const unsigned char* st = smem + stage * STAGE_BYTES + (((ks * 2 + lg) ^ rsw) << 4);
+#pragma unroll
+    for (int i = 0; i < TM; ++i) {
+      f.ah[i] = *(const f16x8*)(st + a_lds + i * 32 * 128);
+      f.al[i] = *(const f16x8*)(st + a_lds + A_BYTES + i * 32 * 128);
+    }
+#pragma unroll
+    for (int j = 0; j < TN; ++j) {
+      f.bh[j] = *(const f16x8*)(st + b_lds + j * 32 * 128);
+      f.bl[j] = *(const f16x8*)(st + b_lds + B_BYTES + j * 32 * 128);
+    }
+  };
+  auto mfma_step = [&](const Frags& f) {
+#pragma unroll
+    for (int i = 0; i < TM; ++i)
+#pragma unroll
+      for (int j = 0; j < TN; ++j) {
+        acc[i][j] = __builtin_amdgcn_mfma_f32_32x32x16_f16(f.ah[i], f.bh[j], acc[i][j], 0, 0, 0);
+        acc[i][j] = __builtin_amdgcn_mfma_f32_32x32x16_f16(f.al[i], f.bh[j], acc[i][j], 0, 0, 0);
+        acc[i][j] = __builtin_amdgcn_mfma_f32_32x32x16_f16(f.ah[i], f.bl[j], acc[i][j], 0, 0, 0);
+      }
+  };
+
+  SDMI_STAMP(dbg_t1);
+  int ld_kt = kt_begin;
+  auto next_kt = [&]() { const int k = ld_kt; if (ld_kt + 1 < kt_end) ++ld_kt; return k; };
+#pragma unroll
+  for (int s = 0; s < NS - 1; ++s) {
+    const int k = next_kt();
+#pragma unroll
+    for (int q = 0; q < LPT; ++q) issue_piece(k, s, q);
+  }
+  wait_vmcnt<LPT*(NS - 2)>();
+  asm volatile("s_waitcnt lgkmcnt(0)\n\ts_barrier" ::: "memory");
+  Frags fr[2];
+  read_frags(0, 0, fr[0]);
+  int cur = 0, nxt = NS - 1;
+  for (int kt = kt_begin; kt < kt_end; ++kt) {
+    const int kload = next_kt();
+    const int cur1 = (cur + 1 == NS) ? 0 : cur + 1;
+#pragma unroll
+    for (int u = 0; u < KS; ++u) {
+      if (u + 1 < KS) {
+        read_frags(cur, u + 1, fr[(u + 1) & 1]);
+#pragma unroll
+        for (int q = u * PPU; q < (u + 1) * PPU && q < LPT; ++q) issue_piece(kload, nxt, q);
+      } else {
+        wait_vmcnt<LPT*(NS - 2)>();
+        asm volatile("s_waitcnt lgkmcnt(0)\n\ts_barrier" ::: "memory");
+        read_frags(cur1, 0, fr[0]);
+      }
+      mfma_step(fr[u & 1]);
+      __builtin_amdgcn_sched_group_barrier(0x100, 2 * (TM + TN), 0);
+#pragma unroll
+      for (int e = 0; e < 3 * TM * TN; ++e) {
+        __builtin_amdgcn_sched_group_barrier(0x008, 1, 0);
+        if (u + 1 < KS && e < PPU && u * PPU + e < LPT) __builtin_amdgcn_sched_group_barrier(0x010, 1, 0);
+      }
+    }
+    cur = cur1;
+    nxt = (nxt + 1 == NS) ? 0 : nxt + 1;
+  }
+  wait_vmcnt<0>();
+  SDMI_STAMP(dbg_t2);
+  igemm_epilogue<BM, BN, WARPS_M, WARPS_N, LDS_BYTES>(p, acc, m0, n0, split, tile_m, tile_n, smem);
+#ifdef SDMI_IGEMM_TIMING
+  if (p.dbg_times && tid == 0) {
+    long long* d = p.dbg_times + 6 * (size_t)blockIdx.x;
+    d[0] = dbg_t0; d[1] = dbg_t1; d[2] = dbg_t2; d[4] = (long long)__builtin_readcyclecounter();
+  }
+#endif
+}
+#endif
+
+}
+}
diff --git a/stable-diffusion_amd/csrc/igemm.hip b/stable-diffusion_amd/csrc/igemm.hip
--- a/stable-diffusion_amd/csrc/igemm.hip
+++ b/stable-diffusion_amd/csrc/igemm.hip
@@ -161,12 +161,25 @@
   t.valid = t.m < p.M && t.n < p.N;
   return t;
 }
+__host__ __device__ __forceinline__ size_t rs_quad_off(const SlabResidual& r, int N, int mb, int c) {
+  const int sh_bm = __builtin_ctz(r.bm), sh_bn = __builtin_ctz(r.bn);
+  const int sh_wtm = sh_bm - __builtin_ctz(r.wm), sh_wtn = sh_bn - __builtin_ctz(r.wn);
+  const int tiles_n = (N + r.bn - 1) >> sh_bn;
+  const int tile = (mb >> sh_bm) * tiles_n + (c >> sh_bn);
+  const int ml = mb & (r.bm - 1), cl = c & (r.bn - 1);
+  const int wave = (ml >> sh_wtm) * r.wn + (cl >> sh_wtn);
+  const int i = (ml & ((1 << sh_wtm) - 1)) >> 5, j = (cl & ((1 << sh_wtn) - 1)) >> 5, TN = 1 << (sh_wtn - 5);
+  const int r4 = (ml & 31) >> 3, lg = (ml >> 2) & 1;
+  const int thread = (wave << 6) + (lg << 5) + (cl & 31), NT = r.wm * r.wn * 64;
+  return ((size_t)tile << (sh_bm + sh_bn)) + (size_t)((((i * TN + j) * 4 + r4) * NT + thread) * 4);
+}
 #ifndef SDMI_REDUCE_GN_XCD_DEFAULT
 #define SDMI_REDUCE_GN_XCD_DEFAULT 0
 #endif
 constexpr int COOP_BAR_INTS = 18 * 32;
-template <bool COOP>
+template <bool COOP, bool RS = false>
 __global__ void __launch_bounds__(COOP ? 1024 : 256) splitk_reduce_tiled_kernel(IGemmParams p, int nsplit) {
+  static_assert(!(COOP && RS), "32 slab quads in flight do not fit the register budget of 1024-thread workgroups");
   constexpr int NWV = COOP ? 16 : 4;
   __shared__ unsigned long long s_gn[2][NWV][32][GN_WORDS];
   const int tid = threadIdx.x, lane = tid & 63, wv = tid >> 6, NTB = blockDim.x;
@@ -188,13 +201,32 @@
   f32x4 part[16];
 #pragma unroll
   for (int s = 0; s < 16; ++s) part[s] = (s < nsplit) ? *(const f32x4*)(src + s * split_stride) : f32x4{0.f, 0.f, 0.f, 0.f};
+  f32x4 rpart[RS ? 16 : 1], rbias = {0.f, 0.f, 0.f, 0.f};
+  if constexpr (RS) {
+    const int sub = lane & 3;
+    const int mb = min(t.m - sub, (p.M - 1) & ~3), c = n + sub;
+    const size_t rs_stride = (size_t)((p.M + p.rs.bm - 1) / p.rs.bm) * ((p.N + p.rs.bn - 1) / p.rs.bn) * (size_t)(p.rs.bm * p.rs.bn);
+    const float* rsrc = p.rs.ws + rs_quad_off(p.rs, p.N, mb, c);
+#pragma unroll
+    for (int s = 0; s < 16; ++s) rpart[s] = (s < p.rs.nsplit) ? *(const f32x4*)(rsrc + s * rs_stride) : f32x4{0.f, 0.f, 0.f, 0.f};
+    if (p.rs.bias) rbias = *(const f32x4*)(p.rs.bias + n);
+  }
   f32x4 a = part[0];
 #pragma unroll
   for (int s = 1; s < 16; ++s) a += part[s];
   f32x4 v = quad_transpose(a, lane & 3);
   v += biasv;
   if (p.rowvec) v += rvv;
-  if (p.residual) v += resv;
+  if constexpr (RS) {
+    f32x4 ra = rpart[0];
+#pragma unroll
+    for (int s = 1; s < 16; ++s) ra += rpart[s];
+    f32x4 r = quad_transpose(ra, lane & 3);
+    r += rbias;
+    v += r;
+  } else {
+    if (p.residual) v += resv;
+  }
   if (t.valid) {
     if (p.out_f32 && (!COOP || p.pgn_keep_f32)) SDMI_ST_F32X4(p.out_f32, (size_t)m * p.ldo + n, v);
     if (p.out_f16) SDMI_ST_F16X4(p.out_f16, (size_t)m * p.ldo + n, (f16x4{(f16)v[0], (f16)v[1], (f16)v[2], (f16)v[3]}));
@@ -319,8 +351,35 @@
 
 }
 
-int launch_splitk_reduce(const IGemmParams& p, int nsplit, hipStream_t stream) {
-  SDMI_CHECK(nsplit >= 1 && nsplit <= 16 && p.N % 4 == 0 && p.splitk_ws, "splitk_reduce: bad arguments");
+int64_t tiled_slab_floats(int M, int N, int bm, int bn, int nsplit) { return (int64_t)nsplit * cdiv(M, bm) * bm * cdiv(N, bn) * bn; }
+int64_t slab_quad_offset(const SlabResidual& r, int N, int m4, int col) { return (int64_t)rs_quad_off(r, N, m4, col); }
+
+static int launch_rs_materialize(const IGemmParams& p, hipStream_t stream) {
+  SDMI_CHECK(p.out_f32 && p.ldo % 4 == 0 && !p.residual, "residual as slabs: needs an fp32 output (the in-place residual) and no other residual");
+  IGemmParams r = IGemmParams();
+  r.M = p.M; r.N = p.N; r.B = p.B; r.Hout = p.Hout; r.Wout = p.Wout; r.mode = EPI_PLAIN;
+  r.bias = p.rs.bias; r.out_f32 = p.out_f32; r.ldo = p.ldo;
+  r.splitk = p.rs.nsplit; r.splitk_ws = const_cast<float*>(p.rs.ws);
+  r.splitk_ws_floats = tiled_slab_floats(p.M, p.N, p.rs.bm, p.rs.bn, p.rs.nsplit);
+  slab_layout(r, p.rs.bm, p.rs.bn, p.rs.wm, p.rs.wn, p.rs.nsplit);
+  r.slab_tiled = 1;
+  return launch_splitk_reduce(r, p.rs.nsplit, stream);
+}
+
+int launch_splitk_reduce(const IGemmParams& p_in, int nsplit, hipStream_t stream) {
+  SDMI_CHECK(nsplit >= 1 && nsplit <= 16 && p_in.N % 4 == 0 && p_in.splitk_ws, "splitk_reduce: bad arguments");
+  IGemmParams p_own;
+  const IGemmParams* pp = &p_in;
+  if (p_in.rs.nsplit > 0) {
+    SDMI_CHECK(p_in.rs.nsplit <= 16 && p_in.rs.ws && p_in.rs.bm > 0 && p_in.rs.bn > 0 && p_in.rs.wm > 0 && p_in.rs.wn > 0 && !p_in.residual,
+               "residual as slabs: bad descriptor");
+    if (!p_in.slab_tiled || p_in.mode != EPI_PLAIN || p_in.pgn_out) {
+      if (launch_rs_materialize(p_in, stream)) return -1;
+      p_own = p_in; p_own.rs = SlabResidual(); p_own.residual = p_in.out_f32; p_own.ldr = p_in.ldo;
+      pp = &p_own;
+    }
+  }
+  const IGemmParams& p = *pp;
   if (p.slab_tiled) {
     const int64_t quads = (int64_t)cdiv(p.M, p.slab_bm) * cdiv(p.N, p.slab_bn) * (p.slab_bm * p.slab_bn / 4);
     SDMI_CHECK(quads % 256 == 0 && quads / 256 < (1ll << 31) && p.slab_wm > 0 && p.slab_wn > 0, "tiled split-K slabs: bad geometry");
@@ -336,7 +395,8 @@
                       p.gn_cbase[0] == 0 && p.gn_cpg[0] == p.N / 32 && p.N % 128 == 0 && p.N / 32 >= 16 && p.M == p.B * p.Hout * p.Wout &&
                       (p.Hout * p.Wout) % 32 == 0 && !p.out_f16 && !p.out_lo && !p.ln_out && p.splitk_cnt && p.splitk_cnt_ints >= COOP_BAR_INTS &&
                       quads % 1024 == 0 && quads / 1024 <= 256 && (!p.pgn_keep_f32 || (p.out_f32 && p.ldo % 4 == 0));
-    ProfScope pst(coop ? "splitk_reduce_gn" : "splitk_reduce", 0.0, coop ? mn * (4.0 * nsplit + 2.0 + (p.pgn_keep_f32 ? 4.0 : 0.0)) : mn * 4.0 * (nsplit + 1), stream);
+    ProfScope pst(coop ? "splitk_reduce_gn" : "splitk_reduce", 0.0,
+                  coop ? mn * (4.0 * nsplit + 2.0 + (p.pgn_keep_f32 ? 4.0 : 0.0)) : mn * 4.0 * (nsplit + 1 + p.rs.nsplit), stream);
     const int rb_env = env_int("SDMI_REDUCE_BLOCK", 256);
     const int rb = (rb_env == 128 || (rb_env == 0 && quads / 256 < 512)) ? 128 : 256;
     if (coop) {
@@ -347,7 +407,8 @@
       if (range_check_enabled() && range_scan("GroupNorm fp16 output (split-K reduction)", p.pgn_out, (int64_t)p.M * p.N, stream)) return -1;
       return 0;
     }
-    SDMI_LAUNCH(splitk_reduce_tiled_kernel<false>, dim3((unsigned)(quads / rb)), dim3(rb), 0, stream, p, nsplit);
+    if (p.rs.nsplit > 0) SDMI_LAUNCH((splitk_reduce_tiled_kernel<false, true>), dim3((unsigned)(quads / rb)), dim3(rb), 0, stream, p, nsplit);
+    else SDMI_LAUNCH(splitk_reduce_tiled_kernel<false>, dim3((unsigned)(quads / rb)), dim3(rb), 0, stream, p, nsplit);
     SDMI_HIP_OK(hipGetLastError());
     pst.end();
     if (p.ln_out) return launch_layernorm(p.out_f32, p.ln_gamma, p.ln_beta, p.ln_out, p.M, p.N, p.ln_eps, stream);
@@ -578,7 +639,31 @@
   return 0;
 }
 
+static bool table_entry_ok(const IGemmParams& p, int tt, int sk, int splitk_req, bool can_split) {
+  const int nkt = p.K / BK;
+  const bool halo = tile_is_halo(tt);
+  const bool ws_ok = sk == 1 || (can_split && splitk_ws_need(p, kTiles[tt].bm, kTiles[tt].bn, sk) <= p.splitk_ws_floats);
+  const bool split_ok = splitk_req != 0 ? (sk == splitk_req && ws_ok)
+                                        : (sk == 1 || (ws_ok && nkt / sk >= 4 && (halo || (sk != 5 && sk != 10)) &&
+                                                       (!halo || (nkt / 9) % sk == 0)));
+  return split_ok && (p.mode != EPI_GEGLU || tile_tn_even(tt)) && (!halo || halo_supported(p, kTiles[tt].bm)) &&
+         (!p.split16 || split16_tile_supported(tt));
+}
+
+int igemm_table_split(const IGemmParams& p) {
+  if (env_int("SDMI_IGEMM_TILE", -1) >= 0 || env_int("SDMI_SPLITK", -1) >= 0) return -1;
+  std::lock_guard<std::mutex> lk(g_tuner.mu);
+  g_tuner.ensure_loaded();
+  if (g_tuner.collecting) return -1;
+  const TuneKey tkey{p.M, p.N, p.K, p.split16 ? 11 : p.ksize, p.stride, p.up, p.mode, 0};
+  auto it = g_tuner.table.find(tkey);
+  if (it == g_tuner.table.end()) return -1;
+  if (!table_entry_ok(p, it->second.tile, it->second.splitk, 0, false)) return -1;
+  return it->second.splitk;
+}
+
 int launch_igemm(const IGemmParams& p, const IGemmTune& tune, hipStream_t stream) {
+  if (p.ride_taken) *p.ride_taken = 0;
   SDMI_CHECK(p.M > 0 && p.N > 0 && p.K > 0, "empty GEMM");
   SDMI_CHECK(p.ksize == 1 || p.ksize == 3, "ksize must be 1 or 3");
   const int Cin = p.c0 + p.c1 + p.c2;
@@ -648,15 +733,7 @@
       auto it = g_tuner.table.find(tkey);
       if (it != g_tuner.table.end()) {
         const int tt = it->second.tile, sk = it->second.splitk;
-        const bool halo = tile_is_halo(tt);
-        const bool ws_ok = sk == 1 || (can_split && splitk_ws_need(p, kTiles[tt].bm, kTiles[tt].bn, sk) <= p.splitk_ws_floats);
-        const bool split_ok = splitk != 0 ? (sk == splitk && ws_ok)
-                                          : (sk == 1 || (ws_ok && nkt / sk >= 4 && (halo || (sk != 5 && sk != 10)) &&
-                                                         (!halo || (nkt / 9) % sk == 0)));
-        if (split_ok && (p.mode != EPI_GEGLU || tile_tn_even(tt)) && (!halo || halo_supported(p, kTiles[tt].bm)) &&
-            (!p.split16 || split16_tile_supported(tt))) {
-          tile = tt; splitk = sk;
-        }
+        if (table_entry_ok(p, tt, sk, splitk, can_split)) { tile = tt; splitk = sk; }
       }
     }
   }
@@ -688,6 +765,19 @@
   if (splitk > 1) {
     SDMI_CHECK(can_split, "split-K needs plain or head-scatter mode, a slab workspace and N / ldo / ldr multiples of 4");
     SDMI_CHECK(splitk_ws_need(p, kTiles[tile].bm, kTiles[tile].bn, splitk) <= p.splitk_ws_floats, "split-K workspace too small");
+  }
+  if (p.defer) p.defer->got = SlabResidual();
+  if (p.rs.nsplit > 0) {
+    SDMI_CHECK(p.mode == EPI_PLAIN && !p.residual, "residual as slabs: plain mode, no other residual");
+    const int units = tile_is_halo(tile) ? Cin / BK : nkt;
+    if (splitk <= 1 || cdiv(units, cdiv(units, splitk)) <= 1) {
+      if (ev0) { std::lock_guard<std::mutex> lk(g_tuner.mu); g_tuner.pool.push_back(ev0); g_tuner.pool.push_back(ev1); }
+      if (launch_rs_materialize(p, stream)) return -1;
+      IGemmParams p2 = p;
+      p2.rs = SlabResidual(); p2.residual = p.out_f32; p2.ldr = p.ldo; p2.splitk = 1;
+      IGemmTune t2; t2.tile = tile; t2.dma = tune.dma;
+      return launch_igemm(p2, t2, stream);
+    }
   }
   if (ev0) SDMI_HIP_OK(hipEventRecord(ev0, stream));
 #ifdef SDMI_IGEMM_TIMING
diff --git a/stable-diffusion_amd/csrc/igemm_dev.h b/stable-diffusion_amd/csrc/igemm_dev.h
--- a/stable-diffusion_amd/csrc/igemm_dev.h
+++ b/stable-diffusion_amd/csrc/igemm_dev.h
@@ -617,6 +617,18 @@
   q.slab_sh_qpt = lg2(bm * bn / 4); q.slab_sh_nt = lg2(wm * wn * 64); q.slab_sh_tn = lg2(bn / wn / 32); q.slab_sh_wn = lg2(wn);
   if (q.slab_tiled && (((wm * wn) & (wm * wn - 1)) || (wn & (wn - 1)))) q.slab_tiled = 0;
 }
+static bool defer_slabs(const IGemmParams& p, IGemmParams& q, int bm, int bn, int wm, int wn, int nsplit) {
+  if (!p.defer) return false;
+  p.defer->got = SlabResidual();
+  if (nsplit <= 1 || !q.slab_tiled || p.mode != EPI_PLAIN || p.rowvec || p.residual || p.rs.nsplit || p.out_f16 || p.out_lo || p.ln_out ||
+      p.gn_n || p.pgn_out || !p.defer->ws)
+    return false;
+  if (tiled_slab_floats(p.M, p.N, bm, bn, nsplit) > p.defer->ws_floats) return false;
+  q.splitk_ws = p.defer->ws; q.splitk_ws_floats = p.defer->ws_floats;
+  SlabResidual& g = p.defer->got;
+  g.ws = p.defer->ws; g.bias = p.bias; g.nsplit = nsplit; g.bm = bm; g.bn = bn; g.wm = wm; g.wn = wn;
+  return true;
+}
 static int64_t splitk_ws_need(const IGemmParams& p, int bm, int bn, int nsplit) {
   if (nsplit <= 1) return 0;
   if (slab_tiled_ok(p, bm, bn, nsplit)) return (int64_t)nsplit * cdiv(p.M, bm) * bm * cdiv(p.N, bn) * bn;
@@ -635,6 +647,7 @@
 
 }
 
+int igemm_table_split(const IGemmParams& p);
 bool halo_supported(const IGemmParams& p, int bm);
 int launch_halo_tile(int tile, const IGemmParams& p, int splitk, hipStream_t stream);
 bool split16_tile_supported(int tile);
diff --git a/stable-diffusion_amd/csrc/igemm_kernel.h b/stable-diffusion_amd/csrc/igemm_kernel.h
--- a/stable-diffusion_amd/csrc/igemm_kernel.h
+++ b/stable-diffusion_amd/csrc/igemm_kernel.h
@@ -299,6 +299,7 @@
   slab_layout(q, BM, BN, WARPS_M, WARPS_N, nsplit);
   q.epi_vec = epi_vec_ok(p);
   SDMI_CHECK(splitk_ws_need(p, BM, BN, nsplit) <= p.splitk_ws_floats, "split-K workspace too small");
+  const bool deferred = defer_slabs(p, q, BM, BN, WARPS_M, WARPS_N, nsplit);
   SDMI_CHECK((int64_t)p.M < (int64_t)65536 * p.Hout * p.Wout, "fast_div_hw: at most 65535 samples per launch");
   q.magic_hw = div_magic_hw(p.Hout * p.Wout);
   q.magic_w = div_magic(p.Wout);
@@ -333,6 +334,7 @@
 #undef SDMI_LAUNCH_KIND
   SDMI_HIP_OK(hipGetLastError());
   ps.end();
+  if (deferred) return 0;
   if (nsplit > 1) return launch_splitk_reduce(q, nsplit, stream);
   if (q.ln_out) return launch_layernorm(q.out_f32, q.ln_gamma, q.ln_beta, q.ln_out, q.M, q.N, q.ln_eps, stream);
   return 0;
diff --git a/stable-diffusion_amd/csrc/unet.cpp b/stable-diffusion_amd/csrc/unet.cpp
--- a/stable-diffusion_amd/csrc/unet.cpp
+++ b/stable-diffusion_amd/csrc/unet.cpp
@@ -549,6 +549,8 @@
   bool st_tail_on = false;
   bool st_mid_ctx_on = false;
   bool ctx1_on = false;
+  bool skip_ride_on = false;
+  bool skip_slabs_on = false;
   bool gn_conv_on = false;
   float* emb_all = nullptr;
   int emb_ld = 0;
@@ -575,6 +577,8 @@
     f16* a2 = nullptr;
     int& gn2_applied = u->gn2_applied_;
     gn2_applied = 0;
+    IGemmParams& ride = u->ride_params_; int& ride_taken = u->ride_taken_;
+    ride = IGemmParams(); ride_taken = 0;
     const bool gc1 = gn_conv_on && !p3 && Cin == Cout && gn_conv3_supported(B, H, W, x0.C, x1 ? x1->C : 0, Cout);
     const bool gc2 = gn_conv_on && !p3 && gn_conv3_supported(B, H, W, Cout, 0, Cout);
     auto gn_conv = [&](const Act& a0, const Act* a1, const float* gamma, const float* beta, const f16* w, IGemmParams& e) {
@@ -604,13 +608,24 @@
         a2 = S<f16>((size_t)M * Cout);
         p.pgn_gamma = L.f32[3]; p.pgn_beta = L.f32[4]; p.pgn_eps = 1e-5f; p.pgn_silu = 1; p.pgn_out = a2; p.pgn_applied = &gn2_applied;
       }
+      if (Cin != Cout) {
+        ride = dense1x1(raw, raw_lo, M, Cin, L.w16[2], Cout, H * W, p1);
+        ride.bias = L.f32[6]; ride.out_f32 = out.p; ride.ldo = Cout; ride.zero_page = zero;
+        if (skip_ride_on && ride.split16) { p.ride = &ride; p.ride_taken = &ride_taken; }
+      }
       TapeCaller tc(Tape::R_EMB, emb_caller ? p.rowvec : nullptr);
       gemm(p);
     }
     const float* residual = x0.p;
-    if (Cin != Cout) {
-      IGemmParams p = dense1x1(raw, raw_lo, M, Cin, L.w16[2], Cout, H * W, p1);
-      p.bias = L.f32[6]; p.out_f32 = out.p; p.ldo = Cout;
+    SlabDefer& skip_slabs = u->skip_slabs_;
+    skip_slabs = SlabDefer();
+    if (Cin != Cout && ride_taken) residual = out.p;
+    else if (Cin != Cout) {
+      IGemmParams p = ride;
+      if (skip_slabs_on && !gc2) {
+        skip_slabs.ws = skip_ws; skip_slabs.ws_floats = skip_ws_floats;
+        p.defer = &skip_slabs;
+      }
       gemm(p);
       residual = out.p;
     }
@@ -627,6 +642,7 @@
       IGemmParams p = conv3(a2, Cout, H, W, H, W, 1, 0, L.w16[1], Cout);
       if (p3) split3(p, a2, a2_lo, Cout);
       p.bias = L.f32[5]; p.residual = residual; p.ldr = Cout; p.out_f32 = out.p; p.ldo = Cout;
+      if (skip_slabs.got.nsplit > 0) { p.residual = nullptr; p.ldr = 0; p.rs = skip_slabs.got; }
       attach_gn_targets(p, out);
       attach_f16_copy(p, out);
       gemm(p);
@@ -1182,6 +1198,10 @@
     f.ctx1_on = !(e_c1 && atoi(e_c1) == 0);
     const char* e_gc = getenv("SDMI_GN_CONV");
     f.gn_conv_on = e_gc ? atoi(e_gc) != 0 : false;
+    const char* e_ss = getenv("SDMI_SKIP_SLABS");
+    f.skip_slabs_on = !(e_ss && atoi(e_ss) == 0) && !full();
+    const char* e_sr = getenv("SDMI_SKIP_RIDE");
+    f.skip_ride_on = !(e_sr && atoi(e_sr) == 0) && !full();
     if (full()) {
       f.ln_fold_on = f.ff_tail_on = f.st_head_on = f.st_mid_on = f.st_tail_on = f.st_mid_ctx_on = f.gn_conv_on = false;
     }
diff --git a/stable-diffusion_amd/csrc/unet.h b/stable-diffusion_amd/csrc/unet.h
--- a/stable-diffusion_amd/csrc/unet.h
+++ b/stable-diffusion_amd/csrc/unet.h
@@ -42,6 +42,7 @@
   long long* gn_acc = nullptr;
   int gn_calls = 0;
   float* splitk_ws = nullptr; int64_t splitk_ws_floats = 0;
+  float* skip_ws = nullptr; int64_t skip_ws_floats = 0;
   int* splitk_cnt = nullptr;
   static constexpr int SPLITK_CNT_INTS = 8192;
   int rc = 0;
@@ -103,7 +104,8 @@
     if (!dry) SDMI_HIP_OK(memset_async(blk, 0, (acc_words + SPLITK_CNT_INTS / 2) * sizeof(long long), s));
     splitk_ws_floats = splitk_floats;
     splitk_ws = P<float>((size_t)splitk_floats);
-    (void)P<float>((size_t)(splitk_floats / 2));
+    skip_ws_floats = splitk_floats / 2;
+    skip_ws = P<float>((size_t)skip_ws_floats);
     return 0;
   }
 
@@ -275,6 +277,8 @@
   static constexpr size_t kMaxTapes = 12;
   uint64_t weights_gen_ = 0, ctx_gen_ = 0;
   int gn2_applied_ = 0;
+  IGemmParams ride_params_; int ride_taken_ = 0;
+  SlabDefer skip_slabs_;
  public:
   uint64_t tape_hits_ = 0, tape_records_ = 0;
  private:
```
